# rodrigo-paganini/kalman-vae

Hardware: AMD Instinct MI355X
Metric: sequences/sec (ELBO training step, 32x32xT bouncing-ball) (higher is better)
Workload: dtype f32; 1 GPU; BASELINE configs[1] (configs[2] per-GPU shard): bouncing-ball 32x32, T=50, batch=256/GPU, dynamics=lstm K=3, z=4, u=4, a=2, full train step (fwd incl. sigmoid(x_logits) + loss incl. active-unit stats + bwd + clip + Adam); both the GPU leg and the cpu_baseline leg do this work; preset=c2, global_batch=256, seq_len=50, parallelism=dp1, capture=hipgraph, loss_finite=True, dist_backend=none

## Files before the change

include/kvae_lgssm.h:

```cpp
#ifndef KVAE_LGSSM_H
#define KVAE_LGSSM_H

#include <stdint.h>

#ifdef __cplusplus
extern "C" {
#endif

#define KVAE_MAX_DIM 16
#define KVAE_ABI_VERSION 20

typedef enum {
  KVAE_OK = 0,
  KVAE_ERR_DIMS = 1,
  KVAE_ERR_NULL = 2,
  KVAE_ERR_LAUNCH = 3,
  KVAE_ERR_ARG = 4
} kvae_status;

typedef struct {
  const float *ptr;
  int64_t sb, st;
} kvae_stack;

typedef struct {
  int32_t B, T, n, m, p;
  kvae_stack A;
  kvae_stack Bm;
  kvae_stack C;
  kvae_stack Q;
  const float *R;
  const float *mu0;
  int64_t mu0_sb;
  const float *Sigma0;
  int64_t Sigma0_sb;
  const float *Y;
  const float *U;
  const float *mask;
} kvae_lgssm_problem;

typedef struct {
  float *mus_filt;
  float *Sigmas_filt;
  float *mus_pred;
  float *Sigmas_pred;
  float *mus_smooth;
  float *Sigmas_smooth;
  float *aux;
} kvae_lgssm_states;
#define KVAE_AUX(n, p) ((n) * (p) + (p) * (p) + (n) * (n))

typedef struct {
  float *ptr;
  int64_t sb, st;
} kvae_gstack;

typedef struct {
  kvae_gstack gA, gB, gC, gQ;
  float *gY, *gU;
  float *g_mu0, *g_Sigma0;
} kvae_lgssm_input_grads;


int kvae_lgssm_filter_fwd(const kvae_lgssm_problem *prob, const kvae_lgssm_states *out, void *stream);

int kvae_lgssm_rts_fwd(const kvae_lgssm_problem *prob, const kvae_lgssm_states *io, void *stream);

int kvae_lgssm_smooth_fwd(const kvae_lgssm_problem *prob, const kvae_lgssm_states *out, void *stream);

int kvae_lgssm_filter_alpha_lstm(const kvae_lgssm_problem *prob, const kvae_lgssm_states *out, const float *w_ih,
                                 const float *w_hh, const float *b_ih, const float *b_hh, const float *head_w,
                                 const float *head_b, const float *A, const float *Bm, const float *C, int32_t K, int32_t H,
                                 float *record, float *alpha, float *gates, float *c_seq, float *h_seq, float *x_seq,
                                 void *stream);


int kvae_lgssm_smooth_bwd(const kvae_lgssm_problem *prob, const kvae_lgssm_states *saved,
                          const kvae_lgssm_states *up, const kvae_lgssm_input_grads *out,
                          float *ws, int with_rts, void *stream);

int kvae_lgssm_alpha_lstm_bwd(const kvae_lgssm_problem *prob, const kvae_lgssm_states *saved, const kvae_lgssm_states *up,
                              const kvae_lgssm_input_grads *out, float *ws, int with_rts, const float *w_ih,
                              const float *w_hh, const float *head_w, const float *A, const float *Bm, const float *C,
                              int32_t K, int32_t H, const float *alpha, const float *gates, const float *c_seq,
                              const float *g_record_up, const float *g_alpha_up, float *g_record, float *d_pre,
                              float *g_logit, void *stream);


int kvae_lgssm_elbo(const kvae_lgssm_problem *prob, const float *mus_smooth, const float *Sigmas_smooth,
                    const float *eps, float *terms, int32_t *chol_levels, float *ws_lz, float *g_mus,
                    float *g_Sigmas, const kvae_lgssm_input_grads *g, void *stream);


int kvae_mix_fwd(const float *alpha, const float *base, float *out, int64_t rows, int32_t K, int32_t E,
                 void *stream);

int kvae_mix_bwd(const float *alpha, const float *base, const float *g_out, float *g_alpha, float *g_base,
                 float *partials, int64_t rows, int32_t K, int32_t E, int32_t accumulate_alpha, void *stream);
int64_t kvae_mix_bwd_partials(int64_t rows);


int kvae_lstm_fwd(const float *x, const float *w_ih, const float *w_hh, const float *b_ih, const float *b_hh,
                  float *h_seq, float *gates, float *c_seq, int32_t B, int32_t T, int32_t I, int32_t H, void *stream);

int kvae_lstm_bwd(const float *g_h, const float *gates, const float *c_seq, const float *w_ih, const float *w_hh,
                  float *d_pre, float *dx, int32_t B, int32_t T, int32_t I, int32_t H, void *stream);


int kvae_regime_fwd(const float *logits, const float *init_logits, const float *gumbel, const float *P, float *y_seq,
                    float *log_q, float *log_p, int32_t B, int32_t T, int32_t K, float tau, const float *tau_dev,
                    int32_t hard, void *stream);
int kvae_regime_bwd(const float *logits, const float *init_logits, const float *gumbel, const float *P,
                    const float *y_seq, const float *g_y, const float *g_log_q, const float *g_log_p, float *g_logits,
                    float *g_init, int32_t B, int32_t T, int32_t K, float tau, const float *tau_dev, void *stream);

int kvae_regime_decode(const float *logits, const float *init_logits, const float *P, float *marginals, int32_t *path,
                       float *path_logq, float *kl, void *ws, int32_t B, int32_t T, int32_t K, void *stream);
int64_t kvae_regime_decode_ws_bytes(int64_t B, int32_t T, int32_t K);


int kvae_bigru_fwd(const float *x, const float *const w_ih[2], const float *const w_hh[2], const float *const b_ih[2],
                   const float *const b_hh[2], float *h_seq, float *gates, int32_t B, int32_t T, int32_t I, int32_t H,
                   void *stream);
int kvae_bigru_bwd(const float *g_h, const float *gates, const float *h_seq, const float *const w_ih[2],
                   const float *const w_hh[2], float *d_pre_i, float *d_pre_h, float *dx, int32_t B, int32_t T,
                   int32_t I, int32_t H, void *stream);


int kvae_bias_shuffle_act_fwd(const float *in, const float *bias, float *out, int64_t N, int32_t C, int32_t H,
                              int32_t W, int32_t r, int32_t relu, void *stream);
int kvae_bias_shuffle_act_bwd(const float *g_out, const float *out, float *g_in, float *bias_partials, int64_t N,
                              int32_t C, int32_t H, int32_t W, int32_t r, int32_t relu, void *stream);
int64_t kvae_bias_partial_rows(int64_t N);
int kvae_colsum(const float *partials, float *out, int64_t rows, int64_t cols, void *stream);
int kvae_colsum2(const float *partials_a, float *out_a, int64_t rows_a, int64_t cols_a, const float *partials_b, float *out_b,
                 int64_t rows_b, int64_t cols_b, void *stream);


int kvae_clip_adam(float *params, const float *grads, float *exp_avg, float *exp_avg_sq, int64_t n, const int32_t *seg_of,
                   int32_t n_seg, const float *seg_active, float *seg_steps, const float *lr_dev, float lr, float beta1, float beta2,
                   float eps, float weight_decay, float clip, const float *div_dev, float *norm_out, float *ws, void *stream);


int kvae_lgssm_emission_means(const kvae_lgssm_problem *prob, const float *mus_smooth, const float *mus_filt, float *a_imputed,
                              float *a_filtered, void *stream);


typedef struct kvae_wgrad_problem {
  const float *d;
  const float *h;
  const float *x;
  float *g_wh, *g_wx, *g_b;
  int64_t d_stride, h_stride, x_stride, N;
  int32_t R, H, I, bias, T, shift;
} kvae_wgrad_problem;
int64_t kvae_rnn_wgrad_ws_floats(const kvae_wgrad_problem *probs, int32_t n);
int kvae_rnn_wgrad(const kvae_wgrad_problem *probs, int32_t n, float *ws, void *stream);

int kvae_linear_fwd(const float *x, int64_t x_stride, int64_t N, int32_t F, const float *W, const float *b, int32_t O,
                    int32_t softmax, float *y, void *stream);
int kvae_linear_bwd_input(const float *g, const float *y, int64_t N, int32_t F, const float *W, int32_t O, float *g_logit,
                          float *dx, int64_t dx_stride, void *stream);


int kvae_bce_frames_fwd(const float *logits, const float *x, float *frame_ll, int64_t frames, int32_t pixels, void *stream);
int kvae_bce_frames_bwd(const float *logits, const float *x, const float *g_frame, float *g_logits, int64_t frames,
                        int32_t pixels, void *stream);


#define KVAE_DEC_HEAD_SCRATCH_FLOATS 2304
int kvae_dec_head_fwd(const float *in, const float *W, const float *bias, float *logits, float *w_scratch, int64_t N,
                      int32_t Cin, int32_t side, void *stream);
int kvae_dec_head_bwd(const float *in, const float *W, const float *g_logits, float *g_in, float *w_partials,
                      float *b_partials, float *w_scratch, int64_t N, int32_t Cin, int32_t side, void *stream);
int kvae_dec_head_loss_fwd(const float *in, const float *W, const float *bias, const float *x, float *logits, float *x_recon,
                           float *frame_ll, float *w_scratch, int64_t N, int32_t Cin, int32_t side, void *stream);
int kvae_dec_head_loss_bwd(const float *in, const float *W, const float *logits, const float *x, const float *g_frame, float *g_in,
                           float *w_partials, float *b_partials, float *w_scratch, int64_t N, int32_t Cin, int32_t side,
                           void *stream);
int kvae_enc_stem_fwd(const float *x, const float *W, const float *bias, float *out, uint32_t *relu_bits, int64_t N, int32_t Cout,
                      int32_t side, void *stream);
int kvae_enc_stem_bwd(const float *x, const float *out, const uint32_t *relu_bits, const float *g_out, float *w_partials,
                      float *b_partials, int64_t N, int32_t Cout, int32_t side, void *stream);
int64_t kvae_conv_edge_partial_rows(int64_t N);

int kvae_enc_mid_fwd(const float *in, const float *W, const float *bias, float *out, int64_t N, int32_t C, int32_t side,
                     void *stream);
int kvae_enc_mid_bwd(const float *in, const float *W, const float *out, const float *g_out, float *g_in,
                     float *w_partials, float *b_partials, int64_t N, int32_t C, int32_t side, void *stream);
int64_t kvae_enc_mid_partial_rows(int64_t N, int32_t side);

int kvae_dec_up_fwd(const float *x, const float *W, const float *bias, float *out, int64_t N, int32_t Cin, int32_t side,
                    void *stream);
int kvae_dec_up_bwd(const float *x, const float *W, const float *out, const float *g_out, float *g_x, float *w_partials,
                    float *b_partials, int64_t N, int32_t Cin, int32_t side, void *stream);
int64_t kvae_dec_up_partial_rows(int64_t N, int32_t side);
int32_t kvae_dec_up_set_workgroups(int32_t n);


int kvae_enc_head_fwd(const float *feat, const float *Wmu, const float *bmu, const float *Wvar, const float *bvar,
                      const float *eps, float *mu, float *var, float *a, int64_t N, int32_t F, int32_t A,
                      float noise_emission, void *stream);
int kvae_enc_head_bwd(const float *feat, const float *Wmu, const float *Wvar, const float *var, const float *eps,
                      const float *g_a, const float *g_mu, const float *g_var, float *g_feat, float *w_partials,
                      float *b_partials, int64_t N, int32_t F, int32_t A, float noise_emission, void *stream);
int kvae_dec_fc_fwd(const float *a, const float *W, const float *b, float *h, int64_t N, int32_t F, int32_t A, void *stream);
int kvae_dec_fc_bwd(const float *g_h, const float *a, const float *W, float *g_a, float *w_partials, float *b_partials,
                    int64_t N, int32_t F, int32_t A, void *stream);
int64_t kvae_head_partial_rows(void);
int kvae_latent_reg_fwd(const float *a, const float *mu, const float *var, float *reg, int64_t N, int32_t A, void *stream);
int kvae_latent_reg_bwd(const float *a, const float *mu, const float *var, const float *g, float *g_a, float *g_mu,
                        float *g_var, int64_t N, int32_t A, void *stream);

int kvae_loss_head_fwd(const float *lpx, const float *regf, const float *mask, const float *elbo_kf, const float *beta,
                       float scale_reconstruction, float vae_weight, float kf_weight, const float *weights_dev, float *out6,
                       float *coef3, int64_t n, void *stream);
int kvae_loss_head_bwd(const float *g_loss, const float *coef3, const float *mask, float *g_lpx, float *g_regf,
                       float *g_elbo_kf, int64_t n, void *stream);

typedef struct {
  int32_t B, S, H;
  int32_t n, m, p, K;
  int32_t kind;
  int32_t hidden;
  const float *A;
  const float *Bm;
  const float *C;
  const float *LQ;
  const float *LR;
  const float *mu;
  const float *L0;
  const float *U;
  const float *w_ih;
  const float *w_hh;
  const float *b_ih;
  const float *b_hh;
  const float *head_w;
  const float *head_b;
  const float *h0;
  const float *c0;
  const float *y0;
  const float *P;
  const float *s0;
  const float *eps0;
  const float *eps_z;
  const float *eps_a;
  const float *gumbel;
  float *a_out;
  float *z_out;
  float *w_out;
} kvae_gen_problem;
int kvae_lgssm_generate(const kvae_gen_problem *prob, void *stream);

#define KVAE_PSAMPLE_GAINS 1
#define KVAE_PSAMPLE_PATHS 2
typedef struct {
  int32_t B, S, T;
  int32_t n, p;
  int32_t stages;
  const float *mus_filt;
  const float *Sigmas_filt;
  const float *mus_pred;
  const float *Sigmas_pred;
  kvae_stack A;
  kvae_stack C;
  kvae_stack Q;
  const float *LR;
  const float *eps;
  const float *eta;
  float *z_out;
  float *a_out;
  int32_t *levels_out;
  float *ws;
} kvae_psample_problem;
int kvae_lgssm_posterior_sample(const kvae_psample_problem *prob, void *stream);
int64_t kvae_lgssm_posterior_sample_ws_floats(const kvae_psample_problem *prob);

typedef struct {
  int32_t B, T, n, p;
  const float *mus_pred;
  const float *Sigmas_pred;
  kvae_stack C;
  const float *R;
  const float *y;
  const float *mask;
  float *ll;
  float *nis;
  float *a_pred;
  float *S_out;
  int32_t *levels;
  float *seq_ll;
} kvae_pred_problem;
int kvae_lgssm_predictive(const kvae_pred_problem *prob, void *stream);

typedef struct {
  const float *g_ll;
  const float *g_seq;
  float *g_mus_pred;
  float *g_Sigmas_pred;
  float *gY;
  kvae_gstack gC;
} kvae_pred_grads;
int kvae_lgssm_predictive_bwd(const kvae_pred_problem *prob, const kvae_pred_grads *g, void *stream);

typedef struct {
  int32_t B, T, K, n, m, p;
  const float *A;
  const float *Bm;
  const float *Q;
  const float *C;
  const float *R;
  const float *P;
  const float *mu0;
  const float *Sigma0;
  const float *y;
  const float *u;
  const float *mask;
  const float *state_log_w;
  const float *state_mu;
  const float *state_Sigma;
  float *regime_filt;
  float *regime_pred;
  float *ll;
  float *seq_ll;
  float *a_pred;
  float *S_out;
  float *mus_filt;
  float *Sigmas_filt;
  int32_t *levels;
  float *out_log_w;
  float *out_mu;
  float *out_Sigma;
} kvae_swf_problem;
int kvae_lgssm_switching_filter(const kvae_swf_problem *prob, void *stream);

typedef struct {
  kvae_swf_problem filt;
  float *hist_mu;
  float *hist_Sigma;
  float *hist_W;
  float *hist_w;
  float *regime_smooth;
  float *regime_pairs;
  float *mus_smooth;
  float *Sigmas_smooth;
} kvae_sws_problem;
int kvae_lgssm_switching_smoother(const kvae_sws_problem *prob, void *stream);

typedef struct {
  kvae_swf_problem filt;
  float *hist_lw;
  float *hist_mu;
  float *hist_Sigma;
} kvae_swm_problem;
typedef struct {
  const float *g_ll;
  const float *g_seq;
  float *ws;
  float *gA;
  float *gB;
  float *gQ;
  float *gC;
  float *g_logP;
  float *g_mu0;
  float *g_Sigma0;
  float *gY;
  float *gU;
  float *ll_recomputed;
} kvae_swm_grads;
int kvae_lgssm_switching_marginal(const kvae_swm_problem *prob, void *stream);
int kvae_lgssm_switching_marginal_bwd(const kvae_swm_problem *prob, const kvae_swm_grads *g, void *stream);
int64_t kvae_lgssm_switching_marginal_ws_floats(int32_t B, int32_t K, int32_t n, int32_t m);

typedef struct {
  float *ws;
  float *N;
  float *S11;
  float *S10;
  float *S00;
  float *counts;
  float *Syz;
  float *Szz;
  float *Syy;
  float *Nobs;
  float *z0;
  float *z0z0;
  float *nseq;
} kvae_em_stats;
int kvae_lgssm_switching_em(const kvae_sws_problem *prob, const kvae_em_stats *st, void *stream);
int64_t kvae_lgssm_switching_em_ws_floats(int32_t B, int32_t K, int32_t n, int32_t m);

int kvae_abi_version(void);
const char *kvae_last_error(void);
const char *kvae_build_info(void);

#ifdef __cplusplus
}
#endif
#endif
```

kalman-vae_amd/csrc/kvae_vae.hip:

```cpp
#include <hip/hip_runtime.h>

#include <stdint.h>
#include <stdio.h>
#include <stdlib.h>
#include <string.h>

#include "../../include/kvae_lgssm.h"

namespace kvae {}
using namespace kvae;

extern "C" int kvae_launch_status(const char *what);
static int launch_status(const char *what) { return kvae_launch_status(what); }

#include "vae_epilogue.h"

__device__ __forceinline__ void colsum_v4_body(const float *__restrict__ partials, float *__restrict__ out, int64_t rows, int64_t cols,
                                               unsigned block) {
  __shared__ float4 red[8][64];
  const int lane = threadIdx.x & 63, wv = threadIdx.x >> 6;
  const int64_t c = ((int64_t)block * 64 + lane) * 4;
  float4 s0 = make_float4(0.f, 0.f, 0.f, 0.f), s1 = s0, s2 = s0, s3 = s0;
  if (c < cols) {
    const float *p = partials + c;
    int64_t r = wv;
    for (; r + 24 < rows; r += 32) {
      const float4 a = *reinterpret_cast<const float4 *>(p + r * cols), b = *reinterpret_cast<const float4 *>(p + (r + 8) * cols),
                   d = *reinterpret_cast<const float4 *>(p + (r + 16) * cols), e = *reinterpret_cast<const float4 *>(p + (r + 24) * cols);
      s0.x += a.x; s0.y += a.y; s0.z += a.z; s0.w += a.w;
      s1.x += b.x; s1.y += b.y; s1.z += b.z; s1.w += b.w;
      s2.x += d.x; s2.y += d.y; s2.z += d.z; s2.w += d.w;
      s3.x += e.x; s3.y += e.y; s3.z += e.z; s3.w += e.w;
    }
    for (; r < rows; r += 8) {
      const float4 a = *reinterpret_cast<const float4 *>(p + r * cols);
      s0.x += a.x; s0.y += a.y; s0.z += a.z; s0.w += a.w;
    }
  }
  red[wv][lane] = make_float4((s0.x + s1.x) + (s2.x + s3.x), (s0.y + s1.y) + (s2.y + s3.y), (s0.z + s1.z) + (s2.z + s3.z),
                              (s0.w + s1.w) + (s2.w + s3.w));
  __syncthreads();
  if (wv == 0 && c < cols) {
    float4 t = red[0][lane];
#pragma unroll
    for (int w = 1; w < 8; ++w) { const float4 u = red[w][lane]; t.x += u.x; t.y += u.y; t.z += u.z; t.w += u.w; }
    *reinterpret_cast<float4 *>(out + c) = t;
  }
}
__global__ __launch_bounds__(512) void k_colsum_v4(const float *__restrict__ partials, float *__restrict__ out, int64_t rows,
                                                   int64_t cols) {
  colsum_v4_body(partials, out, rows, cols, blockIdx.x);
}
__global__ __launch_bounds__(512) void k_colsum_v4_pair(const float *__restrict__ pa, float *__restrict__ oa, int64_t rows_a, int64_t cols_a,
                                                        unsigned nb_a, const float *__restrict__ pb, float *__restrict__ ob,
                                                        int64_t rows_b, int64_t cols_b) {
  if (blockIdx.x < nb_a) colsum_v4_body(pa, oa, rows_a, cols_a, blockIdx.x);
  else colsum_v4_body(pb, ob, rows_b, cols_b, blockIdx.x - nb_a);
}
__global__ __launch_bounds__(256) void k_colsum(const float *__restrict__ partials, float *__restrict__ out, int64_t rows,
                                                int64_t cols) {
  __shared__ float red[256];
  const int cx = threadIdx.x & 63, ry = threadIdx.x >> 6;
  const int64_t c = (int64_t)blockIdx.x * 64 + cx;
  float s0 = 0.f, s1 = 0.f;
  if (c < cols) {
    int64_t r = ry;
    for (; r + 4 < rows; r += 8) {
      s0 += partials[r * cols + c];
      s1 += partials[(r + 4) * cols + c];
    }
    if (r < rows) s0 += partials[r * cols + c];
  }
  red[threadIdx.x] = s0 + s1;
  __syncthreads();
  if (ry == 0 && c < cols) out[c] = (red[cx] + red[64 + cx]) + (red[128 + cx] + red[192 + cx]);
}

template <int R>
__global__ __launch_bounds__(256) void k_vae_epilogue_fwd_v4(const float *__restrict__ in, const float *__restrict__ bias,
                                                             float *__restrict__ out, int C, int H, int W, int64_t quads,
                                                             int relu) {
  const int OW = W * R, OH = H * R, QW = OW / 4;
  for (int64_t qd = (int64_t)blockIdx.x * 256 + threadIdx.x; qd < quads; qd += (int64_t)gridDim.x * 256) {
    const int qw = (int)(qd % QW);
    const int64_t t1 = qd / QW;
    const int oh = (int)(t1 % OH);
    const int64_t t2 = t1 / OH;
    const int c = (int)(t2 % C);
    const int64_t n = t2 / C;
    float4 v;
    if (R == 1) {
      const float b = bias[c];
      const float4 x = *reinterpret_cast<const float4 *>(in + ((n * C + c) * H + oh) * W + 4 * qw);
      v = make_float4(x.x + b, x.y + b, x.z + b, x.w + b);
    } else {
      const int ch0 = c * 4 + (oh & 1) * 2;
      const int64_t base = ((n * (C * 4) + ch0) * H + (oh >> 1)) * W + 2 * qw;
      const float2 a = *reinterpret_cast<const float2 *>(in + base);
      const float2 d = *reinterpret_cast<const float2 *>(in + base + (int64_t)H * W);
      const float b0 = bias[ch0], b1 = bias[ch0 + 1];
      v = make_float4(a.x + b0, d.x + b1, a.y + b0, d.y + b1);
    }
    if (relu) v = make_float4(fmaxf(v.x, 0.f), fmaxf(v.y, 0.f), fmaxf(v.z, 0.f), fmaxf(v.w, 0.f));
    *reinterpret_cast<float4 *>(out + qd * 4) = v;
  }
}

__global__ __launch_bounds__(256) void k_vae_epilogue_fwd(const float *in, const float *bias, float *out, EpiShape s,
                                                          int64_t total, int relu) {
  for (int64_t o = (int64_t)blockIdx.x * 256 + threadIdx.x; o < total; o += (int64_t)gridDim.x * 256)
    epi_fwd_elem(s, in, bias, out, o, relu);
}

__global__ __launch_bounds__(256) void k_vae_epilogue_bwd_bias(const float *__restrict__ g_out, const float *__restrict__ out,
                                                               float *__restrict__ g_in, float *__restrict__ bias_partials,
                                                               EpiShape s, int n_per_chunk, int relu) {
  extern __shared__ float bins[];
  const int Cin = s.C * s.r * s.r;
  const int OW = s.W * s.r, OH = s.H * s.r;
  const int64_t vol = (int64_t)s.C * OH * OW;
  for (int i = threadIdx.x; i < Cin; i += 256) bins[i] = 0.f;
  __syncthreads();
  const int64_t pos = (int64_t)blockIdx.x * 256 + threadIdx.x;
  if (pos < vol) {
    const int ow = (int)(pos % OW);
    const int oh = (int)((pos / OW) % OH);
    const int c = (int)(pos / ((int64_t)OW * OH));
    const int ch = c * s.r * s.r + (oh % s.r) * s.r + (ow % s.r);
    const int64_t in_off = ((int64_t)ch * s.H + oh / s.r) * s.W + ow / s.r;
    const int64_t in_vol = (int64_t)Cin * s.H * s.W;
    const int64_t n0 = (int64_t)blockIdx.y * n_per_chunk;
    const int64_t n1 = n0 + n_per_chunk < s.N ? n0 + n_per_chunk : s.N;
    float acc = 0.f;
    for (int64_t n = n0; n < n1; ++n) {
      float g = g_out[n * vol + pos];
      if (relu && !(out[n * vol + pos] > 0.f)) g = 0.f;
      g_in[n * in_vol + in_off] = g;
      acc += g;
    }
    atomicAdd(&bins[ch], acc);
  }
  __syncthreads();
  for (int i = threadIdx.x; i < Cin; i += 256) {
    if (bins[i] != 0.f) atomicAdd(&bias_partials[(int64_t)blockIdx.y * Cin + i], bins[i]);
  }
}

__global__ __launch_bounds__(256) void k_vae_epilogue_bwd(const float *g_out, const float *out, float *g_in, EpiShape s,
                                                          int64_t total, int relu) {
  for (int64_t o = (int64_t)blockIdx.x * 256 + threadIdx.x; o < total; o += (int64_t)gridDim.x * 256)
    epi_bwd_elem(s, g_out, out, g_in, o, relu);
}

#define KVAE_EPI_SAMPLES_PER_CHUNK 32
extern "C" int64_t kvae_bias_partial_rows(int64_t N);
static unsigned epi_grid(int64_t total) {
  const int64_t blocks = (total + 255) / 256;
  return (unsigned)(blocks < 256 * 32 ? blocks : 256 * 32);
}

extern "C" {
int kvae_bias_shuffle_act_fwd(const float *in, const float *bias, float *out, int64_t N, int32_t C, int32_t H, int32_t W,
                              int32_t r, int32_t relu, void *stream) {
  if (!in || !bias || !out) return KVAE_ERR_NULL;
  if (N < 1 || C < 1 || H < 1 || W < 1 || r < 1) return KVAE_ERR_ARG;
  const EpiShape s{N, C, H, W, r};
  const int64_t total = N * C * H * W * r * r;
  const bool aligned = ((uintptr_t)in % 16 == 0) && ((uintptr_t)out % 16 == 0);
  if (aligned && r == 1 && W % 4 == 0)
    k_vae_epilogue_fwd_v4<1><<<dim3(epi_grid(total / 4)), dim3(256), 0, (hipStream_t)stream>>>(in, bias, out, C, H, W, total / 4, relu);
  else if (aligned && r == 2 && W % 2 == 0)
    k_vae_epilogue_fwd_v4<2><<<dim3(epi_grid(total / 4)), dim3(256), 0, (hipStream_t)stream>>>(in, bias, out, C, H, W, total / 4, relu);
  else
    k_vae_epilogue_fwd<<<dim3(epi_grid(total)), dim3(256), 0, (hipStream_t)stream>>>(in, bias, out, s, total, relu);
  return launch_status("k_vae_epilogue_fwd");
}
int kvae_bias_shuffle_act_bwd(const float *g_out, const float *out, float *g_in, float *bias_partials, int64_t N, int32_t C,
                              int32_t H, int32_t W, int32_t r, int32_t relu, void *stream) {
  if (!g_out || !g_in || (relu && !out)) return KVAE_ERR_NULL;
  if (N < 1 || C < 1 || H < 1 || W < 1 || r < 1) return KVAE_ERR_ARG;
  const EpiShape s{N, C, H, W, r};
  const int64_t total = N * C * H * W * r * r;
  hipStream_t st = (hipStream_t)stream;
  if (bias_partials) {
    const int Cin = C * r * r;
    const int64_t chunks = kvae_bias_partial_rows(N);
    if (hipMemsetAsync(bias_partials, 0, sizeof(float) * chunks * Cin, st) != hipSuccess) return launch_status("memset bias_partials");
    const int64_t vol = (int64_t)C * H * W * r * r;
    k_vae_epilogue_bwd_bias<<<dim3((unsigned)((vol + 255) / 256), (unsigned)chunks), dim3(256), sizeof(float) * Cin, st>>>(
        g_out, out, g_in, bias_partials, s, KVAE_EPI_SAMPLES_PER_CHUNK, relu);
    return launch_status("k_vae_epilogue_bwd_bias");
  }
  k_vae_epilogue_bwd<<<dim3(epi_grid(total)), dim3(256), 0, st>>>(g_out, out, g_in, s, total, relu);
  return launch_status("k_vae_epilogue_bwd");
}
int kvae_colsum(const float *partials, float *out, int64_t rows, int64_t cols, void *stream) {
  if (!partials || !out) return KVAE_ERR_NULL;
  if (rows < 1 || cols < 1) return KVAE_ERR_ARG;
  if ((cols & 3) == 0 && ((((uintptr_t)partials | (uintptr_t)out) & 15) == 0))
    k_colsum_v4<<<dim3((unsigned)((cols + 255) / 256)), dim3(512), 0, (hipStream_t)stream>>>(partials, out, rows, cols);
  else
    k_colsum<<<dim3((unsigned)((cols + 63) / 64)), dim3(256), 0, (hipStream_t)stream>>>(partials, out, rows, cols);
  return launch_status("k_colsum");
}
int kvae_colsum2(const float *pa, float *oa, int64_t rows_a, int64_t cols_a, const float *pb, float *ob, int64_t rows_b,
                 int64_t cols_b, void *stream) {
  if (!pa || !oa || !pb || !ob) return KVAE_ERR_NULL;
  if (rows_a < 1 || cols_a < 1 || rows_b < 1 || cols_b < 1) return KVAE_ERR_ARG;
  if (((cols_a | cols_b) & 3) == 0 && ((((uintptr_t)pa | (uintptr_t)oa | (uintptr_t)pb | (uintptr_t)ob) & 15) == 0)) {
    const unsigned nb_a = (unsigned)((cols_a + 255) / 256), nb_b = (unsigned)((cols_b + 255) / 256);
    k_colsum_v4_pair<<<dim3(nb_a + nb_b), dim3(512), 0, (hipStream_t)stream>>>(pa, oa, rows_a, cols_a, nb_a, pb, ob, rows_b, cols_b);
    return launch_status("k_colsum_v4_pair");
  }
  const int rc = kvae_colsum(pa, oa, rows_a, cols_a, stream);
  return rc ? rc : kvae_colsum(pb, ob, rows_b, cols_b, stream);
}
int64_t kvae_bias_partial_rows(int64_t N) { return (N + KVAE_EPI_SAMPLES_PER_CHUNK - 1) / KVAE_EPI_SAMPLES_PER_CHUNK; }
}

constexpr int CA_BLOCKS = 512;
constexpr int CA_MAX_SEG = 1024;
__global__ __launch_bounds__(256) void k_grad_sumsq(const float *__restrict__ g, int64_t n, const int32_t *__restrict__ seg_of,
                                                    int n_seg, const float *__restrict__ seg_active,
                                                    const float *__restrict__ div_dev, float *__restrict__ seg_steps,
                                                    float *__restrict__ ws) {
  __shared__ float red[256];
  const float inv = div_dev ? 1.0f / fmaxf(*div_dev, 1.0f) : 1.0f;
  float s = 0.f;
  for (int64_t i = (int64_t)blockIdx.x * 256 + threadIdx.x; i < n; i += (int64_t)gridDim.x * 256) {
    float v = g[i] * inv;
    if (seg_active && seg_active[seg_of ? seg_of[i] : 0] == 0.f) v = 0.f;
    s = fmaf(v, v, s);
  }
  red[threadIdx.x] = s;
  __syncthreads();
  for (int o = 128; o > 0; o >>= 1) {
    if ((int)threadIdx.x < o) red[threadIdx.x] += red[threadIdx.x + o];
    __syncthreads();
  }
  if (threadIdx.x == 0) ws[blockIdx.x] = red[0];
  if (blockIdx.x == 0)
    for (int sg = threadIdx.x; sg < n_seg; sg += 256)
      if (!seg_active || seg_active[sg] != 0.f) seg_steps[sg] += 1.0f;
}
__global__ __launch_bounds__(256) void k_clip_adam(float *__restrict__ p, const float *__restrict__ g, float *__restrict__ m,
                                                   float *__restrict__ v, int64_t n, const int32_t *__restrict__ seg_of, int n_seg,
                                                   const float *__restrict__ seg_active, const float *__restrict__ seg_steps,
                                                   const float *__restrict__ lr_dev, float lr, float beta1, float beta2, float eps,
                                                   float wd, float clip, const float *__restrict__ div_dev,
                                                   float *__restrict__ norm_out, const float *__restrict__ ws, int nparts) {
  __shared__ float red[256];
  __shared__ float s_step_size[CA_MAX_SEG], s_bc2s[CA_MAX_SEG];
  float s = 0.f;
  for (int i = threadIdx.x; i < nparts; i += 256) s += ws[i];
  red[threadIdx.x] = s;
  const float lrv = lr_dev ? *lr_dev : lr;
  for (int sg = threadIdx.x; sg < n_seg; sg += 256) {
    const float step = seg_steps[sg];
    const bool on = !seg_active || seg_active[sg] != 0.f;
    s_step_size[sg] = on ? lrv / (1.0f - powf(beta1, step)) : -1.0f;
    s_bc2s[sg] = on ? sqrtf(1.0f - powf(beta2, step)) : 1.0f;
  }
  __syncthreads();
  for (int o = 128; o > 0; o >>= 1) {
    if ((int)threadIdx.x < o) red[threadIdx.x] += red[threadIdx.x + o];
    __syncthreads();
  }
  const float total = sqrtf(red[0]);
  if (norm_out && blockIdx.x == 0 && threadIdx.x == 0) *norm_out = total;
  const float inv = div_dev ? 1.0f / fmaxf(*div_dev, 1.0f) : 1.0f;
  const float scale = inv * (clip > 0.f ? fminf(clip / (total + 1e-6f), 1.0f) : 1.0f);
  for (int64_t i = (int64_t)blockIdx.x * 256 + threadIdx.x; i < n; i += (int64_t)gridDim.x * 256) {
    const int sg = seg_of ? seg_of[i] : 0;
    const float step_size = s_step_size[sg], bc2s = s_bc2s[sg];
    if (step_size < 0.f) continue;
    float gi = g[i] * scale;
    const float pi = p[i];
    if (wd != 0.f) gi = fmaf(wd, pi, gi);
    const float mi = m[i] + (gi - m[i]) * (1.0f - beta1);
    const float vi = beta2 * v[i] + (1.0f - beta2) * gi * gi;
    m[i] = mi, v[i] = vi;
    p[i] = pi - step_size * mi / (sqrtf(vi) / bc2s + eps);
  }
}
extern "C" int kvae_clip_adam(float *params, const float *grads, float *exp_avg, float *exp_avg_sq, int64_t n,
                              const int32_t *seg_of, int32_t n_seg, const float *seg_active, float *seg_steps, const float *lr_dev,
                              float lr, float beta1, float beta2, float eps, float weight_decay, float clip, const float *div_dev,
                              float *norm_out, float *ws, void *stream) {
  if (!params || !grads || !exp_avg || !exp_avg_sq || !seg_steps || !ws) return KVAE_ERR_NULL;
  if (n < 1 || n_seg < 1 || n_seg > CA_MAX_SEG || (!seg_of && n_seg != 1)) return KVAE_ERR_ARG;
  const int64_t want = (n + 1023) / 1024;
  const unsigned parts = (unsigned)(want < CA_BLOCKS ? want : CA_BLOCKS);
  k_grad_sumsq<<<dim3(parts), dim3(256), 0, (hipStream_t)stream>>>(grads, n, seg_of, n_seg, seg_active, div_dev, seg_steps, ws);
  int rc = launch_status("k_grad_sumsq");
  if (rc) return rc;
  const unsigned blocks = (unsigned)((n + 255) / 256 < 2048 ? (n + 255) / 256 : 2048);
  k_clip_adam<<<dim3(blocks), dim3(256), 0, (hipStream_t)stream>>>(params, grads, exp_avg, exp_avg_sq, n, seg_of, n_seg, seg_active,
                                                                   seg_steps, lr_dev, lr, beta1, beta2, eps, weight_decay, clip,
                                                                   div_dev, norm_out, ws, (int)parts);
  return launch_status("k_clip_adam");
}

#include "vae_loss.h"

__global__ __launch_bounds__(256) void k_vae_bce_fwd(const float *__restrict__ logits, const float *__restrict__ x,
                                                     float *__restrict__ frame_ll, int64_t frames, int pixels) {
  const int64_t f = (int64_t)blockIdx.x * 4 + (threadIdx.x >> 6);
  const int lane = threadIdx.x & 63;
  if (f >= frames) return;
  const float *l = logits + f * pixels, *t = x + f * pixels;
  float acc = 0.f;
  if ((pixels & 3) == 0 && (((uintptr_t)l | (uintptr_t)t) & 15) == 0) {
    for (int i = lane * 4; i < pixels; i += 256) {
      const float4 a = *reinterpret_cast<const float4 *>(l + i), b = *reinterpret_cast<const float4 *>(t + i);
      acc += bce_logit(a.x, b.x) + bce_logit(a.y, b.y) + bce_logit(a.z, b.z) + bce_logit(a.w, b.w);
    }
  } else {
    for (int i = lane; i < pixels; i += 64) acc += bce_logit(l[i], t[i]);
  }
  for (int off = 32; off > 0; off >>= 1) acc += __shfl_down(acc, off, 64);
  if (lane == 0) frame_ll[f] = -acc;
}

__global__ __launch_bounds__(256) void k_vae_bce_bwd(const float *__restrict__ logits, const float *__restrict__ x,
                                                     const float *__restrict__ g_frame, float *__restrict__ g_logits,
                                                     int64_t total, int pixels) {
  for (int64_t i = ((int64_t)blockIdx.x * 256 + threadIdx.x) * 4; i < total; i += (int64_t)gridDim.x * 1024) {
    const float g = -g_frame[i / pixels];
    const float4 a = *reinterpret_cast<const float4 *>(logits + i), b = *reinterpret_cast<const float4 *>(x + i);
    *reinterpret_cast<float4 *>(g_logits + i) = make_float4(g * (sigmoid_stable(a.x) - b.x), g * (sigmoid_stable(a.y) - b.y),
                                                            g * (sigmoid_stable(a.z) - b.z), g * (sigmoid_stable(a.w) - b.w));
  }
}
__global__ __launch_bounds__(256) void k_vae_bce_bwd_scalar(const float *logits, const float *x, const float *g_frame,
                                                            float *g_logits, int64_t total, int pixels) {
  for (int64_t i = (int64_t)blockIdx.x * 256 + threadIdx.x; i < total; i += (int64_t)gridDim.x * 256)
    g_logits[i] = -g_frame[i / pixels] * (sigmoid_stable(logits[i]) - x[i]);
}

extern "C" {
int kvae_bce_frames_fwd(const float *logits, const float *x, float *frame_ll, int64_t frames, int32_t pixels, void *stream) {
  if (!logits || !x || !frame_ll) return KVAE_ERR_NULL;
  if (frames < 1 || pixels < 1) return KVAE_ERR_ARG;
  k_vae_bce_fwd<<<dim3((unsigned)((frames + 3) / 4)), dim3(256), 0, (hipStream_t)stream>>>(logits, x, frame_ll, frames, pixels);
  return launch_status("k_vae_bce_fwd");
}
int kvae_bce_frames_bwd(const float *logits, const float *x, const float *g_frame, float *g_logits, int64_t frames,
                        int32_t pixels, void *stream) {
  if (!logits || !x || !g_frame || !g_logits) return KVAE_ERR_NULL;
  if (frames < 1 || pixels < 1) return KVAE_ERR_ARG;
  const int64_t total = frames * pixels;
  const bool v4 = (pixels & 3) == 0 && ((((uintptr_t)logits | (uintptr_t)x | (uintptr_t)g_logits) & 15) == 0);
  if (v4)
    k_vae_bce_bwd<<<dim3(epi_grid(total / 4)), dim3(256), 0, (hipStream_t)stream>>>(logits, x, g_frame, g_logits, total, pixels);
  else
    k_vae_bce_bwd_scalar<<<dim3(epi_grid(total)), dim3(256), 0, (hipStream_t)stream>>>(logits, x, g_frame, g_logits, total, pixels);
  return launch_status("k_vae_bce_bwd");
}
}

#include "vae_conv_edge.h"
extern "C" {
int64_t kvae_conv_edge_partial_rows(int64_t N) { return N < 1024 ? (N < 1 ? 1 : N) : 1024; }

int kvae_dec_head_fwd(const float *in, const float *W, const float *bias, float *logits, float *w_scratch, int64_t N,
                      int32_t Cin, int32_t side, void *stream) {
  if (!in || !W || !bias || !logits || !w_scratch) return KVAE_ERR_NULL;
  if (N < 1) return KVAE_ERR_ARG;
  if (Cin != DH_CI || side != DH_S) return KVAE_ERR_DIMS;
  k_dec_head_prep<<<dim3(1), dim3(256), 0, (hipStream_t)stream>>>(W, w_scratch);
  k_dec_head_fwd<false><<<dim3((unsigned)N), dim3(256), 0, (hipStream_t)stream>>>(in, w_scratch, bias, logits, nullptr, nullptr, nullptr);
  return launch_status("k_dec_head_fwd");
}
int kvae_dec_head_loss_fwd(const float *in, const float *W, const float *bias, const float *x, float *logits, float *x_recon,
                           float *frame_ll, float *w_scratch, int64_t N, int32_t Cin, int32_t side, void *stream) {
  if (!in || !W || !bias || !x || !logits || !frame_ll || !w_scratch) return KVAE_ERR_NULL;
  if (N < 1) return KVAE_ERR_ARG;
  if (Cin != DH_CI || side != DH_S) return KVAE_ERR_DIMS;
  k_dec_head_prep<<<dim3(1), dim3(256), 0, (hipStream_t)stream>>>(W, w_scratch);
  k_dec_head_fwd<true><<<dim3((unsigned)N), dim3(256), 0, (hipStream_t)stream>>>(in, w_scratch, bias, logits, x, x_recon, frame_ll);
  return launch_status("k_dec_head_loss_fwd");
}
}
template <bool LOSS>
static int dec_head_bwd_launch(const float *in, const float *W, const float *g_logits, const float *logits, const float *x,
                               const float *g_frame, float *g_in, float *w_partials, float *b_partials, float *w_scratch,
                               int64_t N, hipStream_t st) {
  const dim3 grid((unsigned)kvae_conv_edge_partial_rows(N));
  if (g_in) {
    k_dec_head_prep<<<dim3(1), dim3(256), 0, st>>>(W, w_scratch);
    k_dec_head_bwd<LOSS, true><<<grid, dim3(256), 0, st>>>(in, g_logits, logits, x, g_frame, w_scratch, g_in, w_partials, b_partials, N);
  } else {
    k_dec_head_bwd<LOSS, false><<<grid, dim3(256), 0, st>>>(in, g_logits, logits, x, g_frame, w_scratch, g_in, w_partials, b_partials, N);
  }
  return launch_status("k_dec_head_bwd");
}
extern "C" {
int kvae_dec_head_bwd(const float *in, const float *W, const float *g_logits, float *g_in, float *w_partials,
                      float *b_partials, float *w_scratch, int64_t N, int32_t Cin, int32_t side, void *stream) {
  if (!in || !W || !g_logits || !w_partials || !b_partials || !w_scratch) return KVAE_ERR_NULL;
  if (N < 1) return KVAE_ERR_ARG;
  if (Cin != DH_CI || side != DH_S) return KVAE_ERR_DIMS;
  return dec_head_bwd_launch<false>(in, W, g_logits, nullptr, nullptr, nullptr, g_in, w_partials, b_partials, w_scratch, N,
                                    (hipStream_t)stream);
}
int kvae_dec_head_loss_bwd(const float *in, const float *W, const float *logits, const float *x, const float *g_frame, float *g_in,
                           float *w_partials, float *b_partials, float *w_scratch, int64_t N, int32_t Cin, int32_t side,
                           void *stream) {
  if (!in || !W || !logits || !x || !g_frame || !w_partials || !b_partials || !w_scratch) return KVAE_ERR_NULL;
  if (N < 1) return KVAE_ERR_ARG;
  if (Cin != DH_CI || side != DH_S) return KVAE_ERR_DIMS;
  return dec_head_bwd_launch<true>(in, W, nullptr, logits, x, g_frame, g_in, w_partials, b_partials, w_scratch, N,
                                   (hipStream_t)stream);
}
int kvae_enc_stem_fwd(const float *x, const float *W, const float *bias, float *out, uint32_t *relu_bits, int64_t N, int32_t Cout,
                      int32_t side, void *stream) {
  if (!x || !W || !bias || !out) return KVAE_ERR_NULL;
  if (N < 1) return KVAE_ERR_ARG;
  if (Cout != ES_CO || side != ES_IN) return KVAE_ERR_DIMS;
  k_enc_stem_fwd<<<dim3((unsigned)N), dim3(256), 0, (hipStream_t)stream>>>(x, W, bias, out, relu_bits);
  return launch_status("k_enc_stem_fwd");
}
int kvae_enc_stem_bwd(const float *x, const float *out, const uint32_t *relu_bits, const float *g_out, float *w_partials,
                      float *b_partials, int64_t N, int32_t Cout, int32_t side, void *stream) {
  if (!x || (!out && !relu_bits) || !g_out || !w_partials || !b_partials) return KVAE_ERR_NULL;
  if (N < 1) return KVAE_ERR_ARG;
  if (Cout != ES_CO || side != ES_IN) return KVAE_ERR_DIMS;
  static const int mfma = getenv("KVAE_STEM_MFMA") ? atoi(getenv("KVAE_STEM_MFMA")) : 1;
  const dim3 grid((unsigned)kvae_conv_edge_partial_rows(N));
  if (mfma == 1 && relu_bits) k_enc_stem_wrw_mfma<true><<<grid, dim3(256), 0, (hipStream_t)stream>>>(x, out, relu_bits, g_out, w_partials, b_partials, N);
  else if (!out) return KVAE_ERR_NULL;
  else if (mfma) k_enc_stem_wrw_mfma<false><<<grid, dim3(256), 0, (hipStream_t)stream>>>(x, out, relu_bits, g_out, w_partials, b_partials, N);
  else k_enc_stem_wrw<<<grid, dim3(256), 0, (hipStream_t)stream>>>(x, out, g_out, w_partials, b_partials, N);
  return launch_status("k_enc_stem_wrw");
}
}

#include "vae_conv_mid.h"
static inline int64_t enc_mid_grid(int64_t N, int32_t side) {
  const int64_t fpi = side == 16 ? 2 : 8, iters = (N + fpi - 1) / fpi;
  return iters < 256 ? (iters < 1 ? 1 : iters) : 256;
}
extern "C" {
int64_t kvae_enc_mid_partial_rows(int64_t N, int32_t side) { return enc_mid_grid(N, side); }

int kvae_enc_mid_fwd(const float *in, const float *W, const float *bias, float *out, int64_t N, int32_t C, int32_t side,
                     void *stream) {
  if (!in || !W || !bias || !out) return KVAE_ERR_NULL;
  if (N < 1 || (N + 256 * 8) * EM_C * side * side * 4 >= EM_MAX_BYTES) return KVAE_ERR_ARG;
  if (C != EM_C || (side != 16 && side != 8)) return KVAE_ERR_DIMS;
  const dim3 grid((unsigned)enc_mid_grid(N, side));
  if (side == 16) k_enc_mid_fwd<16><<<grid, dim3(256), 0, (hipStream_t)stream>>>(in, W, bias, out, N);
  else k_enc_mid_fwd<8><<<grid, dim3(256), 0, (hipStream_t)stream>>>(in, W, bias, out, N);
  return launch_status("k_enc_mid_fwd");
}
int kvae_enc_mid_bwd(const float *in, const float *W, const float *out, const float *g_out, float *g_in,
                     float *w_partials, float *b_partials, int64_t N, int32_t C, int32_t side, void *stream) {
  if (!in || !W || !out || !g_out || !w_partials || !b_partials) return KVAE_ERR_NULL;
  if (N < 1 || (N + 256 * 8) * EM_C * side * side * 4 >= EM_MAX_BYTES) return KVAE_ERR_ARG;
  if (C != EM_C || (side != 16 && side != 8)) return KVAE_ERR_DIMS;
  const dim3 grid((unsigned)enc_mid_grid(N, side));
  if (g_in) {
    if (side == 16) k_enc_mid_bwd_data<16><<<grid, dim3(256), 0, (hipStream_t)stream>>>(W, out, g_out, g_in, N);
    else k_enc_mid_bwd_data<8><<<grid, dim3(256), 0, (hipStream_t)stream>>>(W, out, g_out, g_in, N);
    const int rc = launch_status("k_enc_mid_bwd_data");
    if (rc) return rc;
  }
  if (side == 16) k_enc_mid_wrw<16><<<grid, dim3(256), 0, (hipStream_t)stream>>>(in, out, g_out, w_partials, b_partials, N);
  else k_enc_mid_wrw<8><<<grid, dim3(256), 0, (hipStream_t)stream>>>(in, out, g_out, w_partials, b_partials, N);
  return launch_status("k_enc_mid_wrw");
}
}

#include "vae_conv_up_wino.h"
static bool dec_up_wino() {
  static const int env = getenv("KVAE_WINO") ? atoi(getenv("KVAE_WINO")) : 1;
  return env != 0;
}
static int g_dec_up_wgs = 0;
static inline int64_t dec_up_cap() {
  static const int env = getenv("KVAE_UP_WGS") ? atoi(getenv("KVAE_UP_WGS")) : 0;
  const int v = env >= 1 && env <= 256 ? env : __atomic_load_n(&g_dec_up_wgs, __ATOMIC_RELAXED);
  return v >= 1 && v <= 256 ? v : 256;
}
static inline int64_t dec_up_grid(int64_t N, int32_t side) {
  const int64_t fpi = side == 8 ? 2 : 8, iters = (N + fpi - 1) / fpi, cap = dec_up_cap();
  return iters < cap ? (iters < 1 ? 1 : iters) : cap;
}
extern "C" {
int64_t kvae_dec_up_partial_rows(int64_t N, int32_t side) { return dec_up_grid(N, side); }
int32_t kvae_dec_up_set_workgroups(int32_t n) {
  const int32_t prev = (int32_t)dec_up_cap();
  __atomic_store_n(&g_dec_up_wgs, n >= 1 && n <= 256 ? n : 0, __ATOMIC_RELAXED);
  return prev;
}

int kvae_dec_up_fwd(const float *x, const float *W, const float *bias, float *out, int64_t N, int32_t Cin, int32_t side,
                    void *stream) {
  if (!x || !W || !bias || !out) return KVAE_ERR_NULL;
  if (N < 1 || (N + 256 * 8) * UP_CO * side * side * 4 >= EM_MAX_BYTES) return KVAE_ERR_ARG;
  if (Cin != UP_CI || (side != 8 && side != 4)) return KVAE_ERR_DIMS;
  const dim3 grid((unsigned)dec_up_grid(N, side));
  if (dec_up_wino()) {
    const int64_t sets = side == 8 ? N : (N + 3) / 4;
    const dim3 wgrid((unsigned)(sets < dec_up_cap() ? sets : dec_up_cap()));
    if (side == 8) k_dec_up_fwd_wino<8><<<wgrid, dim3(512), 0, (hipStream_t)stream>>>(x, W, bias, out, N);
    else k_dec_up_fwd_wino<4><<<wgrid, dim3(512), 0, (hipStream_t)stream>>>(x, W, bias, out, N);
    return launch_status("k_dec_up_fwd_wino");
  }
  if (side == 8) k_dec_up_fwd<8><<<grid, dim3(256), 0, (hipStream_t)stream>>>(x, W, bias, out, N);
  else k_dec_up_fwd<4><<<grid, dim3(256), 0, (hipStream_t)stream>>>(x, W, bias, out, N);
  return launch_status("k_dec_up_fwd");
}
int kvae_dec_up_bwd(const float *x, const float *W, const float *out, const float *g_out, float *g_x, float *w_partials,
                    float *b_partials, int64_t N, int32_t Cin, int32_t side, void *stream) {
  if (!x || !W || !out || !g_out || !w_partials || !b_partials) return KVAE_ERR_NULL;
  if (N < 1 || (N + 256 * 8) * UP_CO * side * side * 4 >= EM_MAX_BYTES) return KVAE_ERR_ARG;
  if (Cin != UP_CI || (side != 8 && side != 4)) return KVAE_ERR_DIMS;
  const dim3 grid((unsigned)dec_up_grid(N, side));
  if (g_x) {
    const int64_t sets = side == 8 ? N : (N + 3) / 4;
    const dim3 wgrid((unsigned)(sets < dec_up_cap() ? sets : dec_up_cap()));
    if (dec_up_wino() && side == 8) k_dec_up_bwd_data_wino<8><<<wgrid, dim3(512), 0, (hipStream_t)stream>>>(W, out, g_out, g_x, N);
    else if (dec_up_wino()) k_dec_up_bwd_data_wino<4><<<wgrid, dim3(512), 0, (hipStream_t)stream>>>(W, out, g_out, g_x, N);
    else if (side == 8) k_dec_up_bwd_data<8><<<grid, dim3(256), 0, (hipStream_t)stream>>>(W, out, g_out, g_x, N);
    else k_dec_up_bwd_data<4><<<grid, dim3(256), 0, (hipStream_t)stream>>>(W, out, g_out, g_x, N);
    const int rc = launch_status("k_dec_up_bwd_data");
    if (rc) return rc;
  }
  if (dec_up_wino()) {
    if (side == 8) k_dec_up_wrw_wino<8><<<grid, dim3(512), 0, (hipStream_t)stream>>>(x, out, g_out, w_partials, b_partials, N);
    else k_dec_up_wrw_wino<4><<<grid, dim3(512), 0, (hipStream_t)stream>>>(x, out, g_out, w_partials, b_partials, N);
    return launch_status("k_dec_up_wrw_wino");
  }
  if (side == 8) k_dec_up_wrw<8><<<grid, dim3(256), 0, (hipStream_t)stream>>>(x, out, g_out, w_partials, b_partials, N);
  else k_dec_up_wrw<4><<<grid, dim3(256), 0, (hipStream_t)stream>>>(x, out, g_out, w_partials, b_partials, N);
  return launch_status("k_dec_up_wrw");
}
}

#include "vae_heads.h"
extern "C" {
int64_t kvae_head_partial_rows(void) { return HD_WAVES; }

int kvae_enc_head_fwd(const float *feat, const float *Wmu, const float *bmu, const float *Wvar, const float *bvar,
                      const float *eps, float *mu, float *var, float *a, int64_t N, int32_t F, int32_t A,
                      float noise_emission, void *stream) {
  if (!feat || !Wmu || !bmu || !Wvar || !bvar || !mu || !var || !a) return KVAE_ERR_NULL;
  if (N < 1) return KVAE_ERR_ARG;
  if (F != HD_F || A != HD_A) return KVAE_ERR_DIMS;
  const unsigned grid = (unsigned)(N < 4 * 512 ? (N + 3) / 4 : 512);
  k_enc_head_fwd<<<dim3(grid), dim3(256), 0, (hipStream_t)stream>>>(feat, Wmu, bmu, Wvar, bvar, eps, noise_emission, mu, var, a, N);
  return launch_status("k_enc_head_fwd");
}
int kvae_enc_head_bwd(const float *feat, const float *Wmu, const float *Wvar, const float *var, const float *eps,
                      const float *g_a, const float *g_mu, const float *g_var, float *g_feat, float *w_partials,
                      float *b_partials, int64_t N, int32_t F, int32_t A, float noise_emission, void *stream) {
  if (!feat || !Wmu || !Wvar || !var || !g_feat || !w_partials || !b_partials) return KVAE_ERR_NULL;
  if (N < 1) return KVAE_ERR_ARG;
  if (F != HD_F || A != HD_A) return KVAE_ERR_DIMS;
  k_enc_head_bwd<<<dim3(HD_WAVES / 4), dim3(256), 0, (hipStream_t)stream>>>(feat, Wmu, Wvar, var, eps, g_a, g_mu, g_var,
                                                                             noise_emission, g_feat, w_partials, b_partials, N);
  return launch_status("k_enc_head_bwd");
}
int kvae_dec_fc_fwd(const float *a, const float *W, const float *b, float *h, int64_t N, int32_t F, int32_t A, void *stream) {
  if (!a || !W || !b || !h) return KVAE_ERR_NULL;
  if (N < 1) return KVAE_ERR_ARG;
  if (F != HD_F || A != HD_A) return KVAE_ERR_DIMS;
  k_dec_fc_fwd<<<dim3(epi_grid(N * (HD_F / 4))), dim3(256), 0, (hipStream_t)stream>>>(a, W, b, h, N * (HD_F / 4));
  return launch_status("k_dec_fc_fwd");
}
int kvae_dec_fc_bwd(const float *g_h, const float *a, const float *W, float *g_a, float *w_partials, float *b_partials,
                    int64_t N, int32_t F, int32_t A, void *stream) {
  if (!g_h || !a || !W || !g_a || !w_partials || !b_partials) return KVAE_ERR_NULL;
  if (N < 1) return KVAE_ERR_ARG;
  if (F != HD_F || A != HD_A) return KVAE_ERR_DIMS;
  k_dec_fc_bwd<<<dim3(HD_WAVES / 4), dim3(256), 0, (hipStream_t)stream>>>(g_h, a, W, g_a, w_partials, b_partials, N);
  return launch_status("k_dec_fc_bwd");
}
int kvae_latent_reg_fwd(const float *a, const float *mu, const float *var, float *reg, int64_t N, int32_t A, void *stream) {
  if (!a || !mu || !var || !reg) return KVAE_ERR_NULL;
  if (N < 1 || A < 1) return KVAE_ERR_ARG;
  k_latent_reg_fwd<<<dim3(epi_grid(N)), dim3(256), 0, (hipStream_t)stream>>>(a, mu, var, reg, N, A);
  return launch_status("k_latent_reg_fwd");
}
int kvae_latent_reg_bwd(const float *a, const float *mu, const float *var, const float *g, float *g_a, float *g_mu,
                        float *g_var, int64_t N, int32_t A, void *stream) {
  if (!a || !mu || !var || !g || !g_a || !g_mu || !g_var) return KVAE_ERR_NULL;
  if (N < 1 || A < 1) return KVAE_ERR_ARG;
  k_latent_reg_bwd<<<dim3(epi_grid(N * A)), dim3(256), 0, (hipStream_t)stream>>>(a, mu, var, g, g_a, g_mu, g_var, N, A);
  return launch_status("k_latent_reg_bwd");
}
int kvae_loss_head_fwd(const float *lpx, const float *regf, const float *mask, const float *elbo_kf, const float *beta,
                       float scale_reconstruction, float vae_weight, float kf_weight, const float *weights_dev, float *out6,
                       float *coef3, int64_t n, void *stream) {
  if (!lpx || !regf || !elbo_kf || !beta || !out6 || !coef3) return KVAE_ERR_NULL;
  if (n < 1) return KVAE_ERR_ARG;
  k_loss_head_fwd<<<dim3(1), dim3(1024), 0, (hipStream_t)stream>>>(lpx, regf, mask, elbo_kf, beta, scale_reconstruction, vae_weight,
                                                                  kf_weight, weights_dev, out6, coef3, n);
  return launch_status("k_loss_head_fwd");
}
int kvae_loss_head_bwd(const float *g_loss, const float *coef3, const float *mask, float *g_lpx, float *g_regf,
                       float *g_elbo_kf, int64_t n, void *stream) {
  if (!g_loss || !coef3 || !g_lpx || !g_regf || !g_elbo_kf) return KVAE_ERR_NULL;
  if (n < 1) return KVAE_ERR_ARG;
  k_loss_head_bwd<<<dim3(epi_grid(n)), dim3(256), 0, (hipStream_t)stream>>>(g_loss, coef3, mask, g_lpx, g_regf,
                                                                            g_elbo_kf, n);
  return launch_status("k_loss_head_bwd");
}
}
```

kalman-vae_amd/csrc/vae_conv_edge.h:

```cpp
#pragma once
#include <hip/hip_runtime.h>
#include <stdint.h>

#include "vae_loss.h"

namespace kvae {

constexpr int DH_CI = 32, DH_CO = 4, DH_S = 16, DH_TS = 18, DH_CS = 325;
constexpr int DH_W = DH_CO * DH_CI * 9;
typedef float kv_f2 __attribute__((ext_vector_type(2)));
typedef float kv_f4 __attribute__((ext_vector_type(4)));

__global__ __launch_bounds__(256) void k_dec_head_prep(const float *__restrict__ W, float *__restrict__ scratch) {
  for (int i = threadIdx.x; i < DH_W; i += 256) {
    const int co = i / (DH_CI * 9), r = i - co * DH_CI * 9, ci = r / 9, k = r - ci * 9;
    const float w = W[i];
    scratch[(ci * 9 + k) * DH_CO + co] = w;
    scratch[DH_W + (co * 9 + k) * DH_CI + ci] = w;
  }
}

__device__ __forceinline__ void dh_zero_halo(float *tile, int channels) {
  for (int i = threadIdx.x; i < channels * 68; i += 256) {
    const int c = i / 68, j = i - c * 68;
    int r, q;
    if (j < 18) { r = 0; q = j; }
    else if (j < 36) { r = 17; q = j - 18; }
    else if (j < 52) { r = j - 35; q = 0; }
    else { r = j - 51; q = 17; }
    tile[c * DH_CS + r * DH_TS + q] = 0.f;
  }
}
__device__ __forceinline__ void dh_store_interior(float *tile, int i, const float4 v) {
  const int e = i * 4, ci = e >> 8, hw = e & 255, h = hw >> 4, w = hw & 15;
  float *d = tile + ci * DH_CS + (h + 1) * DH_TS + (w + 1);
  d[0] = v.x; d[1] = v.y; d[2] = v.z; d[3] = v.w;
}

template <bool LOSS>
__global__ __launch_bounds__(256) void k_dec_head_fwd(const float *__restrict__ in, const float *__restrict__ scratch,
                                                      const float *__restrict__ bias, float *__restrict__ logits,
                                                      const float *__restrict__ x, float *__restrict__ x_recon,
                                                      float *__restrict__ frame_ll) {
  __shared__ float tile[DH_CI * 256];
  const int64_t n = blockIdx.x;
  const float4 *src = reinterpret_cast<const float4 *>(in + n * DH_CI * 256);
  float4 pre[8];
#pragma unroll
  for (int j = 0; j < 8; ++j) pre[j] = src[threadIdx.x + 256 * j];
  const int h = threadIdx.x >> 4, w = threadIdx.x & 15;
  const int64_t po = n * 1024 + (2 * h) * 32 + 2 * w;
  float2 x01 = make_float2(0.f, 0.f), x23 = x01;
  if constexpr (LOSS) {
    x01 = *reinterpret_cast<const float2 *>(x + po);
    x23 = *reinterpret_cast<const float2 *>(x + po + 32);
  }
#pragma unroll
  for (int j = 0; j < 8; ++j) reinterpret_cast<float4 *>(tile)[threadIdx.x + 256 * j] = pre[j];
  __syncthreads();
  constexpr int OOB = 1 << 24;
  const int tb = (h - 1) * 16 + (w - 1);
  int base[9];
#pragma unroll
  for (int tap = 0; tap < 9; ++tap) {
    const int ky = tap / 3, kx = tap % 3;
    const bool z = (ky == 0 && h == 0) || (ky == 2 && h == 15) || (kx == 0 && w == 0) || (kx == 2 && w == 15);
    base[tap] = (z ? OOB : tb) + ky * 16 + kx;
  }
  kv_f2 a01 = {bias[0], bias[1]}, a23 = {bias[2], bias[3]};
  const kv_f4 *Wf = reinterpret_cast<const kv_f4 *>(scratch);
#pragma unroll 4
  for (int ci = 0; ci < DH_CI; ++ci) {
#pragma unroll
    for (int tap = 0; tap < 9; ++tap) {
      const float v = tile[base[tap] + ci * 256];
      const kv_f4 wv = Wf[ci * 9 + tap];
      a01 += wv.xy * v;
      a23 += wv.zw * v;
    }
  }
  float *o = logits + po;
  *reinterpret_cast<float2 *>(o) = make_float2(a01.x, a01.y);
  *reinterpret_cast<float2 *>(o + 32) = make_float2(a23.x, a23.y);
  if constexpr (LOSS) {
    if (x_recon) {
      *reinterpret_cast<float2 *>(x_recon + po) = make_float2(sigmoid_stable(a01.x), sigmoid_stable(a01.y));
      *reinterpret_cast<float2 *>(x_recon + po + 32) = make_float2(sigmoid_stable(a23.x), sigmoid_stable(a23.y));
    }
    float s = (bce_logit(a01.x, x01.x) + bce_logit(a01.y, x01.y)) + (bce_logit(a23.x, x23.x) + bce_logit(a23.y, x23.y));
    for (int off = 32; off > 0; off >>= 1) s += __shfl_down(s, off, 64);
    __syncthreads();
    if ((threadIdx.x & 63) == 0) tile[threadIdx.x >> 6] = s;
    __syncthreads();
    if (threadIdx.x == 0) frame_ll[n] = -((tile[0] + tile[1]) + (tile[2] + tile[3]));
  }
}

template <bool LOSS, bool DATA>
__global__ __launch_bounds__(256, 2) void k_dec_head_bwd(const float *__restrict__ in, const float *__restrict__ g_logits,
                                                         const float *__restrict__ logits, const float *__restrict__ x,
                                                         const float *__restrict__ g_frame, const float *__restrict__ scratch,
                                                         float *__restrict__ g_in, float *__restrict__ partial,
                                                         float *__restrict__ partial_b, int64_t N) {
  constexpr int CS = 257, OOB = 1 << 24;
  __shared__ float lds[DH_CI * CS + DH_CO * DH_CS];
  __shared__ float redb[8 * DH_CO];
  float *tile = lds, *gt = lds + DH_CI * CS;
  const int ci = threadIdx.x & 31, grp = threadIdx.x >> 5;
  const int tin = (((threadIdx.x & 63) >> 4) << 6) | ((threadIdx.x >> 6) << 4) | (threadIdx.x & 15);
  kv_f2 acc[DH_CO / 2][9];
  float accb[DH_CO];
#pragma unroll
  for (int c = 0; c < DH_CO / 2; ++c)
#pragma unroll
    for (int k = 0; k < 9; ++k) acc[c][k] = kv_f2{0.f, 0.f};
#pragma unroll
  for (int co = 0; co < DH_CO; ++co) accb[co] = 0.f;
  float4 pre[8];
  float gp[4], xp[4], gf = 0.f;
  auto fetch = [&](int64_t f) {
    const float4 *src = reinterpret_cast<const float4 *>(in + f * DH_CI * 256);
#pragma unroll
    for (int j = 0; j < 8; ++j) pre[j] = src[tin + 256 * j];
#pragma unroll
    for (int j = 0; j < 4; ++j) {
      if constexpr (LOSS) {
        gp[j] = logits[f * 1024 + threadIdx.x + 256 * j];
        xp[j] = x[f * 1024 + threadIdx.x + 256 * j];
      } else {
        gp[j] = g_logits[f * 1024 + threadIdx.x + 256 * j];
      }
    }
    if constexpr (LOSS) gf = -g_frame[f];
  };
  int64_t n = blockIdx.x;
  if (n < N) fetch(n);
  dh_zero_halo(gt, DH_CO);
  for (; n < N; n += gridDim.x) {
    __syncthreads();
#pragma unroll
    for (int j = 0; j < 8; ++j) {
      const int e = (tin + 256 * j) * 4;
      float *d = tile + (e >> 8) * CS + (e & 255);
      d[0] = pre[j].x; d[1] = pre[j].y; d[2] = pre[j].z; d[3] = pre[j].w;
    }
#pragma unroll
    for (int j = 0; j < 4; ++j) {
      const int i = threadIdx.x + 256 * j, oh = i >> 5, ow = i & 31, co = (oh & 1) * 2 + (ow & 1);
      float g = gp[j];
      if constexpr (LOSS) g = gf * (sigmoid_stable(gp[j]) - xp[j]);
      gt[co * DH_CS + ((oh >> 1) + 1) * DH_TS + (ow >> 1) + 1] = g;
    }
    __syncthreads();
    const int64_t nn = n + gridDim.x;
    if (nn < N) fetch(nn);
#pragma unroll
    for (int rr = 0; rr < 2; ++rr) {
      const int h = 2 * grp + rr;
      int rb[3];
#pragma unroll
      for (int ky = 0; ky < 3; ++ky) {
        const bool off = (ky == 0 && rr == 0 && grp == 0) || (ky == 2 && rr == 1 && grp == 7);
        rb[ky] = (off ? OOB : ci * CS) + (h + ky - 1) * 16;
      }
      float c0[3] = {0.f, 0.f, 0.f}, c1[3], c2[3];
#pragma unroll
      for (int ky = 0; ky < 3; ++ky) c1[ky] = tile[rb[ky]];
      const float *gr = gt + (h + 1) * DH_TS + 1;
#pragma unroll
      for (int w = 0; w < 16; ++w) {
#pragma unroll
        for (int ky = 0; ky < 3; ++ky) c2[ky] = w + 1 < 16 ? tile[rb[ky] + w + 1] : 0.f;
        const kv_f2 g01 = {gr[w], gr[DH_CS + w]}, g23 = {gr[2 * DH_CS + w], gr[3 * DH_CS + w]};
        accb[0] += g01.x; accb[1] += g01.y; accb[2] += g23.x; accb[3] += g23.y;
#pragma unroll
        for (int ky = 0; ky < 3; ++ky) {
          acc[0][ky * 3 + 0] += g01 * c0[ky]; acc[1][ky * 3 + 0] += g23 * c0[ky];
          acc[0][ky * 3 + 1] += g01 * c1[ky]; acc[1][ky * 3 + 1] += g23 * c1[ky];
          acc[0][ky * 3 + 2] += g01 * c2[ky]; acc[1][ky * 3 + 2] += g23 * c2[ky];
          c0[ky] = c1[ky];
          c1[ky] = c2[ky];
        }
      }
    }
    if constexpr (DATA) {
      __builtin_amdgcn_sched_barrier(0);
      const int h = threadIdx.x >> 4, w = threadIdx.x & 15;
      kv_f2 dacc[DH_CI / 2];
#pragma unroll
      for (int j = 0; j < DH_CI / 2; ++j) dacc[j] = kv_f2{0.f, 0.f};
      int wofs = DH_W;
      asm volatile("" : "+s"(wofs));
      const kv_f2 *Wb = reinterpret_cast<const kv_f2 *>(scratch + wofs);
#pragma unroll
      for (int co = 0; co < DH_CO; ++co)
#pragma unroll
        for (int ky = 0; ky < 3; ++ky)
#pragma unroll
          for (int kx = 0; kx < 3; ++kx) {
            const float v = gt[co * DH_CS + (h + 2 - ky) * DH_TS + (w + 2 - kx)];
            const kv_f2 *wr = Wb + (co * 9 + ky * 3 + kx) * (DH_CI / 2);
#pragma unroll
            for (int j = 0; j < DH_CI / 2; ++j) dacc[j] += wr[j] * v;
          }
      float *o = g_in + n * DH_CI * 256 + threadIdx.x;
#pragma unroll
      for (int j = 0; j < DH_CI / 2; ++j) {
        o[(2 * j) * 256] = dacc[j].x;
        o[(2 * j + 1) * 256] = dacc[j].y;
      }
    }
  }
  __syncthreads();
  float *red = lds;
#pragma unroll
  for (int k = 0; k < 9; ++k) {
    float *r = red + (grp * 32 + ci) * 36 + k;
    r[0] = acc[0][k].x; r[9] = acc[0][k].y; r[18] = acc[1][k].x; r[27] = acc[1][k].y;
  }
  if (ci == 0) {
#pragma unroll
    for (int co = 0; co < DH_CO; ++co) redb[grp * 4 + co] = accb[co];
  }
  __syncthreads();
  for (int o = threadIdx.x; o < DH_W; o += 256) {
    const int co = o / (DH_CI * 9), r = o - co * DH_CI * 9, c2 = r / 9, k = r - c2 * 9;
    float s = 0.f;
    for (int gq = 0; gq < 8; ++gq) s += red[(gq * 32 + c2) * 36 + co * 9 + k];
    partial[(int64_t)blockIdx.x * DH_W + o] = s;
  }
  if (threadIdx.x < DH_CO) {
    float s = 0.f;
    for (int gq = 0; gq < 8; ++gq) s += redb[gq * 4 + threadIdx.x];
    partial_b[(int64_t)blockIdx.x * DH_CO + threadIdx.x] = s;
  }
}


constexpr int ES_CO = 32, ES_IN = 32, ES_OUT = 16, ES_TS = 35;

__device__ __forceinline__ void es_load_tile(float *tile, const float *__restrict__ x) {
  for (int i = threadIdx.x; i < 34 * ES_TS; i += 256) tile[i] = 0.f;
  __syncthreads();
  const float4 v = reinterpret_cast<const float4 *>(x)[threadIdx.x];
  const int e = threadIdx.x * 4, h = e >> 5, w = e & 31;
  float *d = tile + (h + 1) * ES_TS + (w + 1);
  d[0] = v.x; d[1] = v.y; d[2] = v.z; d[3] = v.w;
}

__global__ __launch_bounds__(256) void k_enc_stem_fwd(const float *__restrict__ x, const float *__restrict__ W,
                                                      const float *__restrict__ bias, float *__restrict__ out,
                                                      uint32_t *__restrict__ relu_bits) {
  __shared__ float tile[34 * ES_TS];
  const int64_t n = blockIdx.x;
  es_load_tile(tile, x + n * 1024);
  __syncthreads();
  const int oh = threadIdx.x >> 4, ow = threadIdx.x & 15;
  float v[9];
#pragma unroll
  for (int ky = 0; ky < 3; ++ky)
#pragma unroll
    for (int kx = 0; kx < 3; ++kx) v[ky * 3 + kx] = tile[(2 * oh + ky) * ES_TS + 2 * ow + kx];
  float *o = out + n * ES_CO * 256 + threadIdx.x;
  uint32_t bits = 0;
#pragma unroll 8
  for (int co = 0; co < ES_CO; ++co) {
    float acc = bias[co];
#pragma unroll
    for (int k = 0; k < 9; ++k) acc = fmaf(W[co * 9 + k], v[k], acc);
    o[co * 256] = fmaxf(acc, 0.f);
    bits |= (acc > 0.f ? 1u : 0u) << co;
  }
  if (relu_bits) relu_bits[n * 256 + threadIdx.x] = bits;
}

__global__ __launch_bounds__(256) void k_enc_stem_wrw(const float *__restrict__ x, const float *__restrict__ out,
                                                      const float *__restrict__ g_out, float *__restrict__ partial,
                                                      float *__restrict__ partial_b, int64_t N) {
  __shared__ float tile[34 * ES_TS];
  __shared__ float gt[ES_CO * 257];
  const int co = threadIdx.x & 31, grp = threadIdx.x >> 5;
  float acc[9], accb = 0.f;
#pragma unroll
  for (int k = 0; k < 9; ++k) acc[k] = 0.f;
  for (int64_t n = blockIdx.x; n < N; n += gridDim.x) {
    __syncthreads();
    es_load_tile(tile, x + n * 1024);
    const float4 *g4 = reinterpret_cast<const float4 *>(g_out + n * ES_CO * 256);
    const float4 *o4 = reinterpret_cast<const float4 *>(out + n * ES_CO * 256);
    for (int i = threadIdx.x; i < ES_CO * 64; i += 256) {
      const float4 gv = g4[i], ov = o4[i];
      const int e = i * 4, c = e >> 8, hw = e & 255;
      float *d = gt + c * 257 + hw;
      d[0] = ov.x > 0.f ? gv.x : 0.f; d[1] = ov.y > 0.f ? gv.y : 0.f;
      d[2] = ov.z > 0.f ? gv.z : 0.f; d[3] = ov.w > 0.f ? gv.w : 0.f;
    }
    __syncthreads();
    for (int i = 0; i < 32; ++i) {
      const int hw = grp * 32 + i, oh = hw >> 4, ow = hw & 15;
      const float gv = gt[co * 257 + hw];
      accb += gv;
      const float *t = tile + (2 * oh) * ES_TS + 2 * ow;
#pragma unroll
      for (int ky = 0; ky < 3; ++ky)
#pragma unroll
        for (int kx = 0; kx < 3; ++kx) acc[ky * 3 + kx] = fmaf(gv, t[ky * ES_TS + kx], acc[ky * 3 + kx]);
    }
  }
  __syncthreads();
  float *red = gt;
#pragma unroll
  for (int k = 0; k < 9; ++k) red[(grp * 32 + co) * 10 + k] = acc[k];
  red[(grp * 32 + co) * 10 + 9] = accb;
  __syncthreads();
  for (int o = threadIdx.x; o < ES_CO * 10; o += 256) {
    const int c = o / 10, k = o - c * 10;
    float s = 0.f;
    for (int gq = 0; gq < 8; ++gq) s += red[(gq * 32 + c) * 10 + k];
    if (k < 9) partial[(int64_t)blockIdx.x * (ES_CO * 9) + c * 9 + k] = s;
    else partial_b[(int64_t)blockIdx.x * ES_CO + c] = s;
  }
}

typedef float es_f4 __attribute__((ext_vector_type(4)));
template <bool BITS>
__global__ __launch_bounds__(256) void k_enc_stem_wrw_mfma(const float *__restrict__ x, const float *__restrict__ out,
                                                           const uint32_t *__restrict__ relu_bits, const float *__restrict__ g_out,
                                                           float *__restrict__ partial,
                                                           float *__restrict__ partial_b, int64_t N) {
  __shared__ float tile[34 * ES_TS];
  constexpr int GS = 260;
  __shared__ __attribute__((aligned(16))) float gt[ES_CO * GS];
  __shared__ __attribute__((aligned(16))) uint32_t mw[256];
  const int lane = threadIdx.x & 63, wv = threadIdx.x >> 6, j = lane & 15, g = lane >> 4;
  const int tap = j < 9 ? j : 8;
  const float *tb = tile + (8 * wv) * ES_TS + 2 * g + (tap / 3) * ES_TS + tap % 3;
  const float *ga = gt + j * GS + 64 * wv + g;
  es_f4 acc0 = {0.f, 0.f, 0.f, 0.f}, acc1 = acc0;
  float4 gv[8], ov[8], xv;
  uint32_t mv = 0;
  auto fetch = [&](int64_t n) {
    const bool ok = n < N;
    const float4 *g4 = reinterpret_cast<const float4 *>(g_out + (ok ? n : 0) * ES_CO * 256);
    const float4 *o4 = reinterpret_cast<const float4 *>(out + (ok ? n : 0) * ES_CO * 256);
#pragma unroll
    for (int q = 0; q < 8; ++q) {
      gv[q] = g4[threadIdx.x + 256 * q];
      if constexpr (!BITS) ov[q] = o4[threadIdx.x + 256 * q];
    }
    xv = reinterpret_cast<const float4 *>(x + (ok ? n : 0) * 1024)[threadIdx.x];
    if constexpr (BITS) mv = relu_bits[(ok ? n : 0) * 256 + threadIdx.x];
  };
  fetch(blockIdx.x);
  for (int i = threadIdx.x; i < 34 * ES_TS; i += 256) tile[i] = 0.f;
  for (int64_t n = blockIdx.x; n < N; n += gridDim.x) {
    __syncthreads();
    {
      float *d = tile + ((threadIdx.x >> 3) + 1) * ES_TS + 4 * (threadIdx.x & 7) + 1;
      d[0] = xv.x; d[1] = xv.y; d[2] = xv.z; d[3] = xv.w;
    }
    if constexpr (BITS) {
      mw[threadIdx.x] = mv;
      __syncthreads();
    }
#pragma unroll
    for (int q = 0; q < 8; ++q) {
      const int e = (threadIdx.x + 256 * q) * 4, c = e >> 8, hw = e & 255;
      float4 md;
      if constexpr (BITS) {
        const uint4 m = *reinterpret_cast<const uint4 *>(mw + hw);
        md = make_float4((m.x >> c) & 1u ? gv[q].x : 0.f, (m.y >> c) & 1u ? gv[q].y : 0.f, (m.z >> c) & 1u ? gv[q].z : 0.f,
                         (m.w >> c) & 1u ? gv[q].w : 0.f);
      } else {
        md = make_float4(ov[q].x > 0.f ? gv[q].x : 0.f, ov[q].y > 0.f ? gv[q].y : 0.f, ov[q].z > 0.f ? gv[q].z : 0.f,
                         ov[q].w > 0.f ? gv[q].w : 0.f);
      }
      *reinterpret_cast<float4 *>(gt + c * GS + hw) = md;
    }
    __syncthreads();
    fetch(n + gridDim.x);
#pragma unroll
    for (int s = 0; s < 16; ++s) {
      const float xb = tb[2 * (s >> 2) * ES_TS + 8 * (s & 3)];
      const float b = j == 9 ? 1.0f : xb;
      acc0 = __builtin_amdgcn_mfma_f32_16x16x4f32(ga[4 * s], b, acc0, 0, 0, 0);
      acc1 = __builtin_amdgcn_mfma_f32_16x16x4f32(ga[16 * GS + 4 * s], b, acc1, 0, 0, 0);
    }
  }
  __syncthreads();
  float *red = gt;
#pragma unroll
  for (int r = 0; r < 4; ++r) {
    red[(wv * 32 + 4 * g + r) * 16 + j] = acc0[r];
    red[(wv * 32 + 16 + 4 * g + r) * 16 + j] = acc1[r];
  }
  __syncthreads();
  for (int o = threadIdx.x; o < ES_CO * 10; o += 256) {
    const int c = o / 10, k = o - c * 10;
    const float s = (red[c * 16 + k] + red[(32 + c) * 16 + k]) + (red[(64 + c) * 16 + k] + red[(96 + c) * 16 + k]);
    if (k < 9) partial[(int64_t)blockIdx.x * (ES_CO * 9) + c * 9 + k] = s;
    else partial_b[(int64_t)blockIdx.x * ES_CO + c] = s;
  }
}

}
```

kalman-vae_amd/csrc/vae_conv_up_wino.h:

```cpp
#pragma once
#include <type_traits>
#include "vae_conv_up.h"

namespace kvae {

typedef float wn_f4 __attribute__((ext_vector_type(4)));
#ifdef KVAE_EM_STAMPS
#define WN_STAMP(slot, k) do { if (blockIdx.x == 0 && (threadIdx.x & 63) == 0 && (slot) < 40) \
    em_stamps[((threadIdx.x >> 6) * 40 + (slot)) * 8 + (k)] = __builtin_amdgcn_s_memtime(); } while (0)
#else
#define WN_STAMP(slot, k) do {} while (0)
#endif
#define WN_MFMA(a, b, c) __builtin_amdgcn_mfma_f32_16x16x4f32((a), (b), (c), 0, 0, 0)

template <int S>
struct WinoDims {
  static constexpr int TS = S / 2;
  static constexpr int TPF = TS * TS;
  static constexpr int FPC = 16 / TPF;
  static constexpr int RS = S == 8 ? 12 : 8;
  static constexpr int PLANE = (S + 2) * RS;
  static constexpr int FS = 32 * PLANE + (S == 8 ? 0 : 4);
  static constexpr int FPI = UpDims<S>::FPI;
  static constexpr int LDS_IN = FPI * FS;
};

#define WN_BT(o0, o1, o2, o3, d0, d1, d2, d3) do { o0 = (d0) - (d2); o1 = (d1) + (d2); o2 = (d2) - (d1); o3 = (d1) - (d3); } while (0)

__device__ __forceinline__ void wino_filter(const float *g, float *u) {
  float r[4][3];
#pragma unroll
  for (int c = 0; c < 3; ++c) {
    r[0][c] = g[c];
    r[1][c] = 0.5f * (g[c] + g[3 + c] + g[6 + c]);
    r[2][c] = 0.5f * (g[c] - g[3 + c] + g[6 + c]);
    r[3][c] = g[6 + c];
  }
#pragma unroll
  for (int a = 0; a < 4; ++a) {
    u[4 * a + 0] = r[a][0];
    u[4 * a + 1] = 0.5f * (r[a][0] + r[a][1] + r[a][2]);
    u[4 * a + 2] = 0.5f * (r[a][0] - r[a][1] + r[a][2]);
    u[4 * a + 3] = r[a][2];
  }
}

__device__ __forceinline__ void wino_out(const float (&m)[16], float (&y)[4]) {
  float t[2][4];
#pragma unroll
  for (int v = 0; v < 4; ++v) {
    t[0][v] = m[v] + m[4 + v] + m[8 + v];
    t[1][v] = m[4 + v] - m[8 + v] - m[12 + v];
  }
#pragma unroll
  for (int a = 0; a < 2; ++a) {
    y[2 * a + 0] = t[a][0] + t[a][1] + t[a][2];
    y[2 * a + 1] = t[a][1] - t[a][2] - t[a][3];
  }
}

__device__ __forceinline__ void wino_patch_load(const float *p, int RS, float2 (&d)[4][2]) {
#pragma unroll
  for (int r = 0; r < 4; ++r) {
    d[r][0] = *reinterpret_cast<const float2 *>(p + r * RS);
    d[r][1] = *reinterpret_cast<const float2 *>(p + r * RS + 2);
  }
}
__device__ __forceinline__ void wino_patch_xform(const float2 (&d)[4][2], float (&v)[16]) {
  float t[4][4];
  WN_BT(t[0][0], t[1][0], t[2][0], t[3][0], d[0][0].x, d[1][0].x, d[2][0].x, d[3][0].x);
  WN_BT(t[0][1], t[1][1], t[2][1], t[3][1], d[0][0].y, d[1][0].y, d[2][0].y, d[3][0].y);
  WN_BT(t[0][2], t[1][2], t[2][2], t[3][2], d[0][1].x, d[1][1].x, d[2][1].x, d[3][1].x);
  WN_BT(t[0][3], t[1][3], t[2][3], t[3][3], d[0][1].y, d[1][1].y, d[2][1].y, d[3][1].y);
#pragma unroll
  for (int u = 0; u < 4; ++u) WN_BT(v[4 * u], v[4 * u + 1], v[4 * u + 2], v[4 * u + 3], t[u][0], t[u][1], t[u][2], t[u][3]);
}

template <int S>
struct WinoFwd {
  using D = UpDims<S>;
  using Wd = WinoDims<S>;
  static constexpr int CSX = Wd::FPC * Wd::FS;
  static constexpr int CSG = Wd::FPC * D::XFRAME;
  static constexpr int VROW = 20, VSET = 8 * 64 * VROW;
};

template <int S>
__global__ __launch_bounds__(512) void k_dec_up_fwd_wino(const float *__restrict__ x, const float *__restrict__ W,
                                                         const float *__restrict__ bias, float *__restrict__ out, int64_t N) {
  using D = UpDims<S>;
  using Wd = WinoDims<S>;
  using K = WinoFwd<S>;
  __shared__ float xin[2 * K::CSX];
  __shared__ __attribute__((aligned(16))) float vt[2 * K::VSET];
  const int tid = threadIdx.x, lane = tid & 63, wv = tid >> 6, j = lane & 15, g = lane >> 4;
  const int co0 = 16 * wv;
  const int64_t nsets = (N + Wd::FPC - 1) / Wd::FPC, stride = gridDim.x;
  const __amdgpu_buffer_rsrc_t rx = em_rsrc(x, N * D::XFRAME * 4), ry = em_rsrc(out, N * D::YFRAME * 4);
  for (int i = tid; i < 2 * K::CSX; i += 512) xin[i] = 0.f;

  float U[16][8];
#pragma unroll
  for (int s = 0; s < 8; ++s) {
    const float *w = W + ((co0 + j) * UP_CI + 4 * s + g) * 9;
    float gk[9], u[16];
#pragma unroll
    for (int t = 0; t < 9; ++t) gk[t] = w[t];
    wino_filter(gk, u);
#pragma unroll
    for (int p = 0; p < 16; ++p) U[p][s] = u[p];
  }
  float bv[4];
#pragma unroll
  for (int r = 0; r < 4; ++r) bv[r] = bias[co0 + 4 * g + r];

  const int fl = S == 8 ? 0 : (j >> 2), ty = S == 8 ? (j >> 2) : ((j >> 1) & 1), tx = S == 8 ? (j & 3) : (j & 1);
  const int pbase = fl * Wd::FS + g * Wd::PLANE + 2 * ty * Wd::RS + 2 * tx + wv * 4 * Wd::PLANE;
  const int vbase_w = (wv * 64 + lane) * K::VROW, vbase_r = lane * K::VROW;
  const int obase = fl * D::YFRAME + (co0 / 4 + g) * 4 * D::PF + 4 * ty * 2 * S + 4 * tx;
  const bool early = wv < 4;
  int sdst[1];
#pragma unroll
  for (int q = 0; q < 1; ++q) {
    const int e = (tid + 512 * q) * 4, f = e / D::XFRAME, ci = (e % D::XFRAME) / D::PF, pix = e % D::PF;
    sdst[q] = f * Wd::FS + ci * Wd::PLANE + (pix / S + 1) * Wd::RS + pix % S + 1;
  }

  float4 pre[1];
  auto fetch = [&](int64_t k) {
#pragma unroll
    for (int q = 0; q < 1; ++q) pre[q] = em_ld4(rx, (uint32_t)(k * K::CSG + (tid + 512 * q) * 4) * 4u);
  };
  auto stage = [&](float *xw) {
#pragma unroll
    for (int q = 0; q < 1; ++q) {
      float *d = xw + sdst[q];
      d[0] = pre[q].x; d[1] = pre[q].y; d[2] = pre[q].z; d[3] = pre[q].w;
    }
  };
  auto transform = [&](const float *xr, float *vw) {
#pragma unroll
    for (int h = 0; h < 1; ++h) {
      float2 d[4][2];
      float v[16];
      wino_patch_load(xr + pbase + h * 4 * Wd::PLANE, Wd::RS, d);
      wino_patch_xform(d, v);
#pragma unroll
      for (int q = 0; q < 4; ++q)
        *reinterpret_cast<float4 *>(vw + vbase_w + h * 64 * K::VROW + 4 * q) = make_float4(v[4 * q], v[4 * q + 1], v[4 * q + 2], v[4 * q + 3]);
    }
  };
  auto compute_p = [&](const float *vr, int64_t k) {
    float y[4][4];
#pragma unroll
    for (int r = 0; r < 4; ++r)
#pragma unroll
      for (int q = 0; q < 4; ++q) y[r][q] = 0.f;
    float2 bq[8], bn[8];
#pragma unroll
    for (int s = 0; s < 8; ++s) bq[s] = *reinterpret_cast<const float2 *>(vr + vbase_r + s * 64 * K::VROW);
    float sb[4][2];
    wn_f4 p0 = wn_f4{0.f, 0.f, 0.f, 0.f}, p1 = p0;
    auto fold = [&](int pq, int r) {
      const int u = pq >> 1, h = pq & 1;
      if (h == 0) sb[r][0] = p0[r] + p1[r], sb[r][1] = p1[r];
      else {
        sb[r][0] += p0[r], sb[r][1] -= p0[r] + p1[r];
        if (u == 0) y[r][0] += sb[r][0], y[r][1] += sb[r][1];
        if (u == 1) y[r][0] += sb[r][0], y[r][1] += sb[r][1], y[r][2] += sb[r][0], y[r][3] += sb[r][1];
        if (u == 2) y[r][0] += sb[r][0], y[r][1] += sb[r][1], y[r][2] -= sb[r][0], y[r][3] -= sb[r][1];
        if (u == 3) y[r][2] -= sb[r][0], y[r][3] -= sb[r][1];
      }
      asm volatile("" : "+v"(sb[r][0]), "+v"(sb[r][1]), "+v"(y[r][0]), "+v"(y[r][1]), "+v"(y[r][2]), "+v"(y[r][3]));
    };
#pragma unroll
    for (int pp = 0; pp < 8; ++pp) {
      wn_f4 a0 = wn_f4{0.f, 0.f, 0.f, 0.f}, a1 = a0;
#pragma unroll
      for (int s = 0; s < 8; ++s) {
        a0 = WN_MFMA(U[2 * pp][s], bq[s].x, a0);
        a1 = WN_MFMA(U[2 * pp + 1][s], bq[s].y, a1);
        if (pp + 1 < 8) bn[s] = *reinterpret_cast<const float2 *>(vr + vbase_r + s * 64 * K::VROW + 2 * (pp + 1));
        if (pp > 0 && (s & 1)) fold(pp - 1, s >> 1);
        __builtin_amdgcn_sched_barrier(0);
      }
      p0 = a0, p1 = a1;
#pragma unroll
      for (int s = 0; s < 8; ++s) bq[s] = bn[s];
    }
#pragma unroll
    for (int r = 0; r < 4; ++r) fold(7, r);
    const uint32_t o0 = (uint32_t)(k * Wd::FPC * D::YFRAME + obase);
#pragma unroll
    for (int r = 0; r < 4; ++r)
#pragma unroll
      for (int q = 0; q < 4; ++q) y[r][q] = fmaxf(y[r][q] + bv[r], 0.f);
#pragma unroll
    for (int a = 0; a < 2; ++a)
#pragma unroll
      for (int dy = 0; dy < 2; ++dy) {
        const float4 row = make_float4(y[2 * dy][2 * a], y[2 * dy + 1][2 * a], y[2 * dy][2 * a + 1], y[2 * dy + 1][2 * a + 1]);
        em_st4(ry, (o0 + (uint32_t)((2 * a + dy) * 2 * S)) * 4u, row);
      }
  };

#define WN_COMPUTE(vr, k) compute_p((vr), (k))

  int64_t k = blockIdx.x;
  fetch(k);
  __syncthreads();
  stage(xin);
  fetch(k + stride);
  __syncthreads();
  transform(xin, vt);
  stage(xin + K::CSX);
  fetch(k + 2 * stride);
  __syncthreads();
  for (int slot = 0; k < nsets; k += 2 * stride, ++slot) {
    WN_STAMP(slot, 0);
    if (early) {
      stage(xin);
      fetch(k + 3 * stride);
      transform(xin + K::CSX, vt + K::VSET);
    }
    WN_STAMP(slot, 1);
    WN_COMPUTE(vt, k);
    WN_STAMP(slot, 2);
    if (!early) {
      stage(xin);
      fetch(k + 3 * stride);
      transform(xin + K::CSX, vt + K::VSET);
    }
    __syncthreads();
    WN_STAMP(slot, 3);
    if (early) {
      stage(xin + K::CSX);
      fetch(k + 4 * stride);
      transform(xin, vt);
    }
    WN_STAMP(slot, 4);
    WN_COMPUTE(vt + K::VSET, k + stride);
    WN_STAMP(slot, 5);
    if (!early) {
      stage(xin + K::CSX);
      fetch(k + 4 * stride);
      transform(xin, vt);
    }
    __syncthreads();
    WN_STAMP(slot, 6);
  }
}

template <int S>
struct WinoBwd {
  static constexpr int RAW = 8192;
  static constexpr int RS = S == 8 ? 12 : 6;
  static constexpr int PLANE = S == 8 ? 120 : 24;
  static constexpr int FSB = 128 * PLANE + (S == 8 ? 0 : 24);
  static constexpr int GY = WinoDims<S>::FPC * FSB;
  static constexpr int RED = 2048;
};

template <int S>
__global__ __launch_bounds__(512) void k_dec_up_bwd_data_wino(const float *__restrict__ W, const float *__restrict__ out,
                                                              const float *__restrict__ g_out, float *__restrict__ g_x, int64_t N) {
  using D = UpDims<S>;
  using Wd = WinoDims<S>;
  using K = WinoBwd<S>;
  __shared__ __attribute__((aligned(16))) float raw[2 * K::RAW];
  __shared__ __attribute__((aligned(16))) float work[K::GY + 4 * K::RED];
  float *rawg = raw, *rawo = raw + K::RAW, *gy = work, *red = work + K::GY;
  const int tid = threadIdx.x, lane = tid & 63, wv = tid >> 6, j = lane & 15, g = lane >> 4, hh = wv & 1, kq = wv >> 1;
  const int64_t stride = gridDim.x, nsets = (N + Wd::FPC - 1) / Wd::FPC;
  const __amdgpu_buffer_rsrc_t rg = em_rsrc(g_out, N * D::YFRAME * 4), ro = em_rsrc(out, N * D::YFRAME * 4),
                               rgx = em_rsrc(g_x, N * D::XFRAME * 4);
  for (int i = tid; i < K::GY; i += 512) gy[i] = 0.f;

  float U[16][8];
#pragma unroll
  for (int s = 0; s < 8; ++s) {
    const float *w = W + ((32 * kq + 4 * s + g) * UP_CI + 16 * hh + j) * 9;
    float gk[9], u[16];
#pragma unroll
    for (int t = 0; t < 9; ++t) gk[t] = w[8 - t];
    wino_filter(gk, u);
#pragma unroll
    for (int p = 0; p < 16; ++p) U[p][s] = u[p];
  }
  const int fl = S == 8 ? 0 : (j >> 2), ty = S == 8 ? (j >> 2) : ((j >> 1) & 1), tx = S == 8 ? (j & 3) : (j & 1);
  int prow[4];
#pragma unroll
  for (int r = 0; r < 4; ++r) {
    const int row = S == 8 ? 2 * ty + r : 2 * ty - 1 + r;
    prow[r] = (S == 4 && (row < 0 || row > 3)) ? EM_OOB : fl * K::FSB + (32 * kq + g) * K::PLANE + row * K::RS + 2 * tx;
  }
  const int rbase = kq * K::RED + fl * D::XFRAME + (16 * hh + 4 * g) * D::PF + 2 * ty * S + 2 * tx;

  auto dma_piece = [&](int64_t k, int q) {
    int t2 = tid;
    asm volatile("" : "+v"(t2));
    const uint32_t off = (uint32_t)(k * K::RAW + (t2 + 512 * q) * 4) * 4u;
    __builtin_amdgcn_raw_ptr_buffer_load_lds(rg, (__attribute__((address_space(3))) void *)(rawg + (wv * 64 + 512 * q) * 4), 16, off, 0, 0, 0);
    __builtin_amdgcn_raw_ptr_buffer_load_lds(ro, (__attribute__((address_space(3))) void *)(rawo + (wv * 64 + 512 * q) * 4), 16, off, 0, 0, 0);
  };
  auto dma = [&](int64_t k) {
#pragma unroll
    for (int q = 0; q < 4; ++q) dma_piece(k, q);
  };
  auto convert = [&]() {
    int t2 = tid;
    asm volatile("" : "+v"(t2));
#pragma unroll
    for (int q = 0; q < 4; ++q) {
      const int e = (t2 + 512 * q) * 4;
      const float4 gv = *reinterpret_cast<const float4 *>(rawg + e), ov = *reinterpret_cast<const float4 *>(rawo + e);
      float *d;
      if constexpr (S == 8) {
        const int c = e >> 8, y = (e >> 4) & 15, xx = e & 15;
        d = gy + (4 * c + 2 * (y & 1)) * K::PLANE + ((y >> 1) + 1) * K::RS + (xx >> 1) + 1;
      } else {
        const int f = e >> 11, c = (e >> 6) & 31, y = (e >> 3) & 7, xx = e & 7;
        d = gy + f * K::FSB + (4 * c + 2 * (y & 1)) * K::PLANE + (y >> 1) * K::RS + (xx >> 1) + 1;
      }
      d[0] = ov.x > 0.f ? gv.x : 0.f;
      d[K::PLANE] = ov.y > 0.f ? gv.y : 0.f;
      d[1] = ov.z > 0.f ? gv.z : 0.f;
      d[K::PLANE + 1] = ov.w > 0.f ? gv.w : 0.f;
    }
  };
  uint32_t done = 0x80000000u;
  auto fold = [&]() {
    int t2 = tid;
    asm volatile("" : "+v"(t2));
    const float4 a = *reinterpret_cast<const float4 *>(red + 4 * t2), b = *reinterpret_cast<const float4 *>(red + K::RED + 4 * t2),
                 c = *reinterpret_cast<const float4 *>(red + 2 * K::RED + 4 * t2), d = *reinterpret_cast<const float4 *>(red + 3 * K::RED + 4 * t2);
    em_st4(rgx, done + (uint32_t)t2 * 16u, make_float4((a.x + b.x) + (c.x + d.x), (a.y + b.y) + (c.y + d.y), (a.z + b.z) + (c.z + d.z),
                                                        (a.w + b.w) + (c.w + d.w)));
  };
  auto patch = [&](int s, float2 (&d)[4][2]) {
#pragma unroll
    for (int r = 0; r < 4; ++r) {
      const float *p = gy + prow[r] + s * 4 * K::PLANE;
      d[r][0] = *reinterpret_cast<const float2 *>(p);
      d[r][1] = *reinterpret_cast<const float2 *>(p + 2);
    }
  };
  auto compute = [&](int64_t knext) {
    wn_f4 acc[16];
#pragma unroll
    for (int p = 0; p < 16; ++p) acc[p] = wn_f4{0.f, 0.f, 0.f, 0.f};
    float2 d[4][2], dn[4][2];
    patch(0, d);
#pragma unroll
    for (int s = 0; s < 8; ++s) {
      if (s + 1 < 8) patch(s + 1, dn);
      float v[16];
      wino_patch_xform(d, v);
      __builtin_amdgcn_sched_barrier(0);
#pragma unroll
      for (int p = 0; p < 16; ++p) acc[p] = WN_MFMA(U[p][s], v[p], acc[p]);
      __builtin_amdgcn_sched_barrier(0);
      if (s < 4) dma_piece(knext, s);
      __builtin_amdgcn_sched_barrier(0);
#pragma unroll
      for (int r = 0; r < 4; ++r) d[r][0] = dn[r][0], d[r][1] = dn[r][1];
    }
#pragma unroll
    for (int r = 0; r < 4; ++r) {
      float m[16], y[4];
#pragma unroll
      for (int p = 0; p < 16; ++p) m[p] = acc[p][r];
      wino_out(m, y);
      *reinterpret_cast<float2 *>(red + rbase + r * D::PF) = make_float2(y[0], y[1]);
      *reinterpret_cast<float2 *>(red + rbase + r * D::PF + S) = make_float2(y[2], y[3]);
    }
  };

  int64_t k = blockIdx.x;
  dma(k);
  __syncthreads();
  for (int slot = 0; k < nsets; k += stride, ++slot) {
    WN_STAMP(slot, 0);
    convert();
    fold();
    WN_STAMP(slot, 1);
    __syncthreads();
    WN_STAMP(slot, 2);
    WN_STAMP(slot, 3);
    compute(k + stride);
    done = (uint32_t)(k * 2048) * 4u;
    WN_STAMP(slot, 4);
    __syncthreads();
    WN_STAMP(slot, 5);
  }
  fold();
}

template <int S>
struct WinoWrw {
  static constexpr int RAW = 8192;
  static constexpr int GY4 = 8192;
  static constexpr int RS = S == 8 ? 12 : 6;
  static constexpr int XP = S == 8 ? 130 : 38;
  static constexpr int XPL = WinoDims<S>::FPC * 32 * XP;
  static constexpr int VROW = 20, VSET = 8 * 64 * VROW;
};

template <int S>
__global__ __launch_bounds__(512) void k_dec_up_wrw_wino(const float *__restrict__ x, const float *__restrict__ out,
                                                         const float *__restrict__ g_out, float *__restrict__ w_partials,
                                                         float *__restrict__ b_partials, int64_t N) {
  using D = UpDims<S>;
  using Wd = WinoDims<S>;
  using K = WinoWrw<S>;
  __shared__ __attribute__((aligned(16))) float raw[2 * K::RAW];
  __shared__ __attribute__((aligned(16))) float work[K::GY4 + K::XPL + K::VSET];
  float *rawg = raw, *rawo = raw + K::RAW, *gy4 = work, *xp = work + K::GY4, *vt = xp + K::XPL;
  const int tid = threadIdx.x, lane = tid & 63, wv = tid >> 6, j = lane & 15, g = lane >> 4;
  const int64_t stride = gridDim.x, nsets = (N + Wd::FPC - 1) / Wd::FPC;
  const __amdgpu_buffer_rsrc_t rx = em_rsrc(x, N * D::XFRAME * 4), rg = em_rsrc(g_out, N * D::YFRAME * 4),
                               ro = em_rsrc(out, N * D::YFRAME * 4);
  for (int i = tid; i < K::XPL; i += 512) xp[i] = 0.f;

  wn_f4 acc[16][2];
#pragma unroll
  for (int p = 0; p < 16; ++p) acc[p][0] = acc[p][1] = wn_f4{0.f, 0.f, 0.f, 0.f};
  float bsum = 0.f;

  auto dma_piece = [&](int64_t k, int q) {
    int t2 = tid;
    asm volatile("" : "+v"(t2));
    const uint32_t off = (uint32_t)(k * K::RAW + (t2 + 512 * q) * 4) * 4u;
    __builtin_amdgcn_raw_ptr_buffer_load_lds(rg, (__attribute__((address_space(3))) void *)(rawg + (wv * 64 + 512 * q) * 4), 16, off, 0, 0, 0);
    __builtin_amdgcn_raw_ptr_buffer_load_lds(ro, (__attribute__((address_space(3))) void *)(rawo + (wv * 64 + 512 * q) * 4), 16, off, 0, 0, 0);
  };
  auto dma = [&](int64_t k) {
#pragma unroll
    for (int q = 0; q < 4; ++q) dma_piece(k, q);
  };
  float4 pre;
  auto fetch = [&](int64_t k) {
    int t2 = tid;
    asm volatile("" : "+v"(t2));
    pre = em_ld4(rx, (uint32_t)(k * 2048 + t2 * 4) * 4u);
  };
  auto stage = [&]() {
    int t2 = tid;
    asm volatile("" : "+v"(t2));
    const int e = t2 * 4, pl = e / D::PF, pix = e % D::PF;
    float *d = xp + pl * K::XP + (pix / S + 1) * K::RS + pix % S + 1;
    d[0] = pre.x; d[1] = pre.y; d[2] = pre.z; d[3] = pre.w;
  };
  auto convert = [&]() {
    int t2 = tid;
    asm volatile("" : "+v"(t2));
#pragma unroll
    for (int q = 0; q < 4; ++q) {
      const int e = (t2 + 512 * q) * 4;
      const float4 gv = *reinterpret_cast<const float4 *>(rawg + e), ov = *reinterpret_cast<const float4 *>(rawo + e);
      int ks, co, tg, a;
      if constexpr (S == 8) {
        const int c = e >> 8, y = (e >> 4) & 15, xx = e & 15;
        ks = y >> 2, co = 4 * c + 2 * (y & 1), tg = xx >> 2, a = (y >> 1) & 1;
      } else {
        const int f = e >> 11, c = (e >> 6) & 31, y = (e >> 3) & 7, xx = e & 7;
        ks = f, co = 4 * c + 2 * (y & 1), tg = 2 * (y >> 2) + (xx >> 2), a = (y >> 1) & 1;
      }
      float *d = gy4 + ((ks * 128 + co) * 4 + tg) * 4 + 2 * a;
      *reinterpret_cast<float2 *>(d) = make_float2(ov.x > 0.f ? gv.x : 0.f, ov.z > 0.f ? gv.z : 0.f);
      *reinterpret_cast<float2 *>(d + 16) = make_float2(ov.y > 0.f ? gv.y : 0.f, ov.w > 0.f ? gv.w : 0.f);
    }
  };
  auto transform = [&]() {
    int t2 = tid;
    asm volatile("" : "+v"(t2));
    const int l2 = t2 & 63, w2 = t2 >> 6, ks = w2 >> 1, ci = 16 * (w2 & 1) + (l2 & 15), tg = l2 >> 4;
    const int pb = S == 8 ? ci * K::XP + 2 * ks * K::RS + 2 * tg : (ks * 32 + ci) * K::XP + 2 * (tg >> 1) * K::RS + 2 * (tg & 1);
    float2 d[4][2];
    float v[16];
    wino_patch_load(xp + pb, K::RS, d);
    wino_patch_xform(d, v);
#pragma unroll
    for (int q = 0; q < 4; ++q)
      *reinterpret_cast<float4 *>(vt + t2 * K::VROW + 4 * q) = make_float4(v[4 * q], v[4 * q + 1], v[4 * q + 2], v[4 * q + 3]);
  };
  auto compute = [&](int64_t knext) {
#pragma unroll
    for (int ks = 0; ks < 4; ++ks) {
      const float4 t = *reinterpret_cast<const float4 *>(gy4 + ((ks * 128 + 16 * wv + j) * 4 + g) * 4);
      bsum += (t.x + t.y) + (t.z + t.w);
      float yh[16];
      {
        const float r0[2] = {t.x, t.y}, r1[2] = {t.x + t.z, t.y + t.w}, r2[2] = {t.x - t.z, t.y - t.w}, r3[2] = {-t.z, -t.w};
        const float *rr[4] = {r0, r1, r2, r3};
#pragma unroll
        for (int u = 0; u < 4; ++u) {
          yh[4 * u + 0] = rr[u][0];
          yh[4 * u + 1] = rr[u][0] + rr[u][1];
          yh[4 * u + 2] = rr[u][0] - rr[u][1];
          yh[4 * u + 3] = -rr[u][1];
        }
      }
#pragma unroll
      for (int nh = 0; nh < 2; ++nh) {
        float4 b[4];
#pragma unroll
        for (int q = 0; q < 4; ++q) b[q] = *reinterpret_cast<const float4 *>(vt + ((2 * ks + nh) * 64 + lane) * K::VROW + 4 * q);
#pragma unroll
        for (int q = 0; q < 4; ++q) {
          acc[4 * q + 0][nh] = WN_MFMA(yh[4 * q + 0], b[q].x, acc[4 * q + 0][nh]);
          acc[4 * q + 1][nh] = WN_MFMA(yh[4 * q + 1], b[q].y, acc[4 * q + 1][nh]);
          acc[4 * q + 2][nh] = WN_MFMA(yh[4 * q + 2], b[q].z, acc[4 * q + 2][nh]);
          acc[4 * q + 3][nh] = WN_MFMA(yh[4 * q + 3], b[q].w, acc[4 * q + 3][nh]);
        }
      }
      __builtin_amdgcn_sched_barrier(0);
      if (ks < 2) dma_piece(knext, 2 * ks), dma_piece(knext, 2 * ks + 1);
      __builtin_amdgcn_sched_barrier(0);
    }
  };

  int64_t k = blockIdx.x;
  dma(k);
  fetch(k);
  __syncthreads();
  stage();
  fetch(k + stride);
  __syncthreads();
  for (int slot = 0; k < nsets; k += stride, ++slot) {
    WN_STAMP(slot, 0);
    convert();
    WN_STAMP(slot, 1);
    transform();
    WN_STAMP(slot, 2);
    __syncthreads();
    WN_STAMP(slot, 3);
    stage();
    fetch(k + 2 * stride);
    compute(k + stride);
    WN_STAMP(slot, 4);
    __syncthreads();
    WN_STAMP(slot, 5);
  }
  float *wp = w_partials + (int64_t)blockIdx.x * UP_W;
#pragma unroll
  for (int nh = 0; nh < 2; ++nh)
#pragma unroll
    for (int r = 0; r < 4; ++r) {
      float t[3][4];
#pragma unroll
      for (int v = 0; v < 4; ++v) {
        const float z0 = acc[v][nh][r], z1 = acc[4 + v][nh][r], z2 = acc[8 + v][nh][r], z3 = acc[12 + v][nh][r];
        t[0][v] = z0 + 0.5f * (z1 + z2);
        t[1][v] = 0.5f * (z1 - z2);
        t[2][v] = 0.5f * (z1 + z2) + z3;
      }
      float *o = wp + ((16 * wv + 4 * g + r) * UP_CI + 16 * nh + j) * 9;
#pragma unroll
      for (int a = 0; a < 3; ++a) {
        o[3 * a + 0] = t[a][0] + 0.5f * (t[a][1] + t[a][2]);
        o[3 * a + 1] = 0.5f * (t[a][1] - t[a][2]);
        o[3 * a + 2] = 0.5f * (t[a][1] + t[a][2]) + t[a][3];
      }
    }
  bsum += __shfl_xor(bsum, 16);
  bsum += __shfl_xor(bsum, 32);
  if (g == 0) b_partials[(int64_t)blockIdx.x * UP_CO + 16 * wv + j] = bsum;
}

}
```

kalman-vae_amd/csrc/vae_loss.h:

```cpp
#pragma once
#include "lgssm_vm.h"

namespace kvae {

KV_DEV float bce_logit(float l, float x) { return fmaxf(l, 0.f) - l * x + log1pf(expf(-fabsf(l))); }
KV_DEV float sigmoid_stable(float l) {
  const float e = expf(-fabsf(l));
  return l >= 0.f ? 1.0f / (1.0f + e) : e / (1.0f + e);
}

}

#ifdef KVAE_HOSTSIM
#include <stdlib.h>
extern "C" {
int kvae_dec_head_loss_fwd(const float *in, const float *W, const float *bias, const float *x, float *logits, float *x_recon,
                           float *frame_ll, float *w_scratch, int64_t N, int32_t Cin, int32_t side, void *) {
  if (!in || !W || !bias || !x || !logits || !frame_ll || !w_scratch) return KVAE_ERR_NULL;
  if (N < 1) return KVAE_ERR_ARG;
  if (Cin != 32 || side != 16) return KVAE_ERR_DIMS;
  const int rc = kvae_dec_head_fwd(in, W, bias, logits, w_scratch, N, Cin, side, nullptr);
  if (rc) return rc;
  for (int64_t n = 0; n < N; ++n) {
    const float *l = logits + n * 1024, *t = x + n * 1024;
    float wave[4];
    for (int wv = 0; wv < 4; ++wv) {
      float lane[64];
      for (int j = 0; j < 64; ++j) {
        const int tid = wv * 64 + j, p = (2 * (tid >> 4)) * 32 + 2 * (tid & 15);
        lane[j] = (kvae::bce_logit(l[p], t[p]) + kvae::bce_logit(l[p + 1], t[p + 1])) +
                  (kvae::bce_logit(l[p + 32], t[p + 32]) + kvae::bce_logit(l[p + 33], t[p + 33]));
      }
      for (int off = 32; off > 0; off >>= 1)
        for (int j = 0; j < off; ++j) lane[j] += lane[j + off];
      wave[wv] = lane[0];
    }
    frame_ll[n] = -((wave[0] + wave[1]) + (wave[2] + wave[3]));
    if (x_recon)
      for (int p = 0; p < 1024; ++p) x_recon[n * 1024 + p] = kvae::sigmoid_stable(l[p]);
  }
  return KVAE_OK;
}
int kvae_dec_head_loss_bwd(const float *in, const float *W, const float *logits, const float *x, const float *g_frame,
                           float *g_in, float *w_partials, float *b_partials, float *w_scratch, int64_t N, int32_t Cin,
                           int32_t side, void *) {
  if (!in || !W || !logits || !x || !g_frame || !w_partials || !b_partials || !w_scratch) return KVAE_ERR_NULL;
  if (N < 1) return KVAE_ERR_ARG;
  if (Cin != 32 || side != 16) return KVAE_ERR_DIMS;
  float *g = static_cast<float *>(malloc(sizeof(float) * N * 1024));
  if (!g) return KVAE_ERR_ARG;
  int rc = kvae_bce_frames_bwd(logits, x, g_frame, g, N, 1024, nullptr);
  if (!rc) rc = kvae_dec_head_bwd(in, W, g, g_in, w_partials, b_partials, w_scratch, N, Cin, side, nullptr);
  free(g);
  return rc;
}
}
#endif
```

kalman-vae_amd/kvae/_native.py:

```python
import ctypes as C
import os
from pathlib import Path

import torch

_HERE = Path(__file__).resolve().parent
LIB_PATH = _HERE / "lib" / "libkvae_lgssm.so"

KVAE_MAX_DIM = 16
KVAE_MAX_K = 16
LSTM_MAX_H, LSTM_MAX_I = 52, 16
ABI_VERSION = 20

_STATUS = {1: "KVAE_ERR_DIMS (n, m, p must be in [1,16]; B, T >= 1)", 2: "KVAE_ERR_NULL", 3: "KVAE_ERR_LAUNCH",
           4: "KVAE_ERR_ARG"}


class Stack(C.Structure):
    _fields_ = [("ptr", C.c_void_p), ("sb", C.c_int64), ("st", C.c_int64)]


class Problem(C.Structure):
    _fields_ = [("B", C.c_int32), ("T", C.c_int32), ("n", C.c_int32), ("m", C.c_int32), ("p", C.c_int32),
                ("A", Stack), ("Bm", Stack), ("C", Stack), ("Q", Stack),
                ("R", C.c_void_p), ("mu0", C.c_void_p), ("mu0_sb", C.c_int64),
                ("Sigma0", C.c_void_p), ("Sigma0_sb", C.c_int64),
                ("Y", C.c_void_p), ("U", C.c_void_p), ("mask", C.c_void_p)]


class States(C.Structure):
    _fields_ = [(k, C.c_void_p) for k in ("mus_filt", "Sigmas_filt", "mus_pred", "Sigmas_pred",
                                          "mus_smooth", "Sigmas_smooth", "aux")]


class WgradProblem(C.Structure):
    _fields_ = [("d", C.c_void_p), ("h", C.c_void_p), ("x", C.c_void_p), ("g_wh", C.c_void_p), ("g_wx", C.c_void_p),
                ("g_b", C.c_void_p), ("d_stride", C.c_int64), ("h_stride", C.c_int64), ("x_stride", C.c_int64), ("N", C.c_int64),
                ("R", C.c_int32), ("H", C.c_int32), ("I", C.c_int32), ("bias", C.c_int32), ("T", C.c_int32), ("shift", C.c_int32)]


class GenProblem(C.Structure):
    _fields_ = ([(k, C.c_int32) for k in ("B", "S", "H", "n", "m", "p", "K", "kind", "hidden")]
                + [(k, C.c_void_p) for k in ("A", "Bm", "C", "LQ", "LR", "mu", "L0", "U", "w_ih", "w_hh", "b_ih", "b_hh",
                                             "head_w", "head_b", "h0", "c0", "y0", "P", "s0", "eps0", "eps_z", "eps_a",
                                             "gumbel", "a_out", "z_out", "w_out")])


class PsampleProblem(C.Structure):
    _fields_ = ([(k, C.c_int32) for k in ("B", "S", "T", "n", "p", "stages")]
                + [(k, C.c_void_p) for k in ("mus_filt", "Sigmas_filt", "mus_pred", "Sigmas_pred")]
                + [("A", Stack), ("C", Stack), ("Q", Stack)]
                + [(k, C.c_void_p) for k in ("LR", "eps", "eta", "z_out", "a_out", "levels_out", "ws")])


class PredProblem(C.Structure):
    _fields_ = ([(k, C.c_int32) for k in ("B", "T", "n", "p")]
                + [(k, C.c_void_p) for k in ("mus_pred", "Sigmas_pred")] + [("C", Stack)]
                + [(k, C.c_void_p) for k in ("R", "y", "mask", "ll", "nis", "a_pred", "S_out", "levels", "seq_ll")])


class PredGrads(C.Structure):
    _fields_ = [(k, C.c_void_p) for k in ("g_ll", "g_seq", "g_mus_pred", "g_Sigmas_pred", "gY")] + [("gC", Stack)]


class SwfProblem(C.Structure):
    _fields_ = ([(k, C.c_int32) for k in ("B", "T", "K", "n", "m", "p")]
                + [(k, C.c_void_p) for k in ("A", "Bm", "Q", "C", "R", "P", "mu0", "Sigma0", "y", "u", "mask", "state_log_w", "state_mu",
                                             "state_Sigma", "regime_filt", "regime_pred", "ll", "seq_ll", "a_pred", "S_out", "mus_filt",
                                             "Sigmas_filt", "levels", "out_log_w", "out_mu", "out_Sigma")])


class SwsProblem(C.Structure):
    _fields_ = [("filt", SwfProblem)] + [(k, C.c_void_p) for k in ("hist_mu", "hist_Sigma", "hist_W", "hist_w", "regime_smooth",
                                                                  "regime_pairs", "mus_smooth", "Sigmas_smooth")]


class SwmProblem(C.Structure):
    _fields_ = [("filt", SwfProblem)] + [(k, C.c_void_p) for k in ("hist_lw", "hist_mu", "hist_Sigma")]


class SwmGrads(C.Structure):
    _fields_ = [(k, C.c_void_p) for k in ("g_ll", "g_seq", "ws", "gA", "gB", "gQ", "gC", "g_logP", "g_mu0", "g_Sigma0", "gY", "gU",
                                         "ll_recomputed")]


class EmStats(C.Structure):
    _fields_ = [(k, C.c_void_p) for k in ("ws", "N", "S11", "S10", "S00", "counts", "Syz", "Szz", "Syy", "Nobs", "z0", "z0z0", "nseq")]


class InputGrads(C.Structure):
    _fields_ = [("gA", Stack), ("gB", Stack), ("gC", Stack), ("gQ", Stack),
                ("gY", C.c_void_p), ("gU", C.c_void_p), ("g_mu0", C.c_void_p), ("g_Sigma0", C.c_void_p)]


SYMBOLS = (
    "kvae_lgssm_filter_alpha_lstm", "kvae_lgssm_alpha_lstm_bwd", "kvae_lgssm_filter_fwd", "kvae_lgssm_rts_fwd",
    "kvae_lgssm_smooth_fwd", "kvae_lgssm_smooth_bwd", "kvae_lgssm_elbo", "kvae_mix_fwd", "kvae_mix_bwd",
    "kvae_mix_bwd_partials", "kvae_lstm_fwd", "kvae_lstm_bwd", "kvae_bias_shuffle_act_fwd",
    "kvae_bias_shuffle_act_bwd", "kvae_bias_partial_rows", "kvae_colsum", "kvae_colsum2", "kvae_clip_adam",
    "kvae_regime_fwd", "kvae_regime_bwd", "kvae_regime_decode", "kvae_regime_decode_ws_bytes", "kvae_bigru_fwd",
    "kvae_bigru_bwd", "kvae_bce_frames_fwd", "kvae_bce_frames_bwd", "kvae_dec_head_fwd", "kvae_dec_head_bwd",
    "kvae_dec_head_loss_fwd", "kvae_dec_head_loss_bwd",
    "kvae_enc_stem_fwd", "kvae_enc_stem_bwd", "kvae_conv_edge_partial_rows", "kvae_enc_mid_fwd", "kvae_enc_mid_bwd",
    "kvae_enc_mid_partial_rows", "kvae_dec_up_fwd", "kvae_dec_up_bwd", "kvae_dec_up_partial_rows",
    "kvae_dec_up_set_workgroups", "kvae_enc_head_fwd", "kvae_enc_head_bwd", "kvae_dec_fc_fwd", "kvae_dec_fc_bwd",
    "kvae_head_partial_rows", "kvae_latent_reg_fwd", "kvae_latent_reg_bwd", "kvae_loss_head_fwd",
    "kvae_loss_head_bwd", "kvae_lgssm_emission_means", "kvae_lgssm_generate", "kvae_lgssm_posterior_sample",
    "kvae_lgssm_posterior_sample_ws_floats", "kvae_lgssm_predictive", "kvae_lgssm_predictive_bwd",
    "kvae_lgssm_switching_filter", "kvae_lgssm_switching_smoother", "kvae_lgssm_switching_marginal",
    "kvae_lgssm_switching_marginal_bwd", "kvae_lgssm_switching_marginal_ws_floats", "kvae_lgssm_switching_em",
    "kvae_lgssm_switching_em_ws_floats", "kvae_rnn_wgrad", "kvae_rnn_wgrad_ws_floats", "kvae_linear_fwd",
    "kvae_linear_bwd_input", "kvae_abi_version", "kvae_last_error", "kvae_build_info",
)


class LgssmLib:

    def __init__(self, path):
        self.path = str(path)
        self.dll = C.CDLL(self.path)
        missing = [s for s in SYMBOLS if not hasattr(self.dll, s)]
        if missing:
            raise OSError(f"{self.path} does not export {missing}")
        d = self.dll
        P, S, G, vp = C.POINTER(Problem), C.POINTER(States), C.POINTER(InputGrads), C.c_void_p
        for name in ("kvae_lgssm_filter_fwd", "kvae_lgssm_rts_fwd", "kvae_lgssm_smooth_fwd"):
            getattr(d, name).argtypes = [P, S, vp]
            getattr(d, name).restype = C.c_int
        d.kvae_lgssm_filter_alpha_lstm.argtypes = [P, S] + [vp] * 9 + [C.c_int32, C.c_int32] + [vp] * 7
        d.kvae_lgssm_filter_alpha_lstm.restype = C.c_int
        d.kvae_lgssm_alpha_lstm_bwd.argtypes = [P, S, S, G, vp, C.c_int] + [vp] * 6 + [C.c_int32, C.c_int32] + [vp] * 9
        d.kvae_lgssm_alpha_lstm_bwd.restype = C.c_int
        d.kvae_lgssm_generate.argtypes = [C.POINTER(GenProblem), vp]
        d.kvae_lgssm_generate.restype = C.c_int
        d.kvae_lgssm_posterior_sample.argtypes = [C.POINTER(PsampleProblem), vp]
        d.kvae_lgssm_posterior_sample.restype = C.c_int
        d.kvae_lgssm_posterior_sample_ws_floats.argtypes = [C.POINTER(PsampleProblem)]
        d.kvae_lgssm_posterior_sample_ws_floats.restype = C.c_int64
        d.kvae_lgssm_predictive.argtypes = [C.POINTER(PredProblem), vp]
        d.kvae_lgssm_predictive.restype = C.c_int
        d.kvae_lgssm_predictive_bwd.argtypes = [C.POINTER(PredProblem), C.POINTER(PredGrads), vp]
        d.kvae_lgssm_predictive_bwd.restype = C.c_int
        d.kvae_lgssm_switching_filter.argtypes = [C.POINTER(SwfProblem), vp]
        d.kvae_lgssm_switching_filter.restype = C.c_int
        d.kvae_lgssm_switching_smoother.argtypes = [C.POINTER(SwsProblem), vp]
        d.kvae_lgssm_switching_smoother.restype = C.c_int
        d.kvae_lgssm_switching_marginal.argtypes = [C.POINTER(SwmProblem), vp]
        d.kvae_lgssm_switching_marginal.restype = C.c_int
        d.kvae_lgssm_switching_marginal_bwd.argtypes = [C.POINTER(SwmProblem), C.POINTER(SwmGrads), vp]
        d.kvae_lgssm_switching_marginal_bwd.restype = C.c_int
        d.kvae_lgssm_switching_marginal_ws_floats.argtypes = [C.c_int32] * 4
        d.kvae_lgssm_switching_marginal_ws_floats.restype = C.c_int64
        d.kvae_lgssm_switching_em.argtypes = [C.POINTER(SwsProblem), C.POINTER(EmStats), vp]
        d.kvae_lgssm_switching_em.restype = C.c_int
        d.kvae_lgssm_switching_em_ws_floats.argtypes = [C.c_int32] * 4
        d.kvae_lgssm_switching_em_ws_floats.restype = C.c_int64
        d.kvae_lgssm_smooth_bwd.argtypes = [P, S, S, G, vp, C.c_int, vp]
        d.kvae_lgssm_smooth_bwd.restype = C.c_int
        d.kvae_lgssm_elbo.argtypes = [P, vp, vp, vp, vp, vp, vp, vp, vp, G, vp]
        d.kvae_lgssm_elbo.restype = C.c_int
        d.kvae_mix_fwd.argtypes = [vp, vp, vp, C.c_int64, C.c_int32, C.c_int32, vp]
        d.kvae_mix_fwd.restype = C.c_int
        d.kvae_mix_bwd.argtypes = [vp, vp, vp, vp, vp, vp, C.c_int64, C.c_int32, C.c_int32, C.c_int32, vp]
        d.kvae_mix_bwd.restype = C.c_int
        d.kvae_mix_bwd_partials.argtypes = [C.c_int64]
        d.kvae_mix_bwd_partials.restype = C.c_int64
        d.kvae_lstm_fwd.argtypes = [vp] * 8 + [C.c_int32] * 4 + [vp]
        d.kvae_lstm_fwd.restype = C.c_int
        d.kvae_lstm_bwd.argtypes = [vp] * 7 + [C.c_int32] * 4 + [vp]
        d.kvae_lstm_bwd.restype = C.c_int
        d.kvae_bias_shuffle_act_fwd.argtypes = [vp, vp, vp, C.c_int64] + [C.c_int32] * 5 + [vp]
        d.kvae_bias_shuffle_act_fwd.restype = C.c_int
        d.kvae_bias_shuffle_act_bwd.argtypes = [vp, vp, vp, vp, C.c_int64] + [C.c_int32] * 5 + [vp]
        d.kvae_bias_shuffle_act_bwd.restype = C.c_int
        d.kvae_regime_fwd.argtypes = [vp] * 7 + [C.c_int32] * 3 + [C.c_float, vp, C.c_int32, vp]
        d.kvae_regime_fwd.restype = C.c_int
        d.kvae_regime_bwd.argtypes = [vp] * 10 + [C.c_int32] * 3 + [C.c_float, vp, vp]
        d.kvae_regime_bwd.restype = C.c_int
        d.kvae_regime_decode.argtypes = [vp] * 8 + [C.c_int32] * 3 + [vp]
        d.kvae_regime_decode.restype = C.c_int
        d.kvae_regime_decode_ws_bytes.argtypes = [C.c_int64, C.c_int32, C.c_int32]
        d.kvae_regime_decode_ws_bytes.restype = C.c_int64
        d.kvae_bigru_fwd.argtypes = [vp] * 7 + [C.c_int32] * 4 + [vp]
        d.kvae_bigru_fwd.restype = C.c_int
        d.kvae_bigru_bwd.argtypes = [vp] * 8 + [C.c_int32] * 4 + [vp]
        d.kvae_bigru_bwd.restype = C.c_int
        d.kvae_bce_frames_fwd.argtypes = [vp, vp, vp, C.c_int64, C.c_int32, vp]
        d.kvae_bce_frames_fwd.restype = C.c_int
        d.kvae_bce_frames_bwd.argtypes = [vp, vp, vp, vp, C.c_int64, C.c_int32, vp]
        d.kvae_bce_frames_bwd.restype = C.c_int
        d.kvae_dec_head_fwd.argtypes = [vp, vp, vp, vp, vp, C.c_int64, C.c_int32, C.c_int32, vp]
        d.kvae_dec_head_fwd.restype = C.c_int
        d.kvae_dec_head_bwd.argtypes = [vp] * 7 + [C.c_int64, C.c_int32, C.c_int32, vp]
        d.kvae_dec_head_bwd.restype = C.c_int
        d.kvae_dec_head_loss_fwd.argtypes = [vp] * 8 + [C.c_int64, C.c_int32, C.c_int32, vp]
        d.kvae_dec_head_loss_fwd.restype = C.c_int
        d.kvae_dec_head_loss_bwd.argtypes = [vp] * 9 + [C.c_int64, C.c_int32, C.c_int32, vp]
        d.kvae_dec_head_loss_bwd.restype = C.c_int
        d.kvae_enc_stem_fwd.argtypes = [vp, vp, vp, vp, vp, C.c_int64, C.c_int32, C.c_int32, vp]
        d.kvae_enc_stem_fwd.restype = C.c_int
        d.kvae_enc_stem_bwd.argtypes = [vp] * 6 + [C.c_int64, C.c_int32, C.c_int32, vp]
        d.kvae_enc_stem_bwd.restype = C.c_int
        d.kvae_enc_mid_fwd.argtypes = [vp, vp, vp, vp, C.c_int64, C.c_int32, C.c_int32, vp]
        d.kvae_enc_mid_fwd.restype = C.c_int
        d.kvae_enc_mid_bwd.argtypes = [vp] * 7 + [C.c_int64, C.c_int32, C.c_int32, vp]
        d.kvae_enc_mid_bwd.restype = C.c_int
        d.kvae_enc_mid_partial_rows.argtypes = [C.c_int64, C.c_int32]
        d.kvae_dec_up_fwd.argtypes = [vp, vp, vp, vp, C.c_int64, C.c_int32, C.c_int32, vp]
        d.kvae_dec_up_fwd.restype = C.c_int
        d.kvae_dec_up_bwd.argtypes = [vp] * 7 + [C.c_int64, C.c_int32, C.c_int32, vp]
        d.kvae_dec_up_bwd.restype = C.c_int
        d.kvae_dec_up_partial_rows.argtypes = [C.c_int64, C.c_int32]
        d.kvae_enc_head_fwd.argtypes = [vp] * 9 + [C.c_int64, C.c_int32, C.c_int32, C.c_float, vp]
        d.kvae_enc_head_fwd.restype = C.c_int
        d.kvae_enc_head_bwd.argtypes = [vp] * 11 + [C.c_int64, C.c_int32, C.c_int32, C.c_float, vp]
        d.kvae_enc_head_bwd.restype = C.c_int
        d.kvae_dec_fc_fwd.argtypes = [vp] * 4 + [C.c_int64, C.c_int32, C.c_int32, vp]
        d.kvae_dec_fc_fwd.restype = C.c_int
        d.kvae_dec_fc_bwd.argtypes = [vp] * 6 + [C.c_int64, C.c_int32, C.c_int32, vp]
        d.kvae_dec_fc_bwd.restype = C.c_int
        d.kvae_head_partial_rows.argtypes = []
        d.kvae_head_partial_rows.restype = C.c_int64
        d.kvae_latent_reg_fwd.argtypes = [vp] * 4 + [C.c_int64, C.c_int32, vp]
        d.kvae_latent_reg_fwd.restype = C.c_int
        d.kvae_latent_reg_bwd.argtypes = [vp] * 7 + [C.c_int64, C.c_int32, vp]
        d.kvae_latent_reg_bwd.restype = C.c_int
        d.kvae_loss_head_fwd.argtypes = [vp] * 5 + [C.c_float] * 3 + [vp, vp, vp, C.c_int64, vp]
        d.kvae_loss_head_fwd.restype = C.c_int
        d.kvae_loss_head_bwd.argtypes = [vp, vp, vp, vp, vp, vp, C.c_int64, vp]
        d.kvae_loss_head_bwd.restype = C.c_int
        d.kvae_dec_up_partial_rows.restype = C.c_int64
        d.kvae_dec_up_set_workgroups.argtypes = [C.c_int32]
        d.kvae_dec_up_set_workgroups.restype = C.c_int32
        d.kvae_enc_mid_partial_rows.restype = C.c_int64
        d.kvae_conv_edge_partial_rows.argtypes = [C.c_int64]
        d.kvae_conv_edge_partial_rows.restype = C.c_int64
        d.kvae_colsum.argtypes = [vp, vp, C.c_int64, C.c_int64, vp]
        d.kvae_colsum.restype = C.c_int
        d.kvae_colsum2.argtypes = [vp, vp, C.c_int64, C.c_int64, vp, vp, C.c_int64, C.c_int64, vp]
        d.kvae_colsum2.restype = C.c_int
        d.kvae_lgssm_emission_means.argtypes = [P, vp, vp, vp, vp, vp]
        d.kvae_lgssm_emission_means.restype = C.c_int
        d.kvae_rnn_wgrad_ws_floats.argtypes = [C.POINTER(WgradProblem), C.c_int32]
        d.kvae_rnn_wgrad_ws_floats.restype = C.c_int64
        d.kvae_rnn_wgrad.argtypes = [C.POINTER(WgradProblem), C.c_int32, vp, vp]
        d.kvae_rnn_wgrad.restype = C.c_int
        d.kvae_linear_fwd.argtypes = [vp, C.c_int64, C.c_int64, C.c_int32, vp, vp, C.c_int32, C.c_int32, vp, vp]
        d.kvae_linear_fwd.restype = C.c_int
        d.kvae_linear_bwd_input.argtypes = [vp, vp, C.c_int64, C.c_int32, vp, C.c_int32, vp, vp, C.c_int64, vp]
        d.kvae_linear_bwd_input.restype = C.c_int
        d.kvae_clip_adam.argtypes = [vp, vp, vp, vp, C.c_int64, vp, C.c_int32, vp, vp, vp, C.c_float, C.c_float, C.c_float, C.c_float,
                                     C.c_float, C.c_float, vp, vp, vp, vp]
        d.kvae_clip_adam.restype = C.c_int
        d.kvae_bias_partial_rows.argtypes = [C.c_int64]
        d.kvae_bias_partial_rows.restype = C.c_int64
        d.kvae_abi_version.restype = C.c_int
        d.kvae_last_error.restype = C.c_char_p
        d.kvae_build_info.restype = C.c_char_p
        if d.kvae_abi_version() != ABI_VERSION:
            raise OSError(f"{self.path}: ABI {d.kvae_abi_version()} != expected {ABI_VERSION}")

    def check(self, rc, what):
        if rc != 0:
            detail = self.dll.kvae_last_error().decode() if rc == 3 else ""
            raise RuntimeError(f"{what} failed: {_STATUS.get(rc, rc)} {detail}")

    @property
    def build_info(self):
        return self.dll.kvae_build_info().decode()


_hip_lib = None
_test_backend = None


def hip_lib():
    global _hip_lib
    if _hip_lib is None:
        if not LIB_PATH.exists():
            raise RuntimeError(
                f"HIP library {LIB_PATH} is missing. Build it with `python __graft_entry__.py build` "
                "(hipcc --offload-arch=gfx950). There is no CPU fallback for the LGSSM path.")
        _hip_lib = LgssmLib(LIB_PATH)
    return _hip_lib


def _set_test_backend(lib):
    global _test_backend
    _test_backend = lib


def fused_ok(t: torch.Tensor) -> bool:
    return t.is_cuda or _test_backend is not None


def lib_for(t: torch.Tensor):
    if t.is_cuda:
        return hip_lib()
    if _test_backend is not None:
        return _test_backend
    raise RuntimeError(
        "kvae LGSSM ops run only on a HIP device (MI355X): got a CPU tensor and there is no CPU fallback. "
        "Move the model and inputs to 'cuda'.")


def stream_for(t: torch.Tensor):
    if t.is_cuda:
        return C.c_void_p(torch.cuda.current_stream(t.device).cuda_stream)
    return C.c_void_p(0)


def ptr(t):
    return C.c_void_p(t.data_ptr()) if t is not None else C.c_void_p(0)


_prof = None


def profile_start():
    global _prof
    _prof = {}


def profile_stop():
    global _prof
    rec, _prof = _prof, None
    torch.cuda.synchronize()
    return {k: [s.elapsed_time(e) for s, e in v] for k, v in (rec or {}).items()}


def timed(name, t, thunk):
    if _prof is None or not t.is_cuda:
        return thunk()
    s, e = torch.cuda.Event(enable_timing=True), torch.cuda.Event(enable_timing=True)
    s.record()
    rc = thunk()
    e.record()
    _prof.setdefault(name, []).append((s, e))
    return rc


def _colsum_raw(p2):
    out = torch.empty(p2.shape[1], device=p2.device, dtype=torch.float32)
    lib = lib_for(p2)
    lib.check(lib.dll.kvae_colsum(ptr(p2), ptr(out), p2.shape[0], p2.shape[1], stream_for(p2)), "kvae_colsum")
    return out


def colsum_pair(a, b):
    a2, b2 = a.reshape(a.shape[0], -1).contiguous(), b.reshape(b.shape[0], -1).contiguous()
    tall = [p.shape[0] >= 1024 and p.shape[1] < 4096 for p in (a2, b2)]
    if a2.device != b2.device or tall[0] != tall[1] or (tall[0] and (a2.shape[0] != b2.shape[0] or a2.shape[0] % 64)):
        return colsum(a), colsum(b)

    def pair(x, y):
        ox = torch.empty(x.shape[1], device=x.device, dtype=torch.float32)
        oy = torch.empty(y.shape[1], device=y.device, dtype=torch.float32)
        lib = lib_for(x)
        lib.check(lib.dll.kvae_colsum2(ptr(x), ptr(ox), x.shape[0], x.shape[1], ptr(y), ptr(oy), y.shape[0], y.shape[1],
                                       stream_for(x)), "kvae_colsum2")
        return ox, oy

    if tall[0]:
        rows = a2.shape[0]
        fa, fb = pair(a2.view(64, (rows // 64) * a2.shape[1]), b2.view(64, (rows // 64) * b2.shape[1]))
        a2, b2 = fa.view(rows // 64, a2.shape[1]), fb.view(rows // 64, b2.shape[1])
    oa, ob = pair(a2, b2)
    return oa.view(a.shape[1:]), ob.view(b.shape[1:])


def colsum(partials):
    p2 = partials.reshape(partials.shape[0], -1).contiguous()
    rows, cols = p2.shape
    if rows >= 1024 and cols < 4096:
        r1 = 64
        while r1 > 1 and rows % r1:
            r1 //= 2
        if r1 > 1:
            p2 = _colsum_raw(p2.view(r1, (rows // r1) * cols)).view(rows // r1, cols)
    return _colsum_raw(p2).view(partials.shape[1:])
```

kalman-vae_amd/kvae/vae/fused.py:

```python
import torch

from .. import _native as N


colsum = N.colsum
colsum_pair = N.colsum_pair


def _chunks(n, size):
    return [(a, min(a + size, n)) for a in range(0, n, size)]


def _acc(total, part):
    return part if total is None else total + part


class BiasShuffleAct(torch.autograd.Function):

    @staticmethod
    def forward(ctx, x, bias, r, relu):
        x = x.contiguous()
        bias = bias.contiguous()
        Nb, Crr, H, W = x.shape
        C = Crr // (r * r)
        out = torch.empty(Nb, C, H * r, W * r, device=x.device, dtype=torch.float32)
        lib = N.lib_for(x)
        lib.check(lib.dll.kvae_bias_shuffle_act_fwd(N.ptr(x), N.ptr(bias), N.ptr(out), Nb, C, H, W, r, int(relu),
                                                    N.stream_for(x)), "kvae_bias_shuffle_act_fwd")
        ctx.r, ctx.relu, ctx.shape = r, relu, (Nb, C, H, W)
        ctx.save_for_backward(out if relu else None)
        return out

    @staticmethod
    def backward(ctx, g):
        (out,) = ctx.saved_tensors
        Nb, C, H, W = ctx.shape
        g = g.contiguous()
        g_in = torch.empty(Nb, C * ctx.r * ctx.r, H, W, device=g.device, dtype=torch.float32)
        lib = N.lib_for(g)
        partials = torch.empty(lib.dll.kvae_bias_partial_rows(Nb), C * ctx.r * ctx.r, device=g.device, dtype=torch.float32)
        lib.check(lib.dll.kvae_bias_shuffle_act_bwd(N.ptr(g), N.ptr(out), N.ptr(g_in), N.ptr(partials), Nb, C, H, W, ctx.r,
                                                    int(ctx.relu), N.stream_for(g)), "kvae_bias_shuffle_act_bwd")
        return g_in, colsum(partials), None, None


def conv_block(x, conv, r=1, relu=True):
    y = torch.nn.functional.conv2d(x, conv.weight, None, conv.stride, conv.padding, conv.dilation, conv.groups)
    return BiasShuffleAct.apply(y, conv.bias, r, relu)


class DecoderHead(torch.autograd.Function):

    SCRATCH = 2304

    @staticmethod
    def supported(h, conv):
        return (h.dim() == 4 and tuple(h.shape[1:]) == (32, 16, 16) and tuple(conv.weight.shape) == (4, 32, 3, 3)
                and conv.stride == (1, 1) and conv.padding == (1, 1) and conv.dilation == (1, 1) and conv.groups == 1
                and conv.bias is not None)

    @staticmethod
    def forward(ctx, h, weight, bias):
        h, weight, bias = h.contiguous(), weight.contiguous(), bias.contiguous()
        Nb, Cin, s, _ = h.shape
        logits = torch.empty(Nb, 1, 2 * s, 2 * s, device=h.device, dtype=torch.float32)
        scratch = torch.empty(DecoderHead.SCRATCH, device=h.device, dtype=torch.float32)
        lib = N.lib_for(h)
        lib.check(lib.dll.kvae_dec_head_fwd(N.ptr(h), N.ptr(weight), N.ptr(bias), N.ptr(logits), N.ptr(scratch), Nb, Cin, s,
                                            N.stream_for(h)), "kvae_dec_head_fwd")
        ctx.save_for_backward(h, weight)
        return logits

    @staticmethod
    def backward(ctx, g):
        h, weight = ctx.saved_tensors
        g = g.contiguous()
        Nb, Cin, s, _ = h.shape
        lib = N.lib_for(h)
        rows = lib.dll.kvae_conv_edge_partial_rows(Nb)
        g_h = torch.empty_like(h) if ctx.needs_input_grad[0] else None
        wp = torch.empty(rows, weight.numel(), device=h.device, dtype=torch.float32)
        bp = torch.empty(rows, 4, device=h.device, dtype=torch.float32)
        scratch = torch.empty(DecoderHead.SCRATCH, device=h.device, dtype=torch.float32)
        lib.check(lib.dll.kvae_dec_head_bwd(N.ptr(h), N.ptr(weight), N.ptr(g), N.ptr(g_h) if g_h is not None else None,
                                            N.ptr(wp), N.ptr(bp), N.ptr(scratch), Nb, Cin, s, N.stream_for(h)),
                  "kvae_dec_head_bwd")
        gw, gb = colsum_pair(wp, bp)
        return g_h, gw.view_as(weight), gb


class DecoderHeadBernoulli(torch.autograd.Function):

    @staticmethod
    def forward(ctx, h, weight, bias, x, *with_recon):
        ctx.n_opt = len(with_recon)
        with_recon = with_recon[0] if with_recon else True
        h, weight, bias, x = h.contiguous(), weight.contiguous(), bias.contiguous(), x.contiguous()
        Nb, Cin, s, _ = h.shape
        logits = torch.empty(Nb, 1, 2 * s, 2 * s, device=h.device, dtype=torch.float32)
        x_recon = torch.empty_like(logits) if with_recon else None
        frame_ll = torch.empty(Nb, device=h.device, dtype=torch.float32)
        scratch = torch.empty(DecoderHead.SCRATCH, device=h.device, dtype=torch.float32)
        lib = N.lib_for(h)
        lib.check(lib.dll.kvae_dec_head_loss_fwd(N.ptr(h), N.ptr(weight), N.ptr(bias), N.ptr(x), N.ptr(logits), _optr(x_recon),
                                                 N.ptr(frame_ll), N.ptr(scratch), Nb, Cin, s, N.stream_for(h)),
                  "kvae_dec_head_loss_fwd")
        ctx.save_for_backward(h, weight, logits, x)
        ctx.set_materialize_grads(False)
        if x_recon is not None:
            ctx.mark_non_differentiable(x_recon)
        return logits, x_recon, frame_ll

    @staticmethod
    def backward(ctx, g_logits, _g_recon, g_ll):
        if g_logits is None and g_ll is None:
            return (None,) * (4 + ctx.n_opt)
        h, weight, logits, x = ctx.saved_tensors
        Nb, Cin, s, _ = h.shape
        lib = N.lib_for(h)
        rows = lib.dll.kvae_conv_edge_partial_rows(Nb)
        g_h = torch.empty_like(h) if ctx.needs_input_grad[0] else None
        wp = torch.empty(rows, weight.numel(), device=h.device, dtype=torch.float32)
        bp = torch.empty(rows, 4, device=h.device, dtype=torch.float32)
        scratch = torch.empty(DecoderHead.SCRATCH, device=h.device, dtype=torch.float32)
        if g_logits is None:
            g_ll = g_ll.contiguous()
            lib.check(lib.dll.kvae_dec_head_loss_bwd(N.ptr(h), N.ptr(weight), N.ptr(logits), N.ptr(x), N.ptr(g_ll), _optr(g_h),
                                                     N.ptr(wp), N.ptr(bp), N.ptr(scratch), Nb, Cin, s, N.stream_for(h)),
                      "kvae_dec_head_loss_bwd")
        else:
            g = g_logits.contiguous()
            if g_ll is not None:
                gl = torch.empty_like(logits)
                lib.check(lib.dll.kvae_bce_frames_bwd(N.ptr(logits), N.ptr(x), N.ptr(g_ll.contiguous()), N.ptr(gl), Nb,
                                                      logits.numel() // Nb, N.stream_for(h)), "kvae_bce_frames_bwd")
                g = gl + g
            lib.check(lib.dll.kvae_dec_head_bwd(N.ptr(h), N.ptr(weight), N.ptr(g), _optr(g_h), N.ptr(wp), N.ptr(bp),
                                                N.ptr(scratch), Nb, Cin, s, N.stream_for(h)), "kvae_dec_head_bwd")
        gw, gb = colsum_pair(wp, bp)
        return (g_h, gw.view_as(weight), gb, None) + (None,) * ctx.n_opt


class EncoderStem(torch.autograd.Function):

    @staticmethod
    def supported(x, conv):
        return (x.dim() == 4 and tuple(x.shape[1:]) == (1, 32, 32) and tuple(conv.weight.shape) == (32, 1, 3, 3)
                and conv.stride == (2, 2) and conv.padding == (1, 1) and conv.dilation == (1, 1) and conv.groups == 1
                and conv.bias is not None and not x.requires_grad)

    @staticmethod
    def forward(ctx, x, weight, bias):
        x, weight, bias = x.contiguous(), weight.contiguous(), bias.contiguous()
        Nb, _, s, _ = x.shape
        Cout = weight.shape[0]
        out = torch.empty(Nb, Cout, s // 2, s // 2, device=x.device, dtype=torch.float32)
        lib = N.lib_for(x)
        bits = torch.empty(Nb, (s // 2) ** 2, device=x.device, dtype=torch.int32) if (x.is_cuda and Cout == 32) else None
        lib.check(lib.dll.kvae_enc_stem_fwd(N.ptr(x), N.ptr(weight), N.ptr(bias), N.ptr(out), N.ptr(bits) if bits is not None else None,
                                            Nb, Cout, s, N.stream_for(x)), "kvae_enc_stem_fwd")
        ctx.save_for_backward(x, out, bits)
        ctx.wshape = weight.shape
        return out

    @staticmethod
    def backward(ctx, g):
        x, out, bits = ctx.saved_tensors
        g = g.contiguous()
        Nb, Cout = out.shape[:2]
        lib = N.lib_for(x)
        rows = lib.dll.kvae_conv_edge_partial_rows(Nb)
        wp = torch.empty(rows, Cout * 9, device=x.device, dtype=torch.float32)
        bp = torch.empty(rows, Cout, device=x.device, dtype=torch.float32)
        lib.check(lib.dll.kvae_enc_stem_bwd(N.ptr(x), N.ptr(out), N.ptr(bits) if bits is not None else None, N.ptr(g), N.ptr(wp),
                                            N.ptr(bp), Nb, Cout, x.shape[2], N.stream_for(x)), "kvae_enc_stem_bwd")
        gw, gb = colsum_pair(wp, bp)
        return None, gw.view(ctx.wshape), gb


class EncoderMid(torch.autograd.Function):

    @staticmethod
    def supported(x, conv):
        return (x.dim() == 4 and x.shape[1] == 32 and x.shape[2] == x.shape[3] and x.shape[2] in (16, 8)
                and tuple(conv.weight.shape) == (32, 32, 3, 3) and conv.stride == (2, 2) and conv.padding == (1, 1)
                and conv.dilation == (1, 1) and conv.groups == 1 and conv.bias is not None)

    CHUNK = 16384

    @staticmethod
    def forward(ctx, x, weight, bias):
        x, weight, bias = x.contiguous(), weight.contiguous(), bias.contiguous()
        Nb, Cc, s, _ = x.shape
        out = torch.empty(Nb, Cc, s // 2, s // 2, device=x.device, dtype=torch.float32)
        lib = N.lib_for(x)
        for a, b in _chunks(Nb, EncoderMid.CHUNK):
            lib.check(N.timed(f"enc_mid_fwd_s{s}", x, lambda: lib.dll.kvae_enc_mid_fwd(
                N.ptr(x[a:b]), N.ptr(weight), N.ptr(bias), N.ptr(out[a:b]), b - a, Cc, s, N.stream_for(x))), "kvae_enc_mid_fwd")
        ctx.save_for_backward(x, weight, out)
        return out

    @staticmethod
    def backward(ctx, g):
        x, weight, out = ctx.saved_tensors
        g = g.contiguous()
        Nb, Cc, s, _ = x.shape
        lib = N.lib_for(x)
        g_x = torch.empty_like(x) if ctx.needs_input_grad[0] else None
        gw = gb = None
        for a, b in _chunks(Nb, EncoderMid.CHUNK):
            rows = lib.dll.kvae_enc_mid_partial_rows(b - a, s)
            wp = torch.empty(rows, weight.numel(), device=x.device, dtype=torch.float32)
            bp = torch.empty(rows, Cc, device=x.device, dtype=torch.float32)
            lib.check(lib.dll.kvae_enc_mid_bwd(N.ptr(x[a:b]), N.ptr(weight), N.ptr(out[a:b]), N.ptr(g[a:b]),
                                               N.ptr(g_x[a:b]) if g_x is not None else None, N.ptr(wp), N.ptr(bp), b - a, Cc, s,
                                               N.stream_for(x)), "kvae_enc_mid_bwd")
            cw, cb = colsum_pair(wp, bp)
            gw, gb = _acc(gw, cw), _acc(gb, cb)
        return g_x, gw.view_as(weight), gb


class DecoderUp(torch.autograd.Function):

    CHUNK = 16384

    @staticmethod
    def supported(x, conv):
        return (x.dim() == 4 and x.shape[1] == 32 and x.shape[2] == x.shape[3] and x.shape[2] in (8, 4)
                and tuple(conv.weight.shape) == (128, 32, 3, 3) and conv.stride == (1, 1) and conv.padding == (1, 1)
                and conv.dilation == (1, 1) and conv.groups == 1 and conv.bias is not None)

    @staticmethod
    def forward(ctx, x, weight, bias):
        x, weight, bias = x.contiguous(), weight.contiguous(), bias.contiguous()
        Nb, Cin, s, _ = x.shape
        out = torch.empty(Nb, 32, 2 * s, 2 * s, device=x.device, dtype=torch.float32)
        lib = N.lib_for(x)
        for a, b in _chunks(Nb, DecoderUp.CHUNK):
            lib.check(N.timed(f"dec_up_fwd_s{s}", x, lambda: lib.dll.kvae_dec_up_fwd(
                N.ptr(x[a:b]), N.ptr(weight), N.ptr(bias), N.ptr(out[a:b]), b - a, Cin, s, N.stream_for(x))), "kvae_dec_up_fwd")
        ctx.save_for_backward(x, weight, out)
        return out

    @staticmethod
    def backward(ctx, g):
        x, weight, out = ctx.saved_tensors
        g = g.contiguous()
        Nb, Cin, s, _ = x.shape
        lib = N.lib_for(x)
        g_x = torch.empty_like(x) if ctx.needs_input_grad[0] else None
        gw = gb = None
        for a, b in _chunks(Nb, DecoderUp.CHUNK):
            rows = lib.dll.kvae_dec_up_partial_rows(b - a, s)
            wp = torch.empty(rows, weight.numel(), device=x.device, dtype=torch.float32)
            bp = torch.empty(rows, 128, device=x.device, dtype=torch.float32)
            lib.check(N.timed(f"dec_up_bwd_s{s}", x, lambda: lib.dll.kvae_dec_up_bwd(
                N.ptr(x[a:b]), N.ptr(weight), N.ptr(out[a:b]), N.ptr(g[a:b]), N.ptr(g_x[a:b]) if g_x is not None else None, N.ptr(wp),
                N.ptr(bp), b - a, Cin, s, N.stream_for(x))), "kvae_dec_up_bwd")
            cw, cb = colsum_pair(wp, bp)
            gw, gb = _acc(gw, cw), _acc(gb, cb)
        return g_x, gw.view_as(weight), gb


def _optr(t):
    return N.ptr(t) if t is not None else None


class EncoderHead(torch.autograd.Function):

    @staticmethod
    def supported(feat, fc_mu, fc_var_lin):
        return (feat.dim() == 2 and feat.shape[1] == 512 and tuple(fc_mu.weight.shape) == (2, 512)
                and tuple(fc_var_lin.weight.shape) == (2, 512) and fc_mu.bias is not None and fc_var_lin.bias is not None)

    @staticmethod
    def forward(ctx, feat, w_mu, b_mu, w_var, b_var, eps, ne):
        feat, w_mu, b_mu, w_var, b_var = (t.contiguous() for t in (feat, w_mu, b_mu, w_var, b_var))
        eps = eps.contiguous() if eps is not None else None
        Nb = feat.shape[0]
        mu, var, a = (torch.empty(Nb, 2, device=feat.device, dtype=torch.float32) for _ in range(3))
        lib = N.lib_for(feat)
        lib.check(lib.dll.kvae_enc_head_fwd(N.ptr(feat), N.ptr(w_mu), N.ptr(b_mu), N.ptr(w_var), N.ptr(b_var), _optr(eps),
                                            N.ptr(mu), N.ptr(var), N.ptr(a), Nb, 512, 2, float(ne), N.stream_for(feat)),
                  "kvae_enc_head_fwd")
        ctx.save_for_backward(feat, w_mu, w_var, var, eps)
        ctx.ne = float(ne)
        return a, mu, var

    @staticmethod
    def backward(ctx, g_a, g_mu, g_var):
        feat, w_mu, w_var, var, eps = ctx.saved_tensors
        g_a, g_mu, g_var = (t.contiguous() if t is not None else None for t in (g_a, g_mu, g_var))
        Nb = feat.shape[0]
        lib = N.lib_for(feat)
        rows = lib.dll.kvae_head_partial_rows()
        g_feat = torch.empty_like(feat)
        wp = torch.empty(rows, 4 * 512, device=feat.device, dtype=torch.float32)
        bp = torch.empty(rows, 4, device=feat.device, dtype=torch.float32)
        lib.check(lib.dll.kvae_enc_head_bwd(N.ptr(feat), N.ptr(w_mu), N.ptr(w_var), N.ptr(var), _optr(eps), _optr(g_a), _optr(g_mu),
                                            _optr(g_var), N.ptr(g_feat), N.ptr(wp), N.ptr(bp), Nb, 512, 2, ctx.ne,
                                            N.stream_for(feat)), "kvae_enc_head_bwd")
        gw, gb = colsum_pair(wp, bp)
        gw, gb = gw.view(2, 2, 512), gb.view(2, 2)
        return g_feat, gw[0], gb[0], gw[1], gb[1], None, None


class DecoderFc(torch.autograd.Function):

    @staticmethod
    def supported(a, fc):
        return a.dim() == 2 and a.shape[1] == 2 and tuple(fc.weight.shape) == (512, 2) and fc.bias is not None

    @staticmethod
    def forward(ctx, a, weight, bias):
        a, weight, bias = a.contiguous(), weight.contiguous(), bias.contiguous()
        Nb = a.shape[0]
        h = torch.empty(Nb, 512, device=a.device, dtype=torch.float32)
        lib = N.lib_for(a)
        lib.check(lib.dll.kvae_dec_fc_fwd(N.ptr(a), N.ptr(weight), N.ptr(bias), N.ptr(h), Nb, 512, 2, N.stream_for(a)),
                  "kvae_dec_fc_fwd")
        ctx.save_for_backward(a, weight)
        return h

    @staticmethod
    def backward(ctx, g):
        a, weight = ctx.saved_tensors
        g = g.contiguous()
        Nb = a.shape[0]
        lib = N.lib_for(a)
        rows = lib.dll.kvae_head_partial_rows()
        g_a = torch.empty_like(a)
        wp = torch.empty(rows, 1024, device=a.device, dtype=torch.float32)
        bp = torch.empty(rows, 512, device=a.device, dtype=torch.float32)
        lib.check(lib.dll.kvae_dec_fc_bwd(N.ptr(g), N.ptr(a), N.ptr(weight), N.ptr(g_a), N.ptr(wp), N.ptr(bp), Nb, 512, 2,
                                          N.stream_for(a)), "kvae_dec_fc_bwd")
        gw, gb = colsum_pair(wp, bp)
        return g_a, gw.view(512, 2), gb


class LatentReg(torch.autograd.Function):

    @staticmethod
    def forward(ctx, a, mu, var):
        a, mu, var = a.contiguous(), mu.contiguous(), var.contiguous()
        A = a.shape[-1]
        Nb = a.numel() // A
        reg = torch.empty(a.shape[:-1], device=a.device, dtype=torch.float32)
        lib = N.lib_for(a)
        lib.check(lib.dll.kvae_latent_reg_fwd(N.ptr(a), N.ptr(mu), N.ptr(var), N.ptr(reg), Nb, A, N.stream_for(a)),
                  "kvae_latent_reg_fwd")
        ctx.save_for_backward(a, mu, var)
        return reg

    @staticmethod
    def backward(ctx, g):
        a, mu, var = ctx.saved_tensors
        g = g.contiguous()
        A = a.shape[-1]
        g_a, g_mu, g_var = torch.empty_like(a), torch.empty_like(a), torch.empty_like(a)
        lib = N.lib_for(a)
        lib.check(lib.dll.kvae_latent_reg_bwd(N.ptr(a), N.ptr(mu), N.ptr(var), N.ptr(g), N.ptr(g_a), N.ptr(g_mu), N.ptr(g_var),
                                              a.numel() // A, A, N.stream_for(a)), "kvae_latent_reg_bwd")
        return g_a, g_mu, g_var


class LossHead(torch.autograd.Function):

    @staticmethod
    def forward(ctx, lpx, regf, elbo_kf, mask, beta, scale, vae_w, kf_w, weights=None):
        lpx, regf = lpx.contiguous(), regf.contiguous()
        mask = mask.contiguous() if mask is not None else None
        kf = elbo_kf.reshape(1).contiguous()
        b = beta.reshape(1).to(device=lpx.device, dtype=torch.float32).contiguous() if torch.is_tensor(beta) else \
            torch.full((1,), float(beta), device=lpx.device, dtype=torch.float32)
        out, coef = torch.empty(6, device=lpx.device, dtype=torch.float32), torch.empty(3, device=lpx.device, dtype=torch.float32)
        lib = N.lib_for(lpx)
        lib.check(lib.dll.kvae_loss_head_fwd(N.ptr(lpx), N.ptr(regf), _optr(mask), N.ptr(kf), N.ptr(b), float(scale), float(vae_w),
                                             float(kf_w), _optr(weights), N.ptr(out), N.ptr(coef), lpx.numel(), N.stream_for(lpx)),
                  "kvae_loss_head_fwd")
        ctx.save_for_backward(coef, mask)
        ctx.set_materialize_grads(False)
        ctx.shape, ctx.kf_shape = lpx.shape, elbo_kf.shape
        vals = out.unbind(0)
        ctx.mark_non_differentiable(*vals[1:])
        return vals

    @staticmethod
    def backward(ctx, g_loss, *_unused):
        if g_loss is None:
            return (None,) * 9
        coef, mask = ctx.saved_tensors
        g = g_loss.reshape(1).contiguous()
        g_lpx = torch.empty(ctx.shape, device=g.device, dtype=torch.float32)
        g_reg = torch.empty(ctx.shape, device=g.device, dtype=torch.float32)
        g_kf = torch.empty(1, device=g.device, dtype=torch.float32)
        lib = N.lib_for(g)
        lib.check(lib.dll.kvae_loss_head_bwd(N.ptr(g), N.ptr(coef), _optr(mask), N.ptr(g_lpx), N.ptr(g_reg), N.ptr(g_kf),
                                             g_lpx.numel(), N.stream_for(g)), "kvae_loss_head_bwd")
        return g_lpx, g_reg, g_kf.reshape(ctx.kf_shape), None, None, None, None, None, None


class BernoulliFrameLogLik(torch.autograd.Function):

    @staticmethod
    def forward(ctx, x_logits, x):
        lg, xx = x_logits.contiguous(), x.contiguous()
        lead = lg.shape[:2]
        frames = lead[0] * lead[1]
        pixels = lg.numel() // frames
        out = torch.empty(lead, device=lg.device, dtype=torch.float32)
        lib = N.lib_for(lg)
        lib.check(lib.dll.kvae_bce_frames_fwd(N.ptr(lg), N.ptr(xx), N.ptr(out), frames, pixels, N.stream_for(lg)),
                  "kvae_bce_frames_fwd")
        ctx.save_for_backward(lg, xx)
        return out

    @staticmethod
    def backward(ctx, g):
        lg, xx = ctx.saved_tensors
        g = g.contiguous()
        frames = g.numel()
        g_logits = torch.empty_like(lg)
        lib = N.lib_for(lg)
        lib.check(lib.dll.kvae_bce_frames_bwd(N.ptr(lg), N.ptr(xx), N.ptr(g), N.ptr(g_logits), frames, lg.numel() // frames,
                                              N.stream_for(lg)), "kvae_bce_frames_bwd")
        return g_logits, None
```

kalman-vae_amd/kvae/vae/vae.py:

```python
import os
from typing import Tuple

import torch
import torch.nn as nn

from kvae import _native
from kvae.utils.config import KVAEConfig
from kvae.vae.fused import DecoderFc, DecoderHead, DecoderHeadBernoulli, DecoderUp, EncoderHead, EncoderMid, EncoderStem, conv_block


def _conv_out(size, k, s, p):
    return (size + 2 * p - k) // s + 1


class Encoder(nn.Module):

    def __init__(self, config: KVAEConfig):
        super().__init__()
        self.config = config
        blocks, c_in, side = [], config.img_channels, config.img_size
        for c_out in config.encoder_channels:
            blocks += [nn.Conv2d(c_in, c_out, config.encoder_kernel_size, config.encoder_stride,
                                 config.encoder_padding), nn.ReLU()]
            side = _conv_out(side, config.encoder_kernel_size, config.encoder_stride, config.encoder_padding)
            c_in = c_out
        self.conv_layers = nn.Sequential(*blocks)
        self.flat_size = c_in * side * side
        self.fc_mu = nn.Linear(self.flat_size, config.a_dim)
        self.fc_var = nn.Sequential(nn.Linear(self.flat_size, config.a_dim), nn.Sigmoid())

    def features(self, x: torch.Tensor) -> torch.Tensor:
        if _native.fused_ok(x) and x.dtype == torch.float32:
            h = x
            for i, layer in enumerate(self.conv_layers):
                if isinstance(layer, nn.Conv2d):
                    if i == 0 and EncoderStem.supported(h, layer):
                        h = EncoderStem.apply(h, layer.weight, layer.bias)
                    elif EncoderMid.supported(h, layer):
                        h = EncoderMid.apply(h, layer.weight, layer.bias)
                    else:
                        h = conv_block(h, layer, r=1, relu=True)
            return h.flatten(1)
        return self.conv_layers(x).flatten(1)

    def heads(self, feat: torch.Tensor, eps=None):
        if _native.fused_ok(feat) and feat.dtype == torch.float32 and EncoderHead.supported(feat, self.fc_mu, self.fc_var[0]):
            return EncoderHead.apply(feat, self.fc_mu.weight, self.fc_mu.bias, self.fc_var[0].weight, self.fc_var[0].bias,
                                     eps, self.config.noise_emission)
        mu, var = self.fc_mu(feat), self.config.noise_emission * self.fc_var(feat)
        return (mu if eps is None else mu + eps * torch.sqrt(var + 1e-6)), mu, var

    def forward(self, x: torch.Tensor) -> Tuple[torch.Tensor, torch.Tensor]:
        _, mu, var = self.heads(self.features(x))
        return mu, var


class Decoder(nn.Module):

    def __init__(self, config: KVAEConfig):
        super().__init__()
        self.config = config
        chans = list(config.decoder_channels)
        self.init_size = config.img_size // (2 ** len(chans))
        self.init_channels = chans[0]
        self.fc = nn.Linear(config.a_dim, self.init_channels * self.init_size ** 2)
        up = []
        for c_in, c_out in zip(chans[:-1], chans[1:]):
            up += [nn.Conv2d(c_in, 4 * c_out, kernel_size=3, padding=1), nn.PixelShuffle(2), nn.ReLU()]
        up += [nn.Conv2d(chans[-1], 4 * config.img_channels, kernel_size=3, padding=1), nn.PixelShuffle(2)]
        self.deconv_layers = nn.Sequential(*up)

    def head_loss_supported(self, h: torch.Tensor, conv: nn.Conv2d, x: torch.Tensor) -> bool:
        return (DecoderHead.supported(h, conv) and self.config.out_distr.lower() == "bernoulli" and h.dtype == torch.float32
                and x.dtype == torch.float32 and not x.requires_grad and x.device == h.device
                and tuple(x.shape) == (h.shape[0], 1, 2 * h.shape[2], 2 * h.shape[3]))

    def _decode(self, a: torch.Tensor, x=None, with_recon=True):
        fused = _native.fused_ok(a) and a.dtype == torch.float32
        h = DecoderFc.apply(a, self.fc.weight, self.fc.bias) if fused and DecoderFc.supported(a, self.fc) else self.fc(a)
        h = h.unflatten(1, (self.init_channels, self.init_size, self.init_size))
        if not fused:
            return self.deconv_layers(h), None, None
        layers = list(self.deconv_layers)
        for i, layer in enumerate(layers):
            if isinstance(layer, nn.Conv2d):
                relu = i + 2 < len(layers) and isinstance(layers[i + 2], nn.ReLU)
                if not relu and x is not None and i + 2 == len(layers) and self.head_loss_supported(h, layer, x):
                    return DecoderHeadBernoulli.apply(h, layer.weight, layer.bias, x, with_recon)
                if not relu and DecoderHead.supported(h, layer):
                    h = DecoderHead.apply(h, layer.weight, layer.bias)
                elif relu and DecoderUp.supported(h, layer):
                    h = DecoderUp.apply(h, layer.weight, layer.bias)
                else:
                    h = conv_block(h, layer, r=2, relu=relu)
        return h, None, None

    def forward(self, a: torch.Tensor) -> torch.Tensor:
        return self._decode(a)[0]

    def forward_with_frames(self, a: torch.Tensor, x: torch.Tensor, with_recon=True):
        return self._decode(a, x, with_recon)


class VAE(nn.Module):

    def __init__(self, config: KVAEConfig):
        super().__init__()
        self.config = config
        self.encoder = Encoder(config)
        self.decoder = Decoder(config)

    def encode(self, x):
        return self.encoder(x)

    def decode(self, a):
        return self.decoder(a)

    def reparameterize(self, mu, var):
        return mu + torch.randn_like(var) * var.sqrt()

    def forward(self, x: torch.Tensor) -> dict:
        lead = x.shape[:2]
        mu, var = self.encode(x.flatten(0, 1))
        a = self.reparameterize(mu, var)
        x_mu = self.decode(a)
        x_rec = torch.sigmoid(x_mu) if self.config.out_distr.lower() == "bernoulli" else x_mu
        back = lambda t: t.unflatten(0, lead)
        return {"x_recon": back(x_rec), "x_recon_mu": back(x_mu),
                "x_recon_var": torch.tensor(self.config.noise_pixel_var, device=x.device, dtype=x_mu.dtype),
                "a_vae": back(a), "a_mu": back(mu), "a_var": back(var)}

    def sample_from_prior(self, n: int = 1, device=None) -> torch.Tensor:
        device = device or next(self.parameters()).device
        return self.decode(torch.randn(n, self.config.a_dim, device=device))

    @classmethod
    def load_from_checkpoint(cls, checkpoint_path: str, config: KVAEConfig = None, device: str = "cpu"):
        if not os.path.exists(checkpoint_path):
            raise FileNotFoundError(checkpoint_path)
        vae = cls(config or KVAEConfig())
        payload = torch.load(checkpoint_path, map_location=device, weights_only=True)
        for key in ("state_dict", "model_state"):
            if isinstance(payload, dict) and key in payload:
                payload = payload[key]
        for part in ("encoder", "decoder"):
            sub = {k.split(part + ".", 1)[1]: v for k, v in payload.items() if (part + ".") in k}
            if sub:
                getattr(vae, part).load_state_dict(sub)
        return vae.to(device)
```

Before: 97030 sequences/s.

## Fuse ReLU backward masking into producer kernels of decoder upsample gradients

```diff
diff --git a/include/kvae_lgssm.h b/include/kvae_lgssm.h
--- a/include/kvae_lgssm.h
+++ b/include/kvae_lgssm.h
@@ -8,7 +8,7 @@
 #endif
 
 #define KVAE_MAX_DIM 16
-#define KVAE_ABI_VERSION 20
+#define KVAE_ABI_VERSION 21
 
 typedef enum {
   KVAE_OK = 0,
@@ -178,6 +178,11 @@
 int kvae_dec_head_loss_bwd(const float *in, const float *W, const float *logits, const float *x, const float *g_frame, float *g_in,
                            float *w_partials, float *b_partials, float *w_scratch, int64_t N, int32_t Cin, int32_t side,
                            void *stream);
+int kvae_dec_head_bwd_masked(const float *in, const float *W, const float *g_logits, float *g_in, float *w_partials,
+                             float *b_partials, float *w_scratch, int64_t N, int32_t Cin, int32_t side, void *stream);
+int kvae_dec_head_loss_bwd_masked(const float *in, const float *W, const float *logits, const float *x, const float *g_frame,
+                                  float *g_in, float *w_partials, float *b_partials, float *w_scratch, int64_t N, int32_t Cin,
+                                  int32_t side, void *stream);
 int kvae_enc_stem_fwd(const float *x, const float *W, const float *bias, float *out, uint32_t *relu_bits, int64_t N, int32_t Cout,
                       int32_t side, void *stream);
 int kvae_enc_stem_bwd(const float *x, const float *out, const uint32_t *relu_bits, const float *g_out, float *w_partials,
@@ -194,6 +199,10 @@
                     void *stream);
 int kvae_dec_up_bwd(const float *x, const float *W, const float *out, const float *g_out, float *g_x, float *w_partials,
                     float *b_partials, int64_t N, int32_t Cin, int32_t side, void *stream);
+#define KVAE_UP_G_PREMASKED 1
+#define KVAE_UP_MASK_GX 2
+int kvae_dec_up_bwd_flags(const float *x, const float *W, const float *out, const float *g_out, float *g_x, float *w_partials,
+                          float *b_partials, int64_t N, int32_t Cin, int32_t side, int32_t flags, void *stream);
 int64_t kvae_dec_up_partial_rows(int64_t N, int32_t side);
 int32_t kvae_dec_up_set_workgroups(int32_t n);
 
diff --git a/kalman-vae_amd/csrc/kvae_vae.hip b/kalman-vae_amd/csrc/kvae_vae.hip
--- a/kalman-vae_amd/csrc/kvae_vae.hip
+++ b/kalman-vae_amd/csrc/kvae_vae.hip
@@ -385,11 +385,14 @@
 template <bool LOSS>
 static int dec_head_bwd_launch(const float *in, const float *W, const float *g_logits, const float *logits, const float *x,
                                const float *g_frame, float *g_in, float *w_partials, float *b_partials, float *w_scratch,
-                               int64_t N, hipStream_t st) {
+                               int64_t N, bool mask, hipStream_t st) {
   const dim3 grid((unsigned)kvae_conv_edge_partial_rows(N));
   if (g_in) {
     k_dec_head_prep<<<dim3(1), dim3(256), 0, st>>>(W, w_scratch);
-    k_dec_head_bwd<LOSS, true><<<grid, dim3(256), 0, st>>>(in, g_logits, logits, x, g_frame, w_scratch, g_in, w_partials, b_partials, N);
+    if (mask)
+      k_dec_head_bwd<LOSS, true, true><<<grid, dim3(256), 0, st>>>(in, g_logits, logits, x, g_frame, w_scratch, g_in, w_partials, b_partials, N);
+    else
+      k_dec_head_bwd<LOSS, true><<<grid, dim3(256), 0, st>>>(in, g_logits, logits, x, g_frame, w_scratch, g_in, w_partials, b_partials, N);
   } else {
     k_dec_head_bwd<LOSS, false><<<grid, dim3(256), 0, st>>>(in, g_logits, logits, x, g_frame, w_scratch, g_in, w_partials, b_partials, N);
   }
@@ -401,7 +404,7 @@
   if (!in || !W || !g_logits || !w_partials || !b_partials || !w_scratch) return KVAE_ERR_NULL;
   if (N < 1) return KVAE_ERR_ARG;
   if (Cin != DH_CI || side != DH_S) return KVAE_ERR_DIMS;
-  return dec_head_bwd_launch<false>(in, W, g_logits, nullptr, nullptr, nullptr, g_in, w_partials, b_partials, w_scratch, N,
+  return dec_head_bwd_launch<false>(in, W, g_logits, nullptr, nullptr, nullptr, g_in, w_partials, b_partials, w_scratch, N, false,
                                     (hipStream_t)stream);
 }
 int kvae_dec_head_loss_bwd(const float *in, const float *W, const float *logits, const float *x, const float *g_frame, float *g_in,
@@ -410,7 +413,24 @@
   if (!in || !W || !logits || !x || !g_frame || !w_partials || !b_partials || !w_scratch) return KVAE_ERR_NULL;
   if (N < 1) return KVAE_ERR_ARG;
   if (Cin != DH_CI || side != DH_S) return KVAE_ERR_DIMS;
-  return dec_head_bwd_launch<true>(in, W, nullptr, logits, x, g_frame, g_in, w_partials, b_partials, w_scratch, N,
+  return dec_head_bwd_launch<true>(in, W, nullptr, logits, x, g_frame, g_in, w_partials, b_partials, w_scratch, N, false,
+                                   (hipStream_t)stream);
+}
+int kvae_dec_head_bwd_masked(const float *in, const float *W, const float *g_logits, float *g_in, float *w_partials,
+                             float *b_partials, float *w_scratch, int64_t N, int32_t Cin, int32_t side, void *stream) {
+  if (!in || !W || !g_logits || !w_partials || !b_partials || !w_scratch) return KVAE_ERR_NULL;
+  if (N < 1) return KVAE_ERR_ARG;
+  if (Cin != DH_CI || side != DH_S) return KVAE_ERR_DIMS;
+  return dec_head_bwd_launch<false>(in, W, g_logits, nullptr, nullptr, nullptr, g_in, w_partials, b_partials, w_scratch, N, true,
+                                    (hipStream_t)stream);
+}
+int kvae_dec_head_loss_bwd_masked(const float *in, const float *W, const float *logits, const float *x, const float *g_frame,
+                                  float *g_in, float *w_partials, float *b_partials, float *w_scratch, int64_t N, int32_t Cin,
+                                  int32_t side, void *stream) {
+  if (!in || !W || !logits || !x || !g_frame || !w_partials || !b_partials || !w_scratch) return KVAE_ERR_NULL;
+  if (N < 1) return KVAE_ERR_ARG;
+  if (Cin != DH_CI || side != DH_S) return KVAE_ERR_DIMS;
+  return dec_head_bwd_launch<true>(in, W, nullptr, logits, x, g_frame, g_in, w_partials, b_partials, w_scratch, N, true,
                                    (hipStream_t)stream);
 }
 int kvae_enc_stem_fwd(const float *x, const float *W, const float *bias, float *out, uint32_t *relu_bits, int64_t N, int32_t Cout,
@@ -512,30 +532,67 @@
   else k_dec_up_fwd<4><<<grid, dim3(256), 0, (hipStream_t)stream>>>(x, W, bias, out, N);
   return launch_status("k_dec_up_fwd");
 }
+}
+__global__ __launch_bounds__(256) void k_relu_mask_inplace(float *__restrict__ g, const float *__restrict__ act, int64_t quads) {
+  for (int64_t q = (int64_t)blockIdx.x * 256 + threadIdx.x; q < quads; q += (int64_t)gridDim.x * 256) {
+    const float4 a = reinterpret_cast<const float4 *>(act)[q];
+    float4 v = reinterpret_cast<float4 *>(g)[q];
+    v = make_float4(a.x > 0.f ? v.x : 0.f, a.y > 0.f ? v.y : 0.f, a.z > 0.f ? v.z : 0.f, a.w > 0.f ? v.w : 0.f);
+    reinterpret_cast<float4 *>(g)[q] = v;
+  }
+}
+static int dec_up_bwd_launch(const float *x, const float *W, const float *out, const float *g_out, float *g_x, float *w_partials,
+                             float *b_partials, int64_t N, int32_t side, int32_t flags, hipStream_t st) {
+  const dim3 grid((unsigned)dec_up_grid(N, side));
+  const bool pre = (flags & KVAE_UP_G_PREMASKED) != 0, wino = dec_up_wino();
+  if (g_x) {
+    const int64_t sets = side == 8 ? N : (N + 3) / 4;
+    const dim3 wgrid((unsigned)(sets < dec_up_cap() ? sets : dec_up_cap()));
+    bool mask_gx = (flags & KVAE_UP_MASK_GX) != 0;
+    if (wino && side == 8 && pre && mask_gx) {
+      k_dec_up_bwd_data_wino<8, true, true><<<wgrid, dim3(512), 0, st>>>(W, x, out, g_out, g_x, N);
+      mask_gx = false;
+    } else if (wino && side == 8 && pre) k_dec_up_bwd_data_wino<8, true><<<wgrid, dim3(512), 0, st>>>(W, x, out, g_out, g_x, N);
+    else if (wino && side == 8) k_dec_up_bwd_data_wino<8><<<wgrid, dim3(512), 0, st>>>(W, x, out, g_out, g_x, N);
+    else if (wino && pre) k_dec_up_bwd_data_wino<4, true><<<wgrid, dim3(512), 0, st>>>(W, x, out, g_out, g_x, N);
+    else if (wino) k_dec_up_bwd_data_wino<4><<<wgrid, dim3(512), 0, st>>>(W, x, out, g_out, g_x, N);
+    else if (side == 8) k_dec_up_bwd_data<8><<<grid, dim3(256), 0, st>>>(W, out, g_out, g_x, N);
+    else k_dec_up_bwd_data<4><<<grid, dim3(256), 0, st>>>(W, out, g_out, g_x, N);
+    int rc = launch_status("k_dec_up_bwd_data");
+    if (rc) return rc;
+    if (mask_gx) {
+      const int64_t quads = N * UP_CI * side * side / 4;
+      k_relu_mask_inplace<<<dim3(epi_grid(quads)), dim3(256), 0, st>>>(g_x, x, quads);
+      rc = launch_status("k_relu_mask_inplace");
+      if (rc) return rc;
+    }
+  }
+  if (wino) {
+    if (side == 8 && pre) k_dec_up_wrw_wino<8, true><<<grid, dim3(512), 0, st>>>(x, out, g_out, w_partials, b_partials, N);
+    else if (side == 8) k_dec_up_wrw_wino<8><<<grid, dim3(512), 0, st>>>(x, out, g_out, w_partials, b_partials, N);
+    else if (pre) k_dec_up_wrw_wino<4, true><<<grid, dim3(512), 0, st>>>(x, out, g_out, w_partials, b_partials, N);
+    else k_dec_up_wrw_wino<4><<<grid, dim3(512), 0, st>>>(x, out, g_out, w_partials, b_partials, N);
+    return launch_status("k_dec_up_wrw_wino");
+  }
+  if (side == 8) k_dec_up_wrw<8><<<grid, dim3(256), 0, st>>>(x, out, g_out, w_partials, b_partials, N);
+  else k_dec_up_wrw<4><<<grid, dim3(256), 0, st>>>(x, out, g_out, w_partials, b_partials, N);
+  return launch_status("k_dec_up_wrw");
+}
+extern "C" {
 int kvae_dec_up_bwd(const float *x, const float *W, const float *out, const float *g_out, float *g_x, float *w_partials,
                     float *b_partials, int64_t N, int32_t Cin, int32_t side, void *stream) {
   if (!x || !W || !out || !g_out || !w_partials || !b_partials) return KVAE_ERR_NULL;
   if (N < 1 || (N + 256 * 8) * UP_CO * side * side * 4 >= EM_MAX_BYTES) return KVAE_ERR_ARG;
   if (Cin != UP_CI || (side != 8 && side != 4)) return KVAE_ERR_DIMS;
-  const dim3 grid((unsigned)dec_up_grid(N, side));
-  if (g_x) {
-    const int64_t sets = side == 8 ? N : (N + 3) / 4;
-    const dim3 wgrid((unsigned)(sets < dec_up_cap() ? sets : dec_up_cap()));
-    if (dec_up_wino() && side == 8) k_dec_up_bwd_data_wino<8><<<wgrid, dim3(512), 0, (hipStream_t)stream>>>(W, out, g_out, g_x, N);
-    else if (dec_up_wino()) k_dec_up_bwd_data_wino<4><<<wgrid, dim3(512), 0, (hipStream_t)stream>>>(W, out, g_out, g_x, N);
-    else if (side == 8) k_dec_up_bwd_data<8><<<grid, dim3(256), 0, (hipStream_t)stream>>>(W, out, g_out, g_x, N);
-    else k_dec_up_bwd_data<4><<<grid, dim3(256), 0, (hipStream_t)stream>>>(W, out, g_out, g_x, N);
-    const int rc = launch_status("k_dec_up_bwd_data");
-    if (rc) return rc;
-  }
-  if (dec_up_wino()) {
-    if (side == 8) k_dec_up_wrw_wino<8><<<grid, dim3(512), 0, (hipStream_t)stream>>>(x, out, g_out, w_partials, b_partials, N);
-    else k_dec_up_wrw_wino<4><<<grid, dim3(512), 0, (hipStream_t)stream>>>(x, out, g_out, w_partials, b_partials, N);
-    return launch_status("k_dec_up_wrw_wino");
-  }
-  if (side == 8) k_dec_up_wrw<8><<<grid, dim3(256), 0, (hipStream_t)stream>>>(x, out, g_out, w_partials, b_partials, N);
-  else k_dec_up_wrw<4><<<grid, dim3(256), 0, (hipStream_t)stream>>>(x, out, g_out, w_partials, b_partials, N);
-  return launch_status("k_dec_up_wrw");
+  return dec_up_bwd_launch(x, W, out, g_out, g_x, w_partials, b_partials, N, side, 0, (hipStream_t)stream);
+}
+int kvae_dec_up_bwd_flags(const float *x, const float *W, const float *out, const float *g_out, float *g_x, float *w_partials,
+                          float *b_partials, int64_t N, int32_t Cin, int32_t side, int32_t flags, void *stream) {
+  if (!x || !W || !out || !g_out || !w_partials || !b_partials) return KVAE_ERR_NULL;
+  if (N < 1 || (N + 256 * 8) * UP_CO * side * side * 4 >= EM_MAX_BYTES) return KVAE_ERR_ARG;
+  if (flags & ~(KVAE_UP_G_PREMASKED | KVAE_UP_MASK_GX)) return KVAE_ERR_ARG;
+  if (Cin != UP_CI || (side != 8 && side != 4)) return KVAE_ERR_DIMS;
+  return dec_up_bwd_launch(x, W, out, g_out, g_x, w_partials, b_partials, N, side, flags, (hipStream_t)stream);
 }
 }
 
diff --git a/kalman-vae_amd/csrc/vae_conv_edge.h b/kalman-vae_amd/csrc/vae_conv_edge.h
--- a/kalman-vae_amd/csrc/vae_conv_edge.h
+++ b/kalman-vae_amd/csrc/vae_conv_edge.h
@@ -96,7 +96,7 @@
   }
 }
 
-template <bool LOSS, bool DATA>
+template <bool LOSS, bool DATA, bool MASK = false>
 __global__ __launch_bounds__(256, 2) void k_dec_head_bwd(const float *__restrict__ in, const float *__restrict__ g_logits,
                                                          const float *__restrict__ logits, const float *__restrict__ x,
                                                          const float *__restrict__ g_frame, const float *__restrict__ scratch,
@@ -206,8 +206,13 @@
       float *o = g_in + n * DH_CI * 256 + threadIdx.x;
 #pragma unroll
       for (int j = 0; j < DH_CI / 2; ++j) {
-        o[(2 * j) * 256] = dacc[j].x;
-        o[(2 * j + 1) * 256] = dacc[j].y;
+        if constexpr (MASK) {
+          o[(2 * j) * 256] = tile[(2 * j) * CS + threadIdx.x] > 0.f ? dacc[j].x : 0.f;
+          o[(2 * j + 1) * 256] = tile[(2 * j + 1) * CS + threadIdx.x] > 0.f ? dacc[j].y : 0.f;
+        } else {
+          o[(2 * j) * 256] = dacc[j].x;
+          o[(2 * j + 1) * 256] = dacc[j].y;
+        }
       }
     }
   }
diff --git a/kalman-vae_amd/csrc/vae_conv_up_wino.h b/kalman-vae_amd/csrc/vae_conv_up_wino.h
--- a/kalman-vae_amd/csrc/vae_conv_up_wino.h
+++ b/kalman-vae_amd/csrc/vae_conv_up_wino.h
@@ -261,19 +261,21 @@
   static constexpr int RED = 2048;
 };
 
-template <int S>
-__global__ __launch_bounds__(512) void k_dec_up_bwd_data_wino(const float *__restrict__ W, const float *__restrict__ out,
-                                                              const float *__restrict__ g_out, float *__restrict__ g_x, int64_t N) {
+template <int S, bool PREMASKED = false, bool MASK_GX = false>
+__global__ __launch_bounds__(512) void k_dec_up_bwd_data_wino(const float *__restrict__ W, const float *__restrict__ x,
+                                                              const float *__restrict__ out, const float *__restrict__ g_out,
+                                                              float *__restrict__ g_x, int64_t N) {
   using D = UpDims<S>;
   using Wd = WinoDims<S>;
   using K = WinoBwd<S>;
-  __shared__ __attribute__((aligned(16))) float raw[2 * K::RAW];
+  static_assert(!MASK_GX || (PREMASKED && S == 8), "MASK_GX: one frame of x per column set, in the space of rawo");
+  __shared__ __attribute__((aligned(16))) float raw[(PREMASKED ? 1 : 2) * K::RAW + (MASK_GX ? K::RED : 0)];
   __shared__ __attribute__((aligned(16))) float work[K::GY + 4 * K::RED];
   float *rawg = raw, *rawo = raw + K::RAW, *gy = work, *red = work + K::GY;
   const int tid = threadIdx.x, lane = tid & 63, wv = tid >> 6, j = lane & 15, g = lane >> 4, hh = wv & 1, kq = wv >> 1;
   const int64_t stride = gridDim.x, nsets = (N + Wd::FPC - 1) / Wd::FPC;
-  const __amdgpu_buffer_rsrc_t rg = em_rsrc(g_out, N * D::YFRAME * 4), ro = em_rsrc(out, N * D::YFRAME * 4),
-                               rgx = em_rsrc(g_x, N * D::XFRAME * 4);
+  const __amdgpu_buffer_rsrc_t rg = em_rsrc(g_out, N * D::YFRAME * 4), ro = em_rsrc(PREMASKED ? g_out : out, N * D::YFRAME * 4),
+                               rxm = em_rsrc(MASK_GX ? x : g_out, N * D::XFRAME * 4), rgx = em_rsrc(g_x, N * D::XFRAME * 4);
   for (int i = tid; i < K::GY; i += 512) gy[i] = 0.f;
 
   float U[16][8];
@@ -301,7 +303,14 @@
     asm volatile("" : "+v"(t2));
     const uint32_t off = (uint32_t)(k * K::RAW + (t2 + 512 * q) * 4) * 4u;
     __builtin_amdgcn_raw_ptr_buffer_load_lds(rg, (__attribute__((address_space(3))) void *)(rawg + (wv * 64 + 512 * q) * 4), 16, off, 0, 0, 0);
-    __builtin_amdgcn_raw_ptr_buffer_load_lds(ro, (__attribute__((address_space(3))) void *)(rawo + (wv * 64 + 512 * q) * 4), 16, off, 0, 0, 0);
+    if constexpr (!PREMASKED)
+      __builtin_amdgcn_raw_ptr_buffer_load_lds(ro, (__attribute__((address_space(3))) void *)(rawo + (wv * 64 + 512 * q) * 4), 16, off, 0, 0, 0);
+  };
+  auto dma_x = [&](int64_t k) {
+    int t2 = tid;
+    asm volatile("" : "+v"(t2));
+    __builtin_amdgcn_raw_ptr_buffer_load_lds(rxm, (__attribute__((address_space(3))) void *)(rawo + wv * 64 * 4), 16,
+                                             (uint32_t)(k * K::RED + t2 * 4) * 4u, 0, 0, 0);
   };
   auto dma = [&](int64_t k) {
 #pragma unroll
@@ -313,7 +322,11 @@
 #pragma unroll
     for (int q = 0; q < 4; ++q) {
       const int e = (t2 + 512 * q) * 4;
-      const float4 gv = *reinterpret_cast<const float4 *>(rawg + e), ov = *reinterpret_cast<const float4 *>(rawo + e);
+      float4 gv = *reinterpret_cast<const float4 *>(rawg + e);
+      if constexpr (!PREMASKED) {
+        const float4 ov = *reinterpret_cast<const float4 *>(rawo + e);
+        gv = make_float4(ov.x > 0.f ? gv.x : 0.f, ov.y > 0.f ? gv.y : 0.f, ov.z > 0.f ? gv.z : 0.f, ov.w > 0.f ? gv.w : 0.f);
+      }
       float *d;
       if constexpr (S == 8) {
         const int c = e >> 8, y = (e >> 4) & 15, xx = e & 15;
@@ -322,10 +335,10 @@
         const int f = e >> 11, c = (e >> 6) & 31, y = (e >> 3) & 7, xx = e & 7;
         d = gy + f * K::FSB + (4 * c + 2 * (y & 1)) * K::PLANE + (y >> 1) * K::RS + (xx >> 1) + 1;
       }
-      d[0] = ov.x > 0.f ? gv.x : 0.f;
-      d[K::PLANE] = ov.y > 0.f ? gv.y : 0.f;
-      d[1] = ov.z > 0.f ? gv.z : 0.f;
-      d[K::PLANE + 1] = ov.w > 0.f ? gv.w : 0.f;
+      d[0] = gv.x;
+      d[K::PLANE] = gv.y;
+      d[1] = gv.z;
+      d[K::PLANE + 1] = gv.w;
     }
   };
   uint32_t done = 0x80000000u;
@@ -334,8 +347,12 @@
     asm volatile("" : "+v"(t2));
     const float4 a = *reinterpret_cast<const float4 *>(red + 4 * t2), b = *reinterpret_cast<const float4 *>(red + K::RED + 4 * t2),
                  c = *reinterpret_cast<const float4 *>(red + 2 * K::RED + 4 * t2), d = *reinterpret_cast<const float4 *>(red + 3 * K::RED + 4 * t2);
-    em_st4(rgx, done + (uint32_t)t2 * 16u, make_float4((a.x + b.x) + (c.x + d.x), (a.y + b.y) + (c.y + d.y), (a.z + b.z) + (c.z + d.z),
-                                                        (a.w + b.w) + (c.w + d.w)));
+    float4 s = make_float4((a.x + b.x) + (c.x + d.x), (a.y + b.y) + (c.y + d.y), (a.z + b.z) + (c.z + d.z), (a.w + b.w) + (c.w + d.w));
+    if constexpr (MASK_GX) {
+      const float4 xv = *reinterpret_cast<const float4 *>(rawo + 4 * t2);
+      s = make_float4(xv.x > 0.f ? s.x : 0.f, xv.y > 0.f ? s.y : 0.f, xv.z > 0.f ? s.z : 0.f, xv.w > 0.f ? s.w : 0.f);
+    }
+    em_st4(rgx, done + (uint32_t)t2 * 16u, s);
   };
   auto patch = [&](int s, float2 (&d)[4][2]) {
 #pragma unroll
@@ -345,7 +362,7 @@
       d[r][1] = *reinterpret_cast<const float2 *>(p + 2);
     }
   };
-  auto compute = [&](int64_t knext) {
+  auto compute = [&](int64_t kcur, int64_t knext) {
     wn_f4 acc[16];
 #pragma unroll
     for (int p = 0; p < 16; ++p) acc[p] = wn_f4{0.f, 0.f, 0.f, 0.f};
@@ -361,6 +378,8 @@
       for (int p = 0; p < 16; ++p) acc[p] = WN_MFMA(U[p][s], v[p], acc[p]);
       __builtin_amdgcn_sched_barrier(0);
       if (s < 4) dma_piece(knext, s);
+      if constexpr (MASK_GX)
+        if (s == 4) dma_x(kcur);
       __builtin_amdgcn_sched_barrier(0);
 #pragma unroll
       for (int r = 0; r < 4; ++r) d[r][0] = dn[r][0], d[r][1] = dn[r][1];
@@ -387,7 +406,7 @@
     __syncthreads();
     WN_STAMP(slot, 2);
     WN_STAMP(slot, 3);
-    compute(k + stride);
+    compute(k, k + stride);
     done = (uint32_t)(k * 2048) * 4u;
     WN_STAMP(slot, 4);
     __syncthreads();
@@ -406,20 +425,20 @@
   static constexpr int VROW = 20, VSET = 8 * 64 * VROW;
 };
 
-template <int S>
+template <int S, bool PREMASKED = false>
 __global__ __launch_bounds__(512) void k_dec_up_wrw_wino(const float *__restrict__ x, const float *__restrict__ out,
                                                          const float *__restrict__ g_out, float *__restrict__ w_partials,
                                                          float *__restrict__ b_partials, int64_t N) {
   using D = UpDims<S>;
   using Wd = WinoDims<S>;
   using K = WinoWrw<S>;
-  __shared__ __attribute__((aligned(16))) float raw[2 * K::RAW];
+  __shared__ __attribute__((aligned(16))) float raw[(PREMASKED ? 1 : 2) * K::RAW];
   __shared__ __attribute__((aligned(16))) float work[K::GY4 + K::XPL + K::VSET];
   float *rawg = raw, *rawo = raw + K::RAW, *gy4 = work, *xp = work + K::GY4, *vt = xp + K::XPL;
   const int tid = threadIdx.x, lane = tid & 63, wv = tid >> 6, j = lane & 15, g = lane >> 4;
   const int64_t stride = gridDim.x, nsets = (N + Wd::FPC - 1) / Wd::FPC;
   const __amdgpu_buffer_rsrc_t rx = em_rsrc(x, N * D::XFRAME * 4), rg = em_rsrc(g_out, N * D::YFRAME * 4),
-                               ro = em_rsrc(out, N * D::YFRAME * 4);
+                               ro = em_rsrc(PREMASKED ? g_out : out, N * D::YFRAME * 4);
   for (int i = tid; i < K::XPL; i += 512) xp[i] = 0.f;
 
   wn_f4 acc[16][2];
@@ -432,7 +451,8 @@
     asm volatile("" : "+v"(t2));
     const uint32_t off = (uint32_t)(k * K::RAW + (t2 + 512 * q) * 4) * 4u;
     __builtin_amdgcn_raw_ptr_buffer_load_lds(rg, (__attribute__((address_space(3))) void *)(rawg + (wv * 64 + 512 * q) * 4), 16, off, 0, 0, 0);
-    __builtin_amdgcn_raw_ptr_buffer_load_lds(ro, (__attribute__((address_space(3))) void *)(rawo + (wv * 64 + 512 * q) * 4), 16, off, 0, 0, 0);
+    if constexpr (!PREMASKED)
+      __builtin_amdgcn_raw_ptr_buffer_load_lds(ro, (__attribute__((address_space(3))) void *)(rawo + (wv * 64 + 512 * q) * 4), 16, off, 0, 0, 0);
   };
   auto dma = [&](int64_t k) {
 #pragma unroll
@@ -457,7 +477,11 @@
 #pragma unroll
     for (int q = 0; q < 4; ++q) {
       const int e = (t2 + 512 * q) * 4;
-      const float4 gv = *reinterpret_cast<const float4 *>(rawg + e), ov = *reinterpret_cast<const float4 *>(rawo + e);
+      float4 gv = *reinterpret_cast<const float4 *>(rawg + e);
+      if constexpr (!PREMASKED) {
+        const float4 ov = *reinterpret_cast<const float4 *>(rawo + e);
+        gv = make_float4(ov.x > 0.f ? gv.x : 0.f, ov.y > 0.f ? gv.y : 0.f, ov.z > 0.f ? gv.z : 0.f, ov.w > 0.f ? gv.w : 0.f);
+      }
       int ks, co, tg, a;
       if constexpr (S == 8) {
         const int c = e >> 8, y = (e >> 4) & 15, xx = e & 15;
@@ -467,8 +491,8 @@
         ks = f, co = 4 * c + 2 * (y & 1), tg = 2 * (y >> 2) + (xx >> 2), a = (y >> 1) & 1;
       }
       float *d = gy4 + ((ks * 128 + co) * 4 + tg) * 4 + 2 * a;
-      *reinterpret_cast<float2 *>(d) = make_float2(ov.x > 0.f ? gv.x : 0.f, ov.z > 0.f ? gv.z : 0.f);
-      *reinterpret_cast<float2 *>(d + 16) = make_float2(ov.y > 0.f ? gv.y : 0.f, ov.w > 0.f ? gv.w : 0.f);
+      *reinterpret_cast<float2 *>(d) = make_float2(gv.x, gv.z);
+      *reinterpret_cast<float2 *>(d + 16) = make_float2(gv.y, gv.w);
     }
   };
   auto transform = [&]() {
diff --git a/kalman-vae_amd/csrc/vae_loss.h b/kalman-vae_amd/csrc/vae_loss.h
--- a/kalman-vae_amd/csrc/vae_loss.h
+++ b/kalman-vae_amd/csrc/vae_loss.h
@@ -54,5 +54,29 @@
   free(g);
   return rc;
 }
+static void kv_relu_mask_host(float *g, const float *act, int64_t n) {
+  for (int64_t i = 0; i < n; ++i) g[i] = act[i] > 0.f ? g[i] : 0.f;
+}
+int kvae_dec_head_bwd_masked(const float *in, const float *W, const float *g_logits, float *g_in, float *w_partials,
+                             float *b_partials, float *w_scratch, int64_t N, int32_t Cin, int32_t side, void *) {
+  const int rc = kvae_dec_head_bwd(in, W, g_logits, g_in, w_partials, b_partials, w_scratch, N, Cin, side, nullptr);
+  if (!rc && g_in) kv_relu_mask_host(g_in, in, N * Cin * side * side);
+  return rc;
+}
+int kvae_dec_head_loss_bwd_masked(const float *in, const float *W, const float *logits, const float *x, const float *g_frame,
+                                  float *g_in, float *w_partials, float *b_partials, float *w_scratch, int64_t N, int32_t Cin,
+                                  int32_t side, void *) {
+  const int rc = kvae_dec_head_loss_bwd(in, W, logits, x, g_frame, g_in, w_partials, b_partials, w_scratch, N, Cin, side, nullptr);
+  if (!rc && g_in) kv_relu_mask_host(g_in, in, N * Cin * side * side);
+  return rc;
+}
+int kvae_dec_up_bwd_flags(const float *x, const float *W, const float *out, const float *g_out, float *g_x, float *w_partials,
+                          float *b_partials, int64_t N, int32_t Cin, int32_t side, int32_t flags, void *) {
+  if (!x || !W || !out || !g_out || !w_partials || !b_partials) return KVAE_ERR_NULL;
+  if (N < 1 || (flags & ~(KVAE_UP_G_PREMASKED | KVAE_UP_MASK_GX))) return KVAE_ERR_ARG;
+  const int rc = kvae_dec_up_bwd(x, W, out, g_out, g_x, w_partials, b_partials, N, Cin, side, nullptr);
+  if (!rc && g_x && (flags & KVAE_UP_MASK_GX)) kv_relu_mask_host(g_x, x, N * Cin * side * side);
+  return rc;
+}
 }
 #endif
diff --git a/kalman-vae_amd/kvae/_native.py b/kalman-vae_amd/kvae/_native.py
--- a/kalman-vae_amd/kvae/_native.py
+++ b/kalman-vae_amd/kvae/_native.py
@@ -10,7 +10,7 @@
 KVAE_MAX_DIM = 16
 KVAE_MAX_K = 16
 LSTM_MAX_H, LSTM_MAX_I = 52, 16
-ABI_VERSION = 20
+ABI_VERSION = 21
 
 _STATUS = {1: "KVAE_ERR_DIMS (n, m, p must be in [1,16]; B, T >= 1)", 2: "KVAE_ERR_NULL", 3: "KVAE_ERR_LAUNCH",
            4: "KVAE_ERR_ARG"}
@@ -100,7 +100,8 @@
     "kvae_bias_shuffle_act_bwd", "kvae_bias_partial_rows", "kvae_colsum", "kvae_colsum2", "kvae_clip_adam",
     "kvae_regime_fwd", "kvae_regime_bwd", "kvae_regime_decode", "kvae_regime_decode_ws_bytes", "kvae_bigru_fwd",
     "kvae_bigru_bwd", "kvae_bce_frames_fwd", "kvae_bce_frames_bwd", "kvae_dec_head_fwd", "kvae_dec_head_bwd",
-    "kvae_dec_head_loss_fwd", "kvae_dec_head_loss_bwd",
+    "kvae_dec_head_loss_fwd", "kvae_dec_head_loss_bwd", "kvae_dec_head_bwd_masked", "kvae_dec_head_loss_bwd_masked",
+    "kvae_dec_up_bwd_flags",
     "kvae_enc_stem_fwd", "kvae_enc_stem_bwd", "kvae_conv_edge_partial_rows", "kvae_enc_mid_fwd", "kvae_enc_mid_bwd",
     "kvae_enc_mid_partial_rows", "kvae_dec_up_fwd", "kvae_dec_up_bwd", "kvae_dec_up_partial_rows",
     "kvae_dec_up_set_workgroups", "kvae_enc_head_fwd", "kvae_enc_head_bwd", "kvae_dec_fc_fwd", "kvae_dec_fc_bwd",
@@ -197,6 +198,10 @@
         d.kvae_dec_head_loss_fwd.restype = C.c_int
         d.kvae_dec_head_loss_bwd.argtypes = [vp] * 9 + [C.c_int64, C.c_int32, C.c_int32, vp]
         d.kvae_dec_head_loss_bwd.restype = C.c_int
+        d.kvae_dec_head_bwd_masked.argtypes = d.kvae_dec_head_bwd.argtypes
+        d.kvae_dec_head_bwd_masked.restype = C.c_int
+        d.kvae_dec_head_loss_bwd_masked.argtypes = d.kvae_dec_head_loss_bwd.argtypes
+        d.kvae_dec_head_loss_bwd_masked.restype = C.c_int
         d.kvae_enc_stem_fwd.argtypes = [vp, vp, vp, vp, vp, C.c_int64, C.c_int32, C.c_int32, vp]
         d.kvae_enc_stem_fwd.restype = C.c_int
         d.kvae_enc_stem_bwd.argtypes = [vp] * 6 + [C.c_int64, C.c_int32, C.c_int32, vp]
@@ -210,6 +215,8 @@
         d.kvae_dec_up_fwd.restype = C.c_int
         d.kvae_dec_up_bwd.argtypes = [vp] * 7 + [C.c_int64, C.c_int32, C.c_int32, vp]
         d.kvae_dec_up_bwd.restype = C.c_int
+        d.kvae_dec_up_bwd_flags.argtypes = [vp] * 7 + [C.c_int64, C.c_int32, C.c_int32, C.c_int32, vp]
+        d.kvae_dec_up_bwd_flags.restype = C.c_int
         d.kvae_dec_up_partial_rows.argtypes = [C.c_int64, C.c_int32]
         d.kvae_enc_head_fwd.argtypes = [vp] * 9 + [C.c_int64, C.c_int32, C.c_int32, C.c_float, vp]
         d.kvae_enc_head_fwd.restype = C.c_int
diff --git a/kalman-vae_amd/kvae/vae/fused.py b/kalman-vae_amd/kvae/vae/fused.py
--- a/kalman-vae_amd/kvae/vae/fused.py
+++ b/kalman-vae_amd/kvae/vae/fused.py
@@ -1,3 +1,5 @@
+import os
+
 import torch
 
 from .. import _native as N
@@ -49,6 +51,19 @@
     return BiasShuffleAct.apply(y, conv.bias, r, relu)
 
 
+UP_G_PREMASKED, UP_MASK_GX = 1, 2
+
+
+def premask_plan(kinds):
+    plan = [[False, False] for _ in kinds]
+    mode = os.environ.get("KVAE_PREMASK", "1")
+    if mode != "0":
+        for i in range(len(kinds) - 1):
+            if kinds[i] == "up" and kinds[i + 1] in (("head",) if mode == "head" else ("up", "head")):
+                plan[i][0] = plan[i + 1][1] = True
+    return [tuple(p) for p in plan]
+
+
 class DecoderHead(torch.autograd.Function):
 
     SCRATCH = 2304
@@ -60,7 +75,7 @@
                 and conv.bias is not None)
 
     @staticmethod
-    def forward(ctx, h, weight, bias):
+    def forward(ctx, h, weight, bias, mask_gh=False):
         h, weight, bias = h.contiguous(), weight.contiguous(), bias.contiguous()
         Nb, Cin, s, _ = h.shape
         logits = torch.empty(Nb, 1, 2 * s, 2 * s, device=h.device, dtype=torch.float32)
@@ -69,6 +84,7 @@
         lib.check(lib.dll.kvae_dec_head_fwd(N.ptr(h), N.ptr(weight), N.ptr(bias), N.ptr(logits), N.ptr(scratch), Nb, Cin, s,
                                             N.stream_for(h)), "kvae_dec_head_fwd")
         ctx.save_for_backward(h, weight)
+        ctx.mask_gh = bool(mask_gh)
         return logits
 
     @staticmethod
@@ -82,19 +98,20 @@
         wp = torch.empty(rows, weight.numel(), device=h.device, dtype=torch.float32)
         bp = torch.empty(rows, 4, device=h.device, dtype=torch.float32)
         scratch = torch.empty(DecoderHead.SCRATCH, device=h.device, dtype=torch.float32)
-        lib.check(lib.dll.kvae_dec_head_bwd(N.ptr(h), N.ptr(weight), N.ptr(g), N.ptr(g_h) if g_h is not None else None,
-                                            N.ptr(wp), N.ptr(bp), N.ptr(scratch), Nb, Cin, s, N.stream_for(h)),
-                  "kvae_dec_head_bwd")
+        bwd = lib.dll.kvae_dec_head_bwd_masked if ctx.mask_gh else lib.dll.kvae_dec_head_bwd
+        lib.check(bwd(N.ptr(h), N.ptr(weight), N.ptr(g), N.ptr(g_h) if g_h is not None else None,
+                      N.ptr(wp), N.ptr(bp), N.ptr(scratch), Nb, Cin, s, N.stream_for(h)), "kvae_dec_head_bwd")
         gw, gb = colsum_pair(wp, bp)
-        return g_h, gw.view_as(weight), gb
+        return g_h, gw.view_as(weight), gb, None
 
 
 class DecoderHeadBernoulli(torch.autograd.Function):
 
     @staticmethod
-    def forward(ctx, h, weight, bias, x, *with_recon):
-        ctx.n_opt = len(with_recon)
-        with_recon = with_recon[0] if with_recon else True
+    def forward(ctx, h, weight, bias, x, *opt):
+        ctx.n_opt = len(opt)
+        with_recon = opt[0] if opt else True
+        ctx.mask_gh = bool(opt[1]) if len(opt) > 1 else False
         h, weight, bias, x = h.contiguous(), weight.contiguous(), bias.contiguous(), x.contiguous()
         Nb, Cin, s, _ = h.shape
         logits = torch.empty(Nb, 1, 2 * s, 2 * s, device=h.device, dtype=torch.float32)
@@ -125,9 +142,9 @@
         scratch = torch.empty(DecoderHead.SCRATCH, device=h.device, dtype=torch.float32)
         if g_logits is None:
             g_ll = g_ll.contiguous()
-            lib.check(lib.dll.kvae_dec_head_loss_bwd(N.ptr(h), N.ptr(weight), N.ptr(logits), N.ptr(x), N.ptr(g_ll), _optr(g_h),
-                                                     N.ptr(wp), N.ptr(bp), N.ptr(scratch), Nb, Cin, s, N.stream_for(h)),
-                      "kvae_dec_head_loss_bwd")
+            bwd = lib.dll.kvae_dec_head_loss_bwd_masked if ctx.mask_gh else lib.dll.kvae_dec_head_loss_bwd
+            lib.check(bwd(N.ptr(h), N.ptr(weight), N.ptr(logits), N.ptr(x), N.ptr(g_ll), _optr(g_h),
+                          N.ptr(wp), N.ptr(bp), N.ptr(scratch), Nb, Cin, s, N.stream_for(h)), "kvae_dec_head_loss_bwd")
         else:
             g = g_logits.contiguous()
             if g_ll is not None:
@@ -135,8 +152,9 @@
                 lib.check(lib.dll.kvae_bce_frames_bwd(N.ptr(logits), N.ptr(x), N.ptr(g_ll.contiguous()), N.ptr(gl), Nb,
                                                       logits.numel() // Nb, N.stream_for(h)), "kvae_bce_frames_bwd")
                 g = gl + g
-            lib.check(lib.dll.kvae_dec_head_bwd(N.ptr(h), N.ptr(weight), N.ptr(g), _optr(g_h), N.ptr(wp), N.ptr(bp),
-                                                N.ptr(scratch), Nb, Cin, s, N.stream_for(h)), "kvae_dec_head_bwd")
+            bwd = lib.dll.kvae_dec_head_bwd_masked if ctx.mask_gh else lib.dll.kvae_dec_head_bwd
+            lib.check(bwd(N.ptr(h), N.ptr(weight), N.ptr(g), _optr(g_h), N.ptr(wp), N.ptr(bp),
+                          N.ptr(scratch), Nb, Cin, s, N.stream_for(h)), "kvae_dec_head_bwd")
         gw, gb = colsum_pair(wp, bp)
         return (g_h, gw.view_as(weight), gb, None) + (None,) * ctx.n_opt
 
@@ -231,7 +249,8 @@
                 and conv.dilation == (1, 1) and conv.groups == 1 and conv.bias is not None)
 
     @staticmethod
-    def forward(ctx, x, weight, bias):
+    def forward(ctx, x, weight, bias, g_premasked=False, mask_gx=False):
+        ctx.flags = (UP_G_PREMASKED if g_premasked else 0) | (UP_MASK_GX if mask_gx else 0)
         x, weight, bias = x.contiguous(), weight.contiguous(), bias.contiguous()
         Nb, Cin, s, _ = x.shape
         out = torch.empty(Nb, 32, 2 * s, 2 * s, device=x.device, dtype=torch.float32)
@@ -254,12 +273,16 @@
             rows = lib.dll.kvae_dec_up_partial_rows(b - a, s)
             wp = torch.empty(rows, weight.numel(), device=x.device, dtype=torch.float32)
             bp = torch.empty(rows, 128, device=x.device, dtype=torch.float32)
-            lib.check(N.timed(f"dec_up_bwd_s{s}", x, lambda: lib.dll.kvae_dec_up_bwd(
-                N.ptr(x[a:b]), N.ptr(weight), N.ptr(out[a:b]), N.ptr(g[a:b]), N.ptr(g_x[a:b]) if g_x is not None else None, N.ptr(wp),
-                N.ptr(bp), b - a, Cin, s, N.stream_for(x))), "kvae_dec_up_bwd")
+            args = (N.ptr(x[a:b]), N.ptr(weight), N.ptr(out[a:b]), N.ptr(g[a:b]), N.ptr(g_x[a:b]) if g_x is not None else None,
+                    N.ptr(wp), N.ptr(bp), b - a, Cin, s)
+            if ctx.flags:
+                lib.check(N.timed(f"dec_up_bwd_s{s}", x, lambda: lib.dll.kvae_dec_up_bwd_flags(*args, ctx.flags, N.stream_for(x))),
+                          "kvae_dec_up_bwd_flags")
+            else:
+                lib.check(N.timed(f"dec_up_bwd_s{s}", x, lambda: lib.dll.kvae_dec_up_bwd(*args, N.stream_for(x))), "kvae_dec_up_bwd")
             cw, cb = colsum_pair(wp, bp)
             gw, gb = _acc(gw, cw), _acc(gb, cb)
-        return g_x, gw.view_as(weight), gb
+        return g_x, gw.view_as(weight), gb, None, None
 
 
 def _optr(t):
diff --git a/kalman-vae_amd/kvae/vae/vae.py b/kalman-vae_amd/kvae/vae/vae.py
--- a/kalman-vae_amd/kvae/vae/vae.py
+++ b/kalman-vae_amd/kvae/vae/vae.py
@@ -6,7 +6,8 @@
 
 from kvae import _native
 from kvae.utils.config import KVAEConfig
-from kvae.vae.fused import DecoderFc, DecoderHead, DecoderHeadBernoulli, DecoderUp, EncoderHead, EncoderMid, EncoderStem, conv_block
+from kvae.vae.fused import (DecoderFc, DecoderHead, DecoderHeadBernoulli, DecoderUp, EncoderHead, EncoderMid, EncoderStem, conv_block,
+                            premask_plan)
 
 
 def _conv_out(size, k, s, p):
@@ -82,17 +83,23 @@
         if not fused:
             return self.deconv_layers(h), None, None
         layers = list(self.deconv_layers)
-        for i, layer in enumerate(layers):
-            if isinstance(layer, nn.Conv2d):
-                relu = i + 2 < len(layers) and isinstance(layers[i + 2], nn.ReLU)
-                if not relu and x is not None and i + 2 == len(layers) and self.head_loss_supported(h, layer, x):
-                    return DecoderHeadBernoulli.apply(h, layer.weight, layer.bias, x, with_recon)
-                if not relu and DecoderHead.supported(h, layer):
-                    h = DecoderHead.apply(h, layer.weight, layer.bias)
-                elif relu and DecoderUp.supported(h, layer):
-                    h = DecoderUp.apply(h, layer.weight, layer.bias)
-                else:
-                    h = conv_block(h, layer, r=2, relu=relu)
+        convs = [(i, layer, i + 2 < len(layers) and isinstance(layers[i + 2], nn.ReLU))
+                 for i, layer in enumerate(layers) if isinstance(layer, nn.Conv2d)]
+        kinds, shape = [], h
+        for _, layer, relu in convs:
+            kinds.append("up" if relu and DecoderUp.supported(shape, layer) else
+                         "head" if not relu and DecoderHead.supported(shape, layer) else "block")
+            shape = torch.empty(shape.shape[0], layer.out_channels // 4, 2 * shape.shape[2], 2 * shape.shape[3], device="meta")
+        plan = premask_plan(kinds)
+        for (i, layer, relu), kind, (g_premasked, mask_gx) in zip(convs, kinds, plan):
+            if kind == "head" and x is not None and i + 2 == len(layers) and self.head_loss_supported(h, layer, x):
+                return DecoderHeadBernoulli.apply(h, layer.weight, layer.bias, x, with_recon, mask_gx)
+            if kind == "head":
+                h = DecoderHead.apply(h, layer.weight, layer.bias, mask_gx)
+            elif kind == "up":
+                h = DecoderUp.apply(h, layer.weight, layer.bias, g_premasked, mask_gx)
+            else:
+                h = conv_block(h, layer, r=2, relu=relu)
         return h, None, None
 
     def forward(self, a: torch.Tensor) -> torch.Tensor:
```

After: 98120 sequences/s, median of 6. 1.01x the previous value.
